# KVM-Explorer/AscendPathTracing

Hardware: AMD Instinct MI355X
Metric: Mray/s (ray segments per second) at 1920x1080, 8 bounces, 256 spp, demo scene (higher is better)
Workload: dtype f32; 1 GPU; C2: gen_spheres() 8-sphere scene, 1920x1080, S=64 (256 spp), depth 8, rays generated on device (counter RNG, seed 0), K-mode arithmetic, all segments traced (no retirement); segments_per_gpu=4246732800, parallelism=single GPU

## Files before the change

### __graft_entry__.py

```python
import os
import subprocess
import sys

ROOT = os.path.dirname(os.path.abspath(__file__))
if ROOT not in sys.path:
    sys.path.insert(0, ROOT)


def _is_current():
    import glob
    try:
        from ascendpathtracing_amd import _lib
    except ImportError:
        return False
    pkg = os.path.join(ROOT, "ascendpathtracing_amd")
    csrc = os.path.join(pkg, "csrc")
    pairs = [([os.path.join(pkg, "librender_mi355x.so"), os.path.join(pkg, "render_gpu")] + [st.built_path for st in _lib.STAGES.values()],
              glob.glob(os.path.join(csrc, "*.h")) + glob.glob(os.path.join(csrc, "*.hip")) + glob.glob(os.path.join(csrc, "*.cpp"))
              + [os.path.join(csrc, "Makefile"), os.path.join(csrc, "apt_exports.map")] + _lib.public_headers()),
             ([os.path.join(ROOT, "oracle", "libpt_oracle.so")],
              [os.path.join(ROOT, "oracle", "pt_oracle.c"), os.path.join(ROOT, "oracle", "Makefile")])]
    for outs, srcs in pairs:
        if not all(os.path.exists(o) for o in outs):
            return False
        if min(os.path.getmtime(o) for o in outs) < max(os.path.getmtime(x) for x in srcs):
            return False
    return True


def _load_all():
    import ascendpathtracing_amd
    from ascendpathtracing_amd import _lib
    _lib.lib()
    for name in _lib.STAGES:
        _lib.stage_lib(name)
    return ascendpathtracing_amd


def build():
    import fcntl
    if _is_current():
        return _load_all()
    with open(os.path.join(ROOT, ".build.lock"), "w") as lock:
        fcntl.flock(lock, fcntl.LOCK_EX)
        try:
            subprocess.run(["make", "-s", "-C", os.path.join(ROOT, "ascendpathtracing_amd", "csrc")], check=True, stdout=sys.stderr)
            subprocess.run(["make", "-s", "-C", os.path.join(ROOT, "oracle")], check=True, stdout=sys.stderr)
            tiny = os.path.join(ROOT, "profiles", "microbench", "lib_tiny_guard.so")
            lib_so = os.path.join(ROOT, "ascendpathtracing_amd", "librender_mi355x.so")
            if not os.path.exists(tiny) or os.path.getmtime(tiny) < os.path.getmtime(lib_so):
                r = subprocess.run(["bash", os.path.join(ROOT, "profiles", "build_variant.sh"), "tiny_guard", "-DAPT_TEST_TINY_GUARD"], stdout=sys.stderr)
                if r.returncode != 0:
                    print("build(): the test variant lib_tiny_guard.so could not be built (ignored)", file=sys.stderr)
        finally:
            fcntl.flock(lock, fcntl.LOCK_UN)
    return _load_all()


def smoke():
    build()
    import numpy as np
    import torch
    import ascendpathtracing_amd as apt
    from ascendpathtracing_amd import gen_data, render
    from oracle import oracle
    apt._lib.require_gpu()
    rays = gen_data.gen_rays(16, 16, 1, seed=0)
    sph = gen_data.gen_spheres()
    d_rays, d_sph = torch.from_numpy(rays.ravel()).cuda(), torch.from_numpy(sph).cuda()
    colors = torch.zeros(3 * 1024, device="cuda")
    render.set_default_params(apt.default_params())
    render.render_do(8, None, None, d_rays, d_sph, colors)
    torch.cuda.synchronize()
    want, _ = oracle.render_paths(oracle.make_params(16, 16, 1, depth=5, mode=oracle.MODE_K), rays, sph)
    got = colors.cpu().numpy().view(np.uint32)
    assert np.array_equal(got, want.ravel().view(np.uint32)), "render_do differs from the CPU restatement"
    for s_, d_ in ((8, 5), (32, 8)):
        p = apt.make_params(16, 16, s_, depth=d_, seed=1)
        fb, u8 = render.render_frame(p, d_sph)
        torch.cuda.synchronize()
        fb_w, u8_w, _, _ = oracle.render_frame(oracle.make_params(16, 16, s_, depth=d_, seed=1), sph, threads=4)
        assert np.array_equal(fb.cpu().numpy().view(np.uint32), fb_w.view(np.uint32)), "render_frame differs"
        assert np.array_equal(u8.cpu().numpy(), u8_w)
    print("smoke ok: render_do and render_frame are bit-identical to the oracle on", torch.cuda.get_device_name(0))


if __name__ == "__main__":
    build()
    if len(sys.argv) > 1 and sys.argv[1] == "smoke":
        smoke()
```

### ascendpathtracing_amd/csrc/apt_host.h

```cpp
#pragma once
#include <stdint.h>

#include <mutex>

#include "../../include/render_mi355x.h"
#include "pt_core.h"

#define APT_API __attribute__((visibility("default")))

namespace apt {

void clear_error();
int set_error(int code, const char *fmt, const char *detail = "");

constexpr uint32_t kDefaultRefillLanes = 32;
constexpr int kMaxStatusDevices = 16;

struct Debug {
    uint32_t queue_ppw = 0;
    uint32_t queue_nbuf = 0;
    uint32_t queue_lds_pad = 0;
    uint32_t grid_walk = 0;
    double grid_spheres_per_cell = 0;
};

}

struct apt_context {
    struct Values {
        apt_render_params params;
        unsigned long long *trace_counter;
        uint32_t refill_lanes;
        apt::Debug debug;
        bool has_camera = false;
        apt_camera camera;
        bool has_env = false;
        apt_environment env;
    };
    apt_context();
    Values snapshot();
    void set_params(const apt_render_params &p);
    void set_trace_counter(unsigned long long *c);
    void set_refill_lanes(uint32_t lanes);
    void set_camera(const apt_camera *cam_or_null);
    void set_environment(const apt_environment *env_or_null);
    int set_debug(const char *key, double value);
    int get_debug(const char *key, double *value);

    uint32_t *status_lookup(int dev);
    uint32_t *status_adopt(int dev, uint32_t *fresh, uint32_t **spare);
    void status_release(uint32_t *out[apt::kMaxStatusDevices]);

  private:
    std::mutex m_;
    Values v_;
    uint32_t *status_[apt::kMaxStatusDevices] = {};
};

namespace apt {
apt_context &default_context();
int film_resolve_check(const apt_film_resolve *r, const void *film, const void *table, const void *out, const void *u8, const char *what);
inline double grid_spheres_per_cell() {
    const double knob = default_context().snapshot().debug.grid_spheres_per_cell;
    return knob > 0.0 ? knob : kGridSpheresPerCell;
}
}
```

### ascendpathtracing_amd/csrc/pt_kernels.h

```cpp
#pragma once
#include "pt_trace.h"
#include "pt_trace2.h"
#include "pt_queue.h"
#include "pt_frame_mt.h"

namespace {

template <int MODE, int SC, bool RETIRE>
__global__ __launch_bounds__(kBlock, SC == kSceneGrid ? APT_GRID_WAVES : 1) void render_paths_kernel(const float *__restrict__ rays,
                                                              const float *__restrict__ sph,
                                                              float *__restrict__ colors, uint64_t n_total,
                                                              uint64_t begin, uint64_t count, TraceArgs ta) {
    constexpr bool NS8 = SC == kScene8;
    static_assert(!(RETIRE && NS8), "APT_FLAG_RETIRE on the 8-sphere scene is render_paths_queue_kernel's");
    __shared__ float4 tab[kTab8Floats4];
    __shared__ float4 tile[SC == kSceneTiles ? kTile : 1];
    Scene8 sc;
    Tab8 tab8{tab, tab + 8};
    if (NS8) tab8 = load_scene8(sph, sc, tab);
    const uint64_t local = (uint64_t)blockIdx.x * kBlock + threadIdx.x;
    const bool valid = local < count;
    const uint64_t p = begin + (valid ? local : 0);
    PathState s;
    path_init(s, rays[p], rays[n_total + p], rays[2 * n_total + p], rays[3 * n_total + p], rays[4 * n_total + p],
              rays[5 * n_total + p]);
    uint32_t traced;
    if (SC == kScene8) traced = trace_ns8<MODE, RETIRE>(sc, tab8, s, valid, ta, p);
    else if (SC == kSceneGrid) traced = trace_grid<MODE, RETIRE>(sph, ta.grid, s, valid, ta, p);
    else traced = trace_dyn<MODE, RETIRE>(sph, tile, s, valid, ta, p);
    if (valid) {
        const Gain3 gain = load_gain(sph, ta);
        colors[p] = s.rxy.x * gain.r;
        colors[n_total + p] = s.rxy.y * gain.g;
        colors[2 * n_total + p] = s.rz * gain.b;
    }
    count_traced(ta, valid ? traced : 0);
}

constexpr int kPaths2Pairs = 2;
template <int MODE>
__global__ __launch_bounds__(kBlock, APT_TWO_WAVES) void render_paths2_kernel(const float *__restrict__ rays, const float *__restrict__ sph,
                                                                              float *__restrict__ colors, uint64_t n_total, uint64_t begin,
                                                                              uint64_t count, TraceArgs ta) {
    __shared__ float4 tab[kTab8Floats4];
    Scene8 sc;
    const Tab8 tab8 = load_scene8(sph, sc, tab);
    const Gain3 gain = load_gain(sph, ta);
    uint32_t traced = 0;
    for (int it = 0; it < kPaths2Pairs; ++it) {
        const uint64_t local = ((uint64_t)blockIdx.x * kPaths2Pairs + it) * (2 * kBlock) + threadIdx.x;
        if (__builtin_amdgcn_readfirstlane((int)(((uint64_t)blockIdx.x * kPaths2Pairs + it) * (2 * kBlock) >= count))) break;
        const bool va = local < count, vb = local + kBlock < count;
        const uint64_t pa = begin + (va ? local : 0), pb = vb ? begin + local + kBlock : pa;
        PathPair pp;
        pp.ox = f2{rays[pa], rays[pb]}; pp.oy = f2{rays[n_total + pa], rays[n_total + pb]}; pp.oz = f2{rays[2 * n_total + pa], rays[2 * n_total + pb]};
        pp.dx = f2{rays[3 * n_total + pa], rays[3 * n_total + pb]}; pp.dy = f2{rays[4 * n_total + pa], rays[4 * n_total + pb]};
        pp.dz = f2{rays[5 * n_total + pa], rays[5 * n_total + pb]};
        trace2_ns8<MODE>(sc, tab8, pp, ta, sc.planes);
        if (va) { colors[pa] = pp.rx.x * gain.r; colors[n_total + pa] = pp.ry.x * gain.g; colors[2 * n_total + pa] = pp.rz.x * gain.b; }
        if (vb) { colors[pb] = pp.rx.y * gain.r; colors[n_total + pb] = pp.ry.y * gain.g; colors[2 * n_total + pb] = pp.rz.y * gain.b; }
        traced += ((va ? 1u : 0u) + (vb ? 1u : 0u)) * ta.depth;
    }
    count_traced(ta, traced);
}

constexpr uint32_t kQueueChunk = 64 * 16;
template <int MODE>
__global__ __launch_bounds__(kBlock) void render_paths_queue_kernel(const float *__restrict__ rays,
                                                                    const float *__restrict__ sph,
                                                                    float *__restrict__ colors, uint64_t n_total,
                                                                    uint64_t begin, uint64_t count, TraceArgs ta) {
    __shared__ float4 tab[kTab8Floats4];
    Scene8 sc;
    const Tab8 tab8 = load_scene8(sph, sc, tab);
    const Gain3 gain = load_gain(sph, ta);
    const KeyConsts kc = make_key_consts(ta.eps);
    const uint64_t wave = (uint64_t)blockIdx.x * (kBlock / 64) + (uint32_t)__builtin_amdgcn_readfirstlane((int)(threadIdx.x >> 6));
    uint64_t next = wave * kQueueChunk;
    const uint64_t end = min(count, next + kQueueChunk);
    uint32_t depth_left = 0, traced = 0;
    uint64_t cur = 0, cur_key = 0;
    PathState s, n;
    path_init(s, 0.f, 0.f, 0.f, 0.f, 0.f, 1.f);
    n = s;
    f2 thr_xy = {1.0f, 1.0f};
    float thr_z = 1.0f;
    uint64_t alive = 0;
    auto refill = [&](PathState &st) -> bool {
        for (;;) {
            const bool want = depth_left == 0;
            const unsigned long long wants = __ballot(want);
            if (next < end && wants) {
                const uint32_t rank = __builtin_amdgcn_mbcnt_hi((uint32_t)(wants >> 32), __builtin_amdgcn_mbcnt_lo((uint32_t)wants, 0u));
                const uint64_t remaining = end - next;
                const bool take = want && rank < remaining;
                if (take) {
                    cur = begin + next + rank;
                    st.oxy = f2{rays[cur], rays[n_total + cur]}; st.oz = rays[2 * n_total + cur];
                    st.dxy = f2{rays[3 * n_total + cur], rays[4 * n_total + cur]}; st.dz = rays[5 * n_total + cur];
                    thr_xy = f2{1.0f, 1.0f}; thr_z = 1.0f;
                    depth_left = ta.depth;
                    if (ta.rr_start) cur_key = rr_path_key(ta.seed, cur);
                    if (ta.depth == 0) { colors[cur] = gain.r; colors[n_total + cur] = gain.g; colors[2 * n_total + cur] = gain.b; }
                }
                alive |= __builtin_amdgcn_ballot_w64(take);
                next += min((uint64_t)__popcll(wants), remaining);
            }
            if (__any(depth_left != 0)) return false;
            if (next >= end) return true;
        }
    };
    auto post = [&](bool active) {
        if (ta.rr_start && ta.depth - depth_left + 1 >= ta.rr_start) {
            PathState t;
            t.rxy = thr_xy; t.rz = thr_z; t.alive = select_const(alive, 1);
            russian_roulette(t, cur_key, ta.depth - depth_left);
            thr_xy = t.rxy; thr_z = t.rz;
        }
        traced += active ? 1u : 0u;
        depth_left -= active ? 1u : 0u;
        const bool fin = select_const(alive, 1) == 0 || (thr_xy.x == 0.0f && thr_xy.y == 0.0f && thr_z == 0.0f);
        if (active && (depth_left == 0 || fin)) {
            depth_left = 0;
            colors[cur] = thr_xy.x * gain.r;
            colors[n_total + cur] = thr_xy.y * gain.g;
            colors[2 * n_total + cur] = thr_z * gain.b;
        }
    };
    auto step_fast = [&](const PathState &in, PathState &out) -> bool {
        const bool active = depth_left != 0;
        Albedo albedo;
        uint64_t alive_out = alive;
        const uint64_t redo = bounce_ns8_v2p<MODE>(sc, tab8, in, out, ta, kc, alive_out, albedo, sc.planes) & __builtin_amdgcn_ballot_w64(active);
        if (__builtin_expect(redo != 0, 0)) {
            const bool fin = select_const(alive, 1) == 0 || (thr_xy.x == 0.0f && thr_xy.y == 0.0f && thr_z == 0.0f);
            if (__any(select_const(redo, 1) != 0 && !fin)) return true;
        }
        apply_albedo(thr_xy, thr_z, albedo, alive_out);
        alive = alive_out;
        post(active);
        return false;
    };
    auto step_exact = [&](PathState &in, PathState &out) {
        const bool active = depth_left != 0;
        in.rxy = thr_xy; in.rz = thr_z; in.alive = select_const(alive, 1);
        bounce_ns8_exact<MODE>(sc, tab8, in, out, ta);
        thr_xy = out.rxy; thr_z = out.rz;
        alive = __builtin_amdgcn_ballot_w64(out.alive != 0);
        post(active);
    };
    bool done = refill(s), exact = !eps_allows_rootkey(ta.eps);
    if (!done && !exact) {
        for (;;) {
            if (__builtin_expect(step_fast(s, n), 0)) { exact = true; break; }
            if ((done = refill(n))) break;
            if (__builtin_expect(step_fast(n, s), 0)) { exact = true; s = n; break; }
            if ((done = refill(s))) break;
        }
    }
    if (!done && exact) {
        for (;;) {
            step_exact(s, n);
            s = n;
            if (refill(s)) break;
        }
    }
    count_traced(ta, traced);
}

template <int MODE, int SC, int GROUP, bool RETIRE, bool TWO = false>
__global__ __launch_bounds__(kBlock, TWO ? APT_TWO_WAVES : (SC == kSceneGrid ? APT_GRID_WAVES : (SC == kSceneTiles ? APT_TILE_WAVES : APT_FULL_WAVES))) void render_frame_kernel(const float *__restrict__ sph, FrameArgs fa,
                                                              TraceArgs ta, LeafProg lp) {
    constexpr bool NS8 = SC == kScene8;
    static_assert(!(RETIRE && NS8 && GROUP == 8), "APT_FLAG_RETIRE on the 8-sphere scene with samples >= 8 is render_frame_queue8_kernel's (pt_queue.h)");
    if (SC == kSceneGrid && ta.grid_walk == 2u && grid_queue_usable(ta)) return;
    __shared__ float4 tab[kTab8Floats4];
    __shared__ float4 tile[SC == kSceneTiles ? kTile : 1];
    extern __shared__ float dyn_lds[];
    float *stack_lds = dyn_lds;
    float *queue_lds = dyn_lds + (lp.nleaves > 1 ? kMaxStack * 3 * kStackSlots : 0);
    __shared__ Camera cam;
    park_camera(cam, fa);
    Scene8 sc;
    Tab8 tab8{tab, tab + 8};
    if (NS8) tab8 = load_scene8(sph, sc, tab);
    else __syncthreads();
    const bool planes = NS8 && sc.planes;
    (void)planes;

    const uint32_t lane = threadIdx.x & 63;
    const FrameLane<GROUP> fl = frame_lane<GROUP>(fa);
    const uint32_t j = fl.j, sub = fl.sub;
    const uint64_t pl = fl.pl;
    const bool valid = fl.valid;
    const uint32_t pi = fl.pi, pj = fl.pj, sy = fl.sy, sx = fl.sx;
    const uint64_t pbase = fl.pbase;
    uint32_t traced = 0;
    uint32_t queue_traced = 0;

    const Gain3 gain = load_gain(sph, ta);
    struct Col { float r, g, b; };
    auto sample = [&](uint32_t k) __attribute__((always_inline)) -> Col {
        uint64_t pb = pbase;
        if (TWO) {
            uint32_t tid = threadIdx.x;
            asm volatile("" : "+v"(tid));
            pb = frame_lane<GROUP>(fa, tid).pbase;
        }
        double u1, u2;
        path_uniforms(fa.seed, pb + k, u1, u2);
        float rox, roy, roz, rdx, rdy, rdz;
        camera_ray(cam, fa.width, fa.height, pi, pj, sy, sx, u1, u2, rox, roy, roz, rdx, rdy, rdz);
        PathState s;
        path_init(s, rox, roy, roz, rdx, rdy, rdz);
        if (SC == kScene8) traced += trace_ns8<MODE, RETIRE>(sc, tab8, s, valid, ta, pb + k);
        else if (SC == kSceneGrid) traced += trace_grid<MODE, RETIRE>(sph, ta.grid, s, valid, ta, pb + k);
        else traced += trace_dyn<MODE, RETIRE>(sph, tile, s, valid, ta, pb + k);
        return Col{s.rxy.x * gain.r, s.rxy.y * gain.g, s.rz * gain.b};
    };
    auto add = [](const Col &a, const Col &b) { return Col{a.r + b.r, a.g + b.g, a.b + b.b}; };
    struct Col2 { Col a, b; };
    const uint64_t lane_state = TWO ? lane_base_state(fa.seed, pbase, j) : 0;
    auto sample2 = [&](uint32_t u) __attribute__((always_inline)) -> Col2 {
        PathPair pp;
        camera_ray_pair(cam, fa.width, fa.height, pi, pj, sy, sx, chain_state_uniform(lane_state, u), pp.ox, pp.oy, pp.oz, pp.dx, pp.dy, pp.dz);
        asm("" : "+v"(pp.ox), "+v"(pp.oy), "+v"(pp.oz), "+v"(pp.dx), "+v"(pp.dy), "+v"(pp.dz));
        trace2_ns8<MODE>(sc, tab8, pp, ta, planes);
        traced += 2 * ta.depth;
        return Col2{Col{pp.rx.x * gain.r, pp.ry.x * gain.g, pp.rz.x * gain.b}, Col{pp.rx.y * gain.r, pp.ry.y * gain.g, pp.rz.y * gain.b}};
    };

    float res[3] = {0.0f, 0.0f, 0.0f};
    uint32_t start = 0;
    int sp = 0;
    for (uint32_t leaf = 0; leaf < lp.nleaves; ++leaf) {
        const uint32_t n = lp.len(leaf);
        float acc[3];
        if (GROUP == 1) {
            Col a = {0.0f, 0.0f, 0.0f};
            for (uint32_t k = 0; k < n; ++k) a = add(a, sample(start + k));
            acc[0] = a.r; acc[1] = a.g; acc[2] = a.b;
        } else {
            const uint32_t nfull = n & ~7u;
            if (RETIRE && SC == kSceneTiles) {
                float *colq = queue_lds + (size_t)(threadIdx.x >> 6) * 3u * 8u * lp.maxleaf;
                const uint32_t total = 8u * nfull;
                const uint32_t qstride = 8u * lp.maxleaf;
                uint32_t next = 0;
                uint32_t depth_left = 0, cur_item = 0, slot_item = 0;
                uint64_t cur_key = 0, slot_key = 0;
                uint32_t n_bounce_exec = 0, n_gen_exec = 0;
                float sl_ox = 0.f, sl_oy = 0.f, sl_oz = 0.f, sl_dx = 0.f, sl_dy = 0.f, sl_dz = 1.f;
                bool slot_full = false, slot_valid = false, cur_valid = false;
                PathState s;
                path_init(s, 0.f, 0.f, 0.f, 0.f, 0.f, 1.f);
                auto refill = [&](PathState &cur) -> bool {
                    for (;;) {
                        const bool want = !slot_full;
                        const unsigned long long wants = __ballot(want);
                        const bool busy_any = __any(depth_left != 0 || slot_full);
                        if (next < total && wants && ((uint32_t)__popcll(wants) >= ta.refill_lanes || !busy_any)) {
                            ++n_gen_exec;
                            const uint32_t rank = __builtin_amdgcn_mbcnt_hi((uint32_t)(wants >> 32),
                                                  __builtin_amdgcn_mbcnt_lo((uint32_t)wants, 0u));
                            const uint32_t remaining = total - next;
                            const bool take = want && rank < remaining;
                            const uint32_t item = take ? next + rank : 0u;
                            const uint32_t g = item / nfull, k = item - g * nfull;
                            const int src = (int)(8u * g);
                            const uint32_t gpi = __shfl(pi, src, 64), gpj = __shfl(pj, src, 64);
                            const uint32_t gsub = __shfl(sub, src, 64);
                            const uint32_t blo = __shfl((uint32_t)pbase, src, 64), bhi = __shfl((uint32_t)(pbase >> 32), src, 64);
                            const bool gvalid = __shfl((int)valid, src, 64) != 0;
                            if (take) {
                                slot_valid = gvalid;
                                double u1, u2;
                                const uint64_t path = (((uint64_t)bhi << 32) | blo) + start + k;
                                if (ta.rr_start) slot_key = rr_path_key(ta.seed, path);
                                path_uniforms(fa.seed, path, u1, u2);
                                camera_ray(cam, fa.width, fa.height, gpi, gpj, gsub >> 1, gsub & 1u, u1, u2, sl_ox, sl_oy, sl_oz, sl_dx,
                                           sl_dy, sl_dz);
                                slot_item = item;
                                slot_full = true;
                            }
                            next += min((uint32_t)__popcll(wants), remaining);
                        }
                        const bool begin = depth_left == 0 && slot_full;
                        if (begin) {
                            cur.oxy = f2{sl_ox, sl_oy}; cur.oz = sl_oz; cur.dxy = f2{sl_dx, sl_dy}; cur.dz = sl_dz;
                            cur.rxy = f2{1.0f, 1.0f}; cur.rz = 1.0f; cur.alive = 1u;
                            cur_item = slot_item;
                            cur_key = slot_key;
                            cur_valid = slot_valid;
                            depth_left = ta.depth;
                            slot_full = false;
                            if (ta.depth == 0 || !cur_valid) {
                                depth_left = 0;
                                colq[cur_item] = gain.r; colq[qstride + cur_item] = gain.g; colq[2 * qstride + cur_item] = gain.b;
                            }
                        }
                        if (__any(depth_left != 0)) return false;
                        if (next >= total && !__any(slot_full)) return true;
                    }
                };
                for (;;) {
                    const bool wave_done = refill(s);
                    if (__syncthreads_and(wave_done)) break;
                    const bool active = depth_left != 0;
                    dyn_segment<MODE>(sph, tile, s, !active, ta);
                    ++n_bounce_exec;
                    if (active && ta.rr_start && ta.depth - depth_left + 1 >= ta.rr_start)
                        russian_roulette(s, cur_key, ta.depth - depth_left);
                    queue_traced += (active && cur_valid) ? 1u : 0u;
                    depth_left -= active ? 1u : 0u;
                    if (active && (depth_left == 0 || path_finished(s))) {
                        depth_left = 0;
                        colq[cur_item] = s.rxy.x * gain.r;
                        colq[qstride + cur_item] = s.rxy.y * gain.g;
                        colq[2 * qstride + cur_item] = s.rz * gain.b;
                    }
                }
                __syncthreads();
                {
                    const uint32_t base = (lane >> 3) * nfull + j;
#pragma unroll
                    for (int ch = 0; ch < 3; ++ch) acc[ch] = colq[ch * qstride + base];
                    for (uint32_t i8 = 8; i8 < nfull; i8 += 8) {
#pragma unroll
                        for (int ch = 0; ch < 3; ++ch) acc[ch] = acc[ch] + colq[ch * qstride + base + i8];
                    }
                }
                __syncthreads();
                if (ta.traced && lane == 0) {
                    atomicAdd(ta.traced + 1, 64ull * n_bounce_exec);
                    atomicAdd(ta.traced + 2, 64ull * n_gen_exec);
                }
            } else {
                Col a;
                uint32_t i8;
                if (TWO && nfull >= 16) {
                    Col2 c = sample2(start);
                    a = add(c.a, c.b);
                    for (i8 = 16; i8 + 16 <= nfull; i8 += 16) {
                        c = sample2(start + i8);
                        a = add(a, c.a);
                        a = add(a, c.b);
                    }
                } else {
                    a = sample(start + j);
                    i8 = 8;
                }
                for (; i8 < nfull; i8 += 8) a = add(a, sample(start + i8 + j));
                acc[0] = a.r; acc[1] = a.g; acc[2] = a.b;
            }
#pragma unroll
            for (int ch = 0; ch < 3; ++ch) {
                float v = acc[ch];
                v = v + __shfl_xor(v, 1, 64);
                v = v + __shfl_xor(v, 2, 64);
                v = v + __shfl_xor(v, 4, 64);
                acc[ch] = v;
            }
            const uint32_t nt = n - nfull;
            if (nt) {
                const uint32_t traced_before = traced;
                const Col c = sample(start + nfull + (j < nt ? j : 0));
                if (j >= nt) traced = traced_before;
                for (uint32_t t = 0; t < nt; ++t) {
                    const int src = (int)((lane & ~7u) + t);
                    acc[0] = acc[0] + __shfl(c.r, src, 64);
                    acc[1] = acc[1] + __shfl(c.g, src, 64);
                    acc[2] = acc[2] + __shfl(c.b, src, 64);
                }
            }
        }
        start += n;
        if (lp.nleaves == 1) {
            res[0] = acc[0]; res[1] = acc[1]; res[2] = acc[2];
        } else {
#pragma unroll
            for (int ch = 0; ch < 3; ++ch) stack_lds[(sp * 3 + ch) * kStackSlots + (threadIdx.x >> 3)] = acc[ch];
            ++sp;
            for (uint32_t m = 0; m < lp.ncomb(leaf); ++m) {
                --sp;
#pragma unroll
                for (int ch = 0; ch < 3; ++ch) {
                    const float a = stack_lds[((sp - 1) * 3 + ch) * kStackSlots + (threadIdx.x >> 3)];
                    const float b = stack_lds[(sp * 3 + ch) * kStackSlots + (threadIdx.x >> 3)];
                    stack_lds[((sp - 1) * 3 + ch) * kStackSlots + (threadIdx.x >> 3)] = a + b;
                }
            }
        }
    }
    if (lp.nleaves > 1) {
#pragma unroll
        for (int ch = 0; ch < 3; ++ch) res[ch] = stack_lds[ch * kStackSlots + (threadIdx.x >> 3)];
    }

    __shared__ uint32_t u8pack[frame_u8_words(GROUP)];
    frame_decode<GROUP, TWO>(fa, pl, valid, res, u8pack);
    count_traced(ta, (valid ? traced : 0) + queue_traced);
}

__global__ __launch_bounds__(kBlock) void test_scene_kernel(const float *__restrict__ rays,
                                                            const float *__restrict__ sph, float *__restrict__ out,
                                                            uint64_t n_total, uint32_t ns, int32_t light, float eps) {
    const uint64_t p = (uint64_t)blockIdx.x * kBlock + threadIdx.x;
    if (p >= n_total) return;
    const float ox = rays[p], oy = rays[n_total + p], oz = rays[2 * n_total + p];
    const float dx = rays[3 * n_total + p], dy = rays[4 * n_total + p], dz = rays[5 * n_total + p];
    float mind = kMissT;
    int id = -1;
    for (uint32_t k = 0; k < ns; ++k)
        test_scene_sphere(sph[ns + k], sph[2 * (size_t)ns + k], sph[3 * (size_t)ns + k], sph[k], ox, oy, oz, dx, dy, dz,
                          eps, (int)k, mind, id);
#pragma unroll
    for (int c = 0; c < 3; ++c) {
        float v = 0.0f;
        if (id >= 0) v = (id == light) ? sph[(size_t)(4 + c) * ns + id] : sph[(size_t)(7 + c) * ns + id];
        out[(uint64_t)c * n_total + p] = v;
    }
}

__global__ __launch_bounds__(kBlock) void gen_rays_kernel(Camera cam, uint32_t width, uint32_t height,
                                                          uint32_t samples, uint64_t seed, uint64_t n_total,
                                                          uint64_t begin, uint64_t count, float *__restrict__ rays) {
    const uint64_t local = (uint64_t)blockIdx.x * kBlock + threadIdx.x;
    if (local >= count) return;
    const uint64_t p = begin + local;
    uint32_t i, j, sy, sx;
    path_coords(p, height, samples, i, j, sy, sx);
    double u1, u2;
    path_uniforms(seed, p, u1, u2);
    float rox, roy, roz, rdx, rdy, rdz;
    camera_ray(cam, width, height, i, j, sy, sx, u1, u2, rox, roy, roz, rdx, rdy, rdz);
    rays[p] = rox; rays[n_total + p] = roy; rays[2 * n_total + p] = roz;
    rays[3 * n_total + p] = rdx; rays[4 * n_total + p] = rdy; rays[5 * n_total + p] = rdz;
}

constexpr int kMtN = 624, kMtM = 397, kPathsPerBlock = 156;

__device__ __forceinline__ uint32_t mt_temper(uint32_t y) {
    y ^= y >> 11;
    y ^= (y << 7) & 0x9d2c5680u;
    y ^= (y << 15) & 0xefc60000u;
    y ^= y >> 18;
    return y;
}

constexpr int kMtGroup = 8;

__global__ __launch_bounds__(kBlock) void gen_rays_mt_kernel(const uint32_t *__restrict__ checkpoints, uint32_t stride,
                                                             uint64_t first_block, uint64_t num_blocks, Camera cam, uint32_t width,
                                                             uint32_t height, uint32_t samples, uint64_t n_total,
                                                             uint64_t begin, uint64_t end, float *__restrict__ rays) {
    __shared__ uint32_t mt[kMtN];
    __shared__ __align__(16) uint32_t outw[kMtGroup * kMtN];
    const uint64_t cb = first_block + (uint64_t)blockIdx.x * stride;
    for (int i = threadIdx.x; i < kMtN; i += kBlock) mt[i] = checkpoints[(uint64_t)blockIdx.x * kMtN + i];
    __syncthreads();
    const uint64_t last = min(cb + stride, num_blocks);
    for (uint64_t g0 = cb; g0 < last; g0 += kMtGroup) {
        const uint32_t nb = (uint32_t)min((uint64_t)kMtGroup, last - g0);
        for (uint32_t bl = 0; bl < nb; ++bl) {
            if (g0 + bl != cb) {
                const int t = threadIdx.x;
                const int lo[3] = {0, 227, 454}, hi[3] = {227, 454, 624};
#pragma unroll
                for (int ph = 0; ph < 3; ++ph) {
                    const int i = lo[ph] + t;
                    uint32_t v = 0;
                    const bool on = i < hi[ph];
                    if (on) {
                        const uint32_t y = (mt[i] & 0x80000000u) | (mt[(i + 1) % kMtN] & 0x7fffffffu);
                        v = mt[(i + kMtM) % kMtN] ^ (y >> 1) ^ ((y & 1u) ? 0x9908b0dfu : 0u);
                    }
                    __syncthreads();
                    if (on) mt[i] = v;
                    __syncthreads();
                }
            }
            for (int i = threadIdx.x; i < kMtN; i += kBlock) outw[bl * kMtN + i] = mt_temper(mt[i]);
        }
        __syncthreads();
        const uint64_t pbase = g0 * kPathsPerBlock;
        const uint64_t rb = pbase / samples;
        const uint32_t kb = (uint32_t)(pbase - rb * samples);
        const uint32_t npaths = nb * kPathsPerBlock;
        for (uint32_t q = threadIdx.x; q < npaths; q += kBlock) {
            const uint64_t p = pbase + q;
            if (p < begin || p >= end) continue;
            const uint4 w4 = *reinterpret_cast<const uint4 *>(&outw[4 * q]);
            const uint32_t a1 = w4.x >> 5, b1 = w4.y >> 6, a2 = w4.z >> 5, b2 = w4.w >> 6;
            const double u1 = ((double)a1 * 67108864.0 + (double)b1) / 9007199254740992.0;
            const double u2 = ((double)a2 * 67108864.0 + (double)b2) / 9007199254740992.0;
            const uint64_t r = rb + (kb + q) / samples;
            const uint32_t sx = (uint32_t)(r & 1), sy = (uint32_t)((r >> 1) & 1);
            const uint64_t r4 = r >> 2;
            uint32_t i, j;
            if (r4 <= 0xffffffffull) { i = (uint32_t)r4 / height; j = (uint32_t)r4 - i * height; }
            else { i = (uint32_t)(r4 / height); j = (uint32_t)(r4 % height); }
            float rox, roy, roz, rdx, rdy, rdz;
            camera_ray(cam, width, height, i, j, sy, sx, u1, u2, rox, roy, roz, rdx, rdy, rdz);
            rays[p] = rox; rays[n_total + p] = roy; rays[2 * n_total + p] = roz;
            rays[3 * n_total + p] = rdx; rays[4 * n_total + p] = rdy; rays[5 * n_total + p] = rdz;
        }
        __syncthreads();
    }
}

__device__ float pairwise_leaf(const float *a, uint32_t n) {
    if (n < 8) {
        float r = 0.0f;
        for (uint32_t i = 0; i < n; ++i) r = r + a[i];
        return r;
    }
    float r[8];
#pragma unroll
    for (int k = 0; k < 8; ++k) r[k] = a[k];
    uint32_t i;
    for (i = 8; i < n - (n % 8); i += 8) {
#pragma unroll
        for (int k = 0; k < 8; ++k) r[k] = r[k] + a[i + k];
    }
    float res = ((r[0] + r[1]) + (r[2] + r[3])) + ((r[4] + r[5]) + (r[6] + r[7]));
    for (; i < n; ++i) res = res + a[i];
    return res;
}

__global__ __launch_bounds__(kBlock) void decode_color_kernel(const float *__restrict__ colors, uint32_t samples,
                                                              uint64_t npix, LeafProg lp, float *__restrict__ fb,
                                                              uint8_t *__restrict__ fb_u8) {
    const uint64_t L = (uint64_t)blockIdx.x * kBlock + threadIdx.x;
    const uint32_t sub = (uint32_t)(L & 3);
    const uint64_t pc = L >> 2;
    const bool valid = pc < 3 * npix;
    const uint64_t ch = valid ? pc / npix : 0, q = valid ? pc % npix : 0;
    const uint64_t n_total = npix * 4 * samples;
    const float *a = colors + ch * n_total + (q * 4 + sub) * samples;
    float st[kMaxStack];
    int sp = 0;
    uint32_t start = 0;
    for (uint32_t leaf = 0; leaf < lp.nleaves; ++leaf) {
        st[sp++] = pairwise_leaf(a + start, lp.len(leaf));
        start += lp.len(leaf);
        for (uint32_t m = 0; m < lp.ncomb(leaf); ++m) { --sp; st[sp - 1] = st[sp - 1] + st[sp]; }
    }
    const float mean = st[0] / (float)samples;
    const int gbase = (int)((threadIdx.x & 63) & ~3u);
    double acc = 0.0;
#pragma unroll
    for (int sq = 0; sq < 4; ++sq) acc = acc + (double)__shfl(mean, gbase + sq, 64);
    const double v = acc / 4;
    const double cl = v < 0 ? 0 : (v > 1 ? 1 : v);
    if (valid && sub == 0) {
        fb[ch * npix + q] = (float)cl;
        if (fb_u8) fb_u8[q * 3 + ch] = (uint8_t)(cl * 255);
    }
}

__global__ __launch_bounds__(kBlock) void decode_color_kernel8(const float *__restrict__ colors, uint32_t samples,
                                                               uint64_t npix, LeafProg lp, float *__restrict__ fb,
                                                               uint8_t *__restrict__ fb_u8) {
    __shared__ float stack_lds[kMaxStack * kStackSlots];
    const uint32_t lane = threadIdx.x & 63;
    const uint32_t j = threadIdx.x & 7u;
    const uint32_t sub = (threadIdx.x >> 3) & 3u;
    const uint32_t slot = threadIdx.x >> 3;
    const uint64_t n_total = npix * 4 * samples;
    const uint64_t items = 3 * npix, per_block = kBlock / 32;
    const uint64_t rounds = (items + per_block * gridDim.x - 1) / (per_block * gridDim.x);
    for (uint64_t r = 0; r < rounds; ++r) {
    const uint64_t pc = (r * gridDim.x + blockIdx.x) * per_block + (threadIdx.x >> 5);
    const bool valid = pc < items;
    const uint64_t ch = valid ? pc / npix : 0, q = valid ? pc % npix : 0;
    const float *a = colors + ch * n_total + (q * 4 + sub) * samples;
    float res = 0.0f;
    uint32_t start = 0;
    int sp = 0;
    for (uint32_t leaf = 0; leaf < lp.nleaves; ++leaf) {
        const uint32_t n = lp.len(leaf), nfull = n & ~7u;
        float v[16];
#pragma unroll
        for (int m = 0; m < 16; ++m) v[m] = (8u * m < nfull) ? a[start + 8u * m + j] : 0.0f;
        float acc = v[0];
#pragma unroll
        for (int m = 1; m < 16; ++m)
            if (8u * m < nfull) acc = acc + v[m];
        acc = acc + __shfl_xor(acc, 1, 64);
        acc = acc + __shfl_xor(acc, 2, 64);
        acc = acc + __shfl_xor(acc, 4, 64);
        const uint32_t nt = n - nfull;
        if (nt) {
            const float c = a[start + nfull + (j < nt ? j : 0)];
            for (uint32_t t = 0; t < nt; ++t) acc = acc + __shfl(c, (int)((lane & ~7u) + t), 64);
        }
        start += n;
        if (lp.nleaves == 1) {
            res = acc;
        } else {
            stack_lds[sp * kStackSlots + slot] = acc;
            ++sp;
            for (uint32_t m = 0; m < lp.ncomb(leaf); ++m) {
                --sp;
                const float x = stack_lds[(sp - 1) * kStackSlots + slot], y = stack_lds[sp * kStackSlots + slot];
                stack_lds[(sp - 1) * kStackSlots + slot] = x + y;
            }
        }
    }
    if (lp.nleaves > 1) res = stack_lds[slot];
    const float mean = res / (float)samples;
    const int gbase = (int)(lane & ~31u);
    double acc64 = 0.0;
#pragma unroll
    for (int sq = 0; sq < 4; ++sq) acc64 = acc64 + (double)__shfl(mean, gbase + sq * 8, 64);
    const double v = acc64 / 4;
    const double cl = v < 0 ? 0 : (v > 1 ? 1 : v);
    if (valid && (lane & 31u) == 0) {
        fb[ch * npix + q] = (float)cl;
        if (fb_u8) fb_u8[q * 3 + ch] = (uint8_t)(cl * 255);
    }
    }
}

constexpr int kDecode4Blocks = 4;
__global__ __launch_bounds__(kBlock) void decode_color_kernel4(const float *__restrict__ colors, uint32_t samples, uint64_t npix, LeafProg lp,
                                                               float *__restrict__ fb, uint8_t *__restrict__ fb_u8) {
    const uint32_t lane = threadIdx.x & 63;
    const uint32_t L = threadIdx.x & 1u;
    const uint32_t sub = (threadIdx.x >> 1) & 3u;
    const uint64_t n_total = npix * 4 * samples;
    const uint64_t items = 3 * npix, per_block = kBlock / 8;
    const uint64_t rounds = (items + per_block * gridDim.x - 1) / (per_block * gridDim.x);
    const uint32_t n = lp.len(0), nfull = n & ~7u, nt = n - nfull;
    for (uint64_t r = 0; r < rounds; ++r) {
        const uint64_t pc = (r * gridDim.x + blockIdx.x) * per_block + (threadIdx.x >> 3);
        const bool valid = pc < items;
        const uint64_t ch = valid ? pc / npix : 0, q = valid ? pc % npix : 0;
        const float *a = colors + ch * n_total + (q * 4 + sub) * samples;
        float4 v[kDecode4Blocks];
#pragma unroll
        for (int m = 0; m < kDecode4Blocks; ++m)
            v[m] = (8u * m < nfull) ? *reinterpret_cast<const float4 *>(a + 8u * m + 4u * L) : make_float4(0.f, 0.f, 0.f, 0.f);
        float4 acc = v[0];
#pragma unroll
        for (int m = 1; m < kDecode4Blocks; ++m)
            if (8u * m < nfull) { acc.x = acc.x + v[m].x; acc.y = acc.y + v[m].y; acc.z = acc.z + v[m].z; acc.w = acc.w + v[m].w; }
        float res = (acc.x + acc.y) + (acc.z + acc.w);
        res = res + __shfl_xor(res, 1, 64);
        if (nt) {
            float c[4];
#pragma unroll
            for (int k = 0; k < 4; ++k) c[k] = (4u * L + k < nt) ? a[nfull + 4u * L + k] : 0.0f;
#pragma unroll
            for (int t = 0; t < 7; ++t)
                if ((uint32_t)t < nt) res = res + __shfl(c[t & 3], (int)((lane & ~1u) + (t >> 2)), 64);
        }
        const float mean = res / (float)samples;
        const int gbase = (int)(lane & ~7u);
        double acc64 = 0.0;
#pragma unroll
        for (int sq = 0; sq < 4; ++sq) acc64 = acc64 + (double)__shfl(mean, gbase + sq * 2, 64);
        const double v64 = acc64 / 4;
        const double cl = v64 < 0 ? 0 : (v64 > 1 ? 1 : v64);
        if (valid && (lane & 7u) == 0) {
            fb[ch * npix + q] = (float)cl;
            if (fb_u8) fb_u8[q * 3 + ch] = (uint8_t)(cl * 255);
        }
    }
}

__global__ __launch_bounds__(kBlock) void selftest_sqrt_kernel(int variant, uint64_t begin, uint64_t count,
                                                               unsigned long long *result) {
#if defined(__HIP_DEVICE_COMPILE__)
    const uint64_t stride = (uint64_t)gridDim.x * kBlock;
    unsigned long long bad = 0, first = ~0ull;
    for (uint64_t i = (uint64_t)blockIdx.x * kBlock + threadIdx.x; i < count; i += stride) {
        const uint32_t bits = (uint32_t)(begin + i);
        const float x = __uint_as_float(bits);
        float amin = 1.0f;
        const float got = variant == 0 ? sqrt_rn_core(x, amin) : variant == 1 ? sqrt_rn_markstein(x, amin)
                        : variant == 2 ? sqrt_rn_rsq1(x, amin) : sqrt_rn_rsq2(x, amin);
        const float want = sqrtf(x);
        const bool fallback = amin < 0x1p-96f;
        const bool same = (__float_as_uint(got) == __float_as_uint(want)) || (got != got && want != want);
        if (!same && !fallback) { ++bad; if (first == ~0ull) first = bits; }
    }
    if (bad) {
        atomicAdd(&result[0], bad);
        atomicMin(&result[1], first);
    }
#endif
}

__global__ __launch_bounds__(kBlock) void selftest_div3_kernel(uint64_t begin, uint64_t count,
                                                               unsigned long long *result) {
#if defined(__HIP_DEVICE_COMPILE__)
    const uint64_t stride = (uint64_t)gridDim.x * kBlock;
    unsigned long long bad = 0, first = ~0ull, accepted = 0;
    if (blockIdx.x == 0 && threadIdx.x == 0) {
        const float qn = __uint_as_float(0x7fc00000u);
        float one = 1.0f, a = -0.5f, b = 3.0f;
        asm volatile("" : "+v"(one), "+v"(a), "+v"(b));
        const float m0 = minimum3_abs(one, a, b), m1 = minimum3_abs(one, qn, b), m2 = minimum3_abs(one, b, -qn), m3 = minimum3_abs(qn, a, b);
        if (!(m0 == 0.5f) || m1 == m1 || m2 == m2 || m3 == m3 || (m1 >= kFastMin) || !(m0 >= kFastMin)) { ++bad; first = 0; }
    }
    for (uint64_t i = (uint64_t)blockIdx.x * kBlock + threadIdx.x; i < count; i += stride) {
        const uint64_t ctr = begin + i;
        uint64_t h = splitmix64(ctr);
        float v[3];
#pragma unroll
        for (int k = 0; k < 3; ++k) {
            h = splitmix64(h);
            uint32_t man = (uint32_t)h & 0x7fffffu, ex = 127u - 100u + (uint32_t)((h >> 23) % 134u), sg = (uint32_t)(h >> 63);
            if ((ctr & 3u) == 0u) {
                const uint32_t pick = (uint32_t)(h >> 40) & 7u;
                man = pick == 0 ? 0x7fffffu : pick == 1 ? 0u : pick == 2 ? 1u : pick == 3 ? 0x7ffffeu
                    : pick == 4 ? 0x400000u : pick == 5 ? 0x3fffffu : pick == 6 ? 0x400001u : man;
                if (((h >> 44) & 3u) == 0u) ex = ((h >> 46) & 1u) ? 127u - 96u : 127u + 29u;
            }
            v[k] = __uint_as_float((sg << 31) | (ex << 23) | man);
        }
        if ((ctr & 63u) == 1u) v[(ctr >> 6) % 3u] = (ctr & 64u) ? 0.0f : -0.0f;
        const uint32_t how = (uint32_t)((ctr >> 2) % 3u);
        float len2, d;
        if (how == 0) {
            len2 = 0.0f + v[0] * v[0];
            len2 = len2 + v[1] * v[1];
            len2 = len2 + v[2] * v[2];
            d = sqrtf(len2);
        } else if (how == 1) {
            const float p0 = v[0] * v[0], p1 = v[1] * v[1], p2 = v[2] * v[2];
            double acc = 0.0 + (double)p0;
            acc = acc + (double)p1;
            acc = acc + (double)p2;
            len2 = (float)acc;
            d = sqrtf(len2);
        } else {
            h = splitmix64(h);
            uint32_t man = (uint32_t)h & 0x7fffffu;
            const uint32_t ex = 127u - 50u + (uint32_t)((h >> 23) % 84u);
            if ((ctr & 3u) == 0u) man = ((h >> 40) & 1u) ? 0x7fffffu : 0u;
            d = __uint_as_float((ex << 23) | man);
            len2 = d * d;
        }
        const float wx = v[0] / d, wy = v[1] / d, wz = v[2] / d;
        {
            float ux, uy, uz, amin = 1.0f;
            uint32_t hiflag = 0;
            div3_shared(v[0], v[1], v[2], d, len2, ux, uy, uz, amin, hiflag);
            if (!(amin < 0x1p-96f || (int32_t)hiflag < 0)) {
                ++accepted;
                if (__float_as_uint(ux) != __float_as_uint(wx) || __float_as_uint(uy) != __float_as_uint(wy) ||
                    __float_as_uint(uz) != __float_as_uint(wz)) { ++bad; if (first == ~0ull) first = ctr; }
            }
        }
        if (div3_operands_ok(len2, v[0], v[1], v[2])) {
            ++accepted;
            f2 uxy;
            float uz;
            div3_packed(f2{v[0], v[1]}, v[2], d, uxy, uz);
            if (__float_as_uint(uxy.x) != __float_as_uint(wx) || __float_as_uint(uxy.y) != __float_as_uint(wy) ||
                __float_as_uint(uz) != __float_as_uint(wz)) { ++bad; if (first == ~0ull) first = ctr; }
        }
    }
    if (bad) { atomicAdd(&result[0], bad); atomicMin(&result[1], first); }
    atomicAdd(&result[2], accepted);
#endif
}


}
```

### ascendpathtracing_amd/csrc/pt_trace.h

```cpp
#pragma once
#include <hip/hip_runtime.h>
#include <stdint.h>

#include "pt_core.h"
#include "pt_leaf.h"

namespace {

using namespace apt;


constexpr int kBlock = 256;
constexpr int kScene8 = 0, kSceneTiles = 1, kSceneGrid = 2;
constexpr int kTile = 1024;
#ifndef APT_GRID_WAVES
#define APT_GRID_WAVES 8
#endif
#ifndef APT_TILE_WAVES
#define APT_TILE_WAVES 6
#endif
#ifndef APT_TWO_WAVES
#define APT_TWO_WAVES 4
#endif
#ifndef APT_FULL_WAVES
#define APT_FULL_WAVES 6
#endif
constexpr int kMaxStack = 8;
constexpr int kStackSlots = kBlock / 8;


struct Scene8 {
    float cx[8], cy[8], cz[8], r2[8];
    bool planes;
};
__device__ __forceinline__ bool scene8_shares_planes(const Scene8 &sc) {
    auto eq = [](float a, float b) { return f32_bits(a) == f32_bits(b); };
    return eq(sc.cx[2], sc.cx[3]) && eq(sc.cx[2], sc.cx[4]) && eq(sc.cx[2], sc.cx[5]) && eq(sc.cx[2], sc.cx[7]) &&
           eq(sc.cy[0], sc.cy[1]) && eq(sc.cy[0], sc.cy[2]) && eq(sc.cy[0], sc.cy[3]) &&
           eq(sc.cz[0], sc.cz[1]) && eq(sc.cz[0], sc.cz[4]) && eq(sc.cz[0], sc.cz[5]) && eq(sc.cz[0], sc.cz[7]);
}

struct Tab8 { const float4 *geo, *alb; };
constexpr int kTab8Floats4 = 17;

struct TraceArgs {
    uint32_t ns;
    uint32_t depth;
    int32_t light;
    float eps, gain;
    uint32_t refill_lanes;
    uint32_t emission;
    uint32_t rr_start;
    uint64_t seed;
    const uint32_t *grid;
    uint32_t grid_walk;
    unsigned long long *traced;
    uint32_t *status;
};
template <uint32_t K>
__device__ __forceinline__ uint32_t xcd_chunked_block(uint32_t wg, uint32_t nwg) {
    constexpr uint32_t kXcds = 8, G = kXcds * K;
    static_assert((K & (K - 1)) == 0, "shifts and masks");
    const uint32_t full = nwg & ~(G - 1u);
    if (wg >= full) return wg;
    const uint32_t r = wg & (G - 1u);
    return (wg & ~(G - 1u)) + (r & (kXcds - 1u)) * K + r / kXcds;
}

__device__ __forceinline__ void report_status(const TraceArgs &ta, uint32_t bit) {
    if (ta.status && (threadIdx.x & 63u) == 0u) atomicOr(ta.status, bit);
}


__device__ __forceinline__ float twice_canonical(float dot) { return __builtin_fmaf(dot, 2.0f, 0.0f); }
__device__ __forceinline__ f2 twice_canonical(f2 dot) { return __builtin_elementwise_fma(dot, f2{2.0f, 2.0f}, f2{0.0f, 0.0f}); }

__device__ __forceinline__ float sum3_f64(float p0, float p1, float p2) {
    double acc = (double)p0;
    acc = acc + (double)p1;
    acc = acc + (double)p2;
    return (float)acc;
}

template <int MODE>
__device__ __forceinline__ float normal_len2(f2 nxy, float nz) {
    const f2 sq = nxy * nxy;
    if (MODE == kModeOracle) return sum3_f64(sq.x, sq.y, nz * nz);
    const float acc = sq.x + sq.y;
    return acc + nz * nz;
}
template <int MODE>
__device__ __forceinline__ float reflect_k2(f2 dxy, float dz, f2 uxy, float uz) {
    const f2 pr = dxy * uxy;
    const float pz = dz * uz;
    if (MODE == kModeOracle) return twice_canonical(sum3_f64(pr.x, pr.y, pz));
    float dot = pr.x;
    dot = dot + pr.y;
    dot = dot + pz;
    return twice_canonical(dot);
}

struct HitPre2 { f2 b, disc; };
__device__ __forceinline__ HitPre2 intersect_pre2(const f2 cx, const f2 cy, const f2 cz, const f2 r2, float ox,
                                                  float oy, float oz, float dx, float dy, float dz) {
    const f2 ocx = cx - ox, ocy = cy - oy, ocz = cz - oz;
    f2 b = ocx * dx;
    b = b + ocy * dy;
    b = b + ocz * dz;
    f2 c = ocx * ocx;
    c = c + ocy * ocy;
    c = c + ocz * ocz;
    c = c - r2;
    f2 disc = b * b;
    disc = disc - c;
    return {b, disc};
}
__device__ __forceinline__ HitPre2 intersect_pre2(const float4 a, const float4 c4, float ox, float oy, float oz,
                                                  float dx, float dy, float dz) {
    return intersect_pre2(f2{a.x, a.y}, f2{a.z, a.w}, f2{c4.x, c4.y}, f2{c4.z, c4.w}, ox, oy, oz, dx, dy, dz);
}


template <bool WANT_C67 = false>
__device__ __forceinline__ void intersect_pre_planes_pairs(const f2 X1, const f2 X2, const f2 Y1, const f2 Y2, const f2 Y3, const f2 Z1, const f2 Z2,
                                                           const f2 R0, const f2 R1, const f2 R2, const f2 R3, float ox, float oy, float oz,
                                                           float dx, float dy, float dz, HitPre2 (&h)[4], f2 *c67 = nullptr) {
    const f2 x1 = X1 - ox, x2 = X2 - ox, y1 = Y1 - oy, y2 = Y2 - oy, y3 = Y3 - oy, z1 = Z1 - oz, z2 = Z2 - oz;
    auto lo = [](f2 v) { return f2{v.x, v.x}; };
    auto swap = [](f2 v) { return f2{v.y, v.x}; };
    {
        const f2 px1 = x1 * dx, px2 = x2 * dx, py1 = y1 * dy, py2 = y2 * dy, py3 = y3 * dy, pz1 = z1 * dz, pz2 = z2 * dz;
        h[0].b = (px1 + py3) + lo(pz2);
        h[1].b = (lo(px2) + py3) + pz1;
        h[2].b = (lo(px2) + py1) + lo(pz2);
        h[3].b = (swap(px2) + py2) + swap(pz2);
    }
    {
        const f2 qx1 = x1 * x1, qx2 = x2 * x2, qy1 = y1 * y1, qy2 = y2 * y2, qy3 = y3 * y3, qz1 = z1 * z1, qz2 = z2 * z2;
        f2 c0 = (qx1 + qy3) + lo(qz2), c1 = (lo(qx2) + qy3) + qz1, c2 = (lo(qx2) + qy1) + lo(qz2), c3 = (swap(qx2) + qy2) + swap(qz2);
        c0 = c0 - R0; c1 = c1 - R1; c2 = c2 - R2; c3 = c3 - R3;
        h[0].disc = h[0].b * h[0].b - c0; h[1].disc = h[1].b * h[1].b - c1;
        h[2].disc = h[2].b * h[2].b - c2; h[3].disc = h[3].b * h[3].b - c3;
        if (WANT_C67) *c67 = c3;
    }
}
template <bool WANT_C67 = false>
__device__ __forceinline__ void intersect_pre_planes(const Scene8 &sc, float ox, float oy, float oz, float dx, float dy, float dz,
                                                     HitPre2 (&h)[4], f2 *c67 = nullptr) {
    intersect_pre_planes_pairs<WANT_C67>(f2{sc.cx[0], sc.cx[1]}, f2{sc.cx[2], sc.cx[6]}, f2{sc.cy[4], sc.cy[5]}, f2{sc.cy[6], sc.cy[7]}, f2{sc.cy[0], sc.cy[0]},
                               f2{sc.cz[2], sc.cz[3]}, f2{sc.cz[0], sc.cz[6]}, f2{sc.r2[0], sc.r2[1]}, f2{sc.r2[2], sc.r2[3]}, f2{sc.r2[4], sc.r2[5]},
                               f2{sc.r2[6], sc.r2[7]}, ox, oy, oz, dx, dy, dz, h, c67);
}

template <int MODE>
__device__ __forceinline__ void bounce_ns8_exact(const Scene8 &sc, const Tab8 tab, const PathState &s, PathState &n,
                                                 const TraceArgs &ta) {
    const int miss = (MODE == kModeOracle) ? -1 : 0;
    float tmin = kMissT;
    int idx = miss;
#pragma unroll
    for (int k = 0; k < 8; ++k) {
        float t0, t1;
        intersect_roots(sc.cx[k], sc.cy[k], sc.cz[k], sc.r2[k], s.oxy.x, s.oxy.y, s.oz, s.dxy.x, s.dxy.y, s.dz, t0, t1);
        const float t = select_root(t0, t1, ta.eps);
        if (t < tmin) { tmin = t; idx = k; }
    }
    const int g = (idx < 0) ? 7 : idx;
    const float4 c = tab.geo[g], col = tab.alb[g];
    n = s;
    shade_and_reflect<MODE>(n, tmin, c.x, c.y, c.z, col.x, col.y, col.z, idx == ta.light);
}

struct KeyConsts { uint32_t bias, init; uint64_t nbias2; };
__device__ __forceinline__ KeyConsts make_key_consts(float eps) {
    KeyConsts kc;
    kc.bias = f32_bits(eps) + 1u;
    kc.init = f32_bits(kMissT) - kc.bias;
    kc.nbias2 = ((uint64_t)(0u - kc.bias) << 32) | (0x80000000u - kc.bias);
    asm volatile("" : "+v"(kc.bias), "+v"(kc.init));
    asm volatile("" : "+s"(kc.nbias2));
    return kc;
}
template <int HALF>
__device__ __forceinline__ uint64_t root_pair(f2 b, f2 q) {
    uint64_t r;
    if (HALF == 0) asm("v_pk_add_f32 %0, %1, %2 op_sel:[0,0] op_sel_hi:[0,0] neg_lo:[1,0] neg_hi:[0,0]" : "=v"(r) : "v"(b), "v"(q));
    else asm("v_pk_add_f32 %0, %1, %2 op_sel:[1,1] op_sel_hi:[1,1] neg_lo:[1,0] neg_hi:[0,0]" : "=v"(r) : "v"(b), "v"(q));
    return r;
}
__device__ __forceinline__ float min3_abs(float a, float b, float c) {
    float r;
    asm("v_min3_f32 %0, %1, |%2|, |%3|" : "=v"(r) : "v"(a), "v"(b), "v"(c));
    return r;
}
constexpr float kFastMin = 0x1p-29f;
__device__ __forceinline__ float minimum3_abs(float a, float b, float c) {
    float r;
    asm("v_minimum3_f32 %0, %1, |%2|, |%3|" : "=v"(r) : "v"(a), "v"(b), "v"(c));
    return r;
}
__device__ __forceinline__ float minimum3_abs_after_trans(float a, float b, float c) {
    float r;
    asm("s_nop 0\n\tv_minimum3_f32 %0, %1, |%2|, |%3|" : "=v"(r) : "v"(a), "v"(b), "v"(c));
    return r;
}
__device__ __forceinline__ float rsq_here(float x) {
    float r;
    asm("v_rsq_f32 %0, %1\n\ts_nop 0" : "=v"(r) : "v"(x));
    return r;
}
__device__ __forceinline__ uint32_t min3_u32(uint32_t a, uint32_t b, uint32_t c) {
    uint32_t r;
    asm("v_min3_u32 %0, %1, %2, %3" : "=v"(r) : "v"(a), "v"(b), "v"(c));
    return r;
}
__device__ __forceinline__ uint32_t select_const(uint64_t mask, uint32_t value_if_set) {
    uint32_t r;
    asm("" : "+s"(mask));
    asm("v_cndmask_b32_e64 %0, 0, %1, %2" : "=v"(r) : "n"(value_if_set), "s"(mask));
    return r;
}

struct Albedo { f2 xy; float z; };
__device__ __forceinline__ void apply_albedo(f2 &rxy, float &rz, const Albedo &a, uint64_t alive) {
    uint64_t saved;
    asm("" : "+s"(alive));
    asm volatile("s_and_saveexec_b64 %[sv], %[m]\n\t"
                 "v_pk_mul_f32 %[rxy], %[cxy], %[rxy]\n\t"
                 "v_mul_f32 %[rz], %[cz], %[rz]\n\t"
                 "s_mov_b64 exec, %[sv]"
                 : [sv] "=&s"(saved), [rxy] "+v"(rxy), [rz] "+v"(rz)
                 : [m] "s"(alive), [cxy] "v"(a.xy), [cz] "v"(a.z)
                 : "scc");
}

struct Hit8 { float tmin; uint32_t addr; uint64_t light; };
__device__ __forceinline__ bool pair_misses_wave(f2 disc) {
    return __builtin_amdgcn_ballot_w64(__builtin_fmaxf(disc.x, disc.y) >= 0.0f) == 0;
}
constexpr float kBehindGuard = 0x1p-60f;
__device__ __forceinline__ uint64_t sphere_reachable_mask(float disc, float b, float c) {
    return __builtin_amdgcn_ballot_w64(__builtin_amdgcn_fmed3f(disc, b, -c) >= -kBehindGuard);
}
__device__ __forceinline__ uint32_t any_lane(uint64_t mask) {
    uint32_t r;
    asm("s_cmp_lg_u64 %1, 0\n\ts_cselect_b32 %0, 1, 0" : "=s"(r) : "s"(mask) : "scc");
    return r;
}
template <int MODE, bool PLANES = false, int SKIP = 0>
__device__ __forceinline__ Hit8 intersect_ns8_v2(const Scene8 &sc, float ox, float oy, float oz, float dx, float dy, float dz,
                                                 const TraceArgs &ta, const KeyConsts &kc, float &amin) {
    uint32_t best = kc.init;
    uint64_t b0 = 0, b1 = 0, b2 = 0, any = 0;
    auto update_keys = [&](uint32_t m0, uint32_t m1, int k) {
        const uint32_t nb = min3_u32(best, m0, m1);
        const uint64_t better = __builtin_amdgcn_ballot_w64(nb != best);
        best = nb;
        b0 = (k & 1) ? (b0 | better) : (b0 & ~better);
        b1 = (k & 2) ? (b1 | better) : (b1 & ~better);
        b2 = (k & 4) ? (b2 | better) : (b2 & ~better);
        if (MODE == kModeOracle) any |= better;
    };
    auto update64 = [&](uint64_t keys, int k) { update_keys((uint32_t)keys, (uint32_t)(keys >> 32), k); };
    auto full_stage = [&](const HitPre2 &h, int k) __attribute__((always_inline)) {
        amin = minimum3_abs(amin, h.disc.x, h.disc.y);
        const f2 q = sqrt_rn_rsq1_pair(h.disc);
        update64(root_pair<0>(h.b, q) + kc.nbias2, k);
        update64(root_pair<1>(h.b, q) + kc.nbias2, k + 1);
    };
    static_assert((SKIP >> 4) == 0 || ((SKIP >> 4) == 0x8 && PLANES), "the per-sphere form: pair (6,7) of the shared-planes form only");
    HitPre2 hp[4];
    f2 c67 = {0.0f, 0.0f};
    if (PLANES) intersect_pre_planes<(SKIP >> 4) != 0>(sc, ox, oy, oz, dx, dy, dz, hp, &c67);
#pragma unroll
    for (int k = 0; k < 8; k += 2) {
        const HitPre2 h = PLANES ? hp[k / 2]
                                 : intersect_pre2(f2{sc.cx[k], sc.cx[k + 1]}, f2{sc.cy[k], sc.cy[k + 1]}, f2{sc.cz[k], sc.cz[k + 1]},
                                                  f2{sc.r2[k], sc.r2[k + 1]}, ox, oy, oz, dx, dy, dz);
        if ((SKIP >> (k / 2)) & 1) {
            if (pair_misses_wave(h.disc)) continue;
        }
        if ((SKIP >> (4 + k / 2)) & 1) {
            const uint32_t lo = any_lane(sphere_reachable_mask(h.disc.x, h.b.x, c67.x)), hi = any_lane(sphere_reachable_mask(h.disc.y, h.b.y, c67.y));
            uint32_t both = lo & hi, only_lo = lo & ~hi, only_hi = hi & ~lo;
            asm("" : "+s"(both), "+s"(only_lo), "+s"(only_hi));
            if (both != 0u) full_stage(h, k);
            if (only_lo != 0u) {
                amin = minimum3_abs(amin, h.disc.x, h.disc.x);
                const float r0 = rsq_here(h.disc.x);
                update64(root_pair<0>(h.b, sqrt_rsq_step(h.disc, f2{r0, r0})) + kc.nbias2, k);
            }
            if (only_hi != 0u) {
                amin = minimum3_abs(amin, h.disc.y, h.disc.y);
                const float r0 = rsq_here(h.disc.y);
                update64(root_pair<1>(h.b, sqrt_rsq_step(h.disc, f2{r0, r0})) + kc.nbias2, k + 1);
            }
            continue;
        }
        full_stage(h, k);
    }
    const float tmin = bits_f32(best + kc.bias);
    uint64_t light_mask;
    if (MODE == kModeOracle) {
        b0 |= ~any; b1 |= ~any; b2 |= ~any;
    }
    uint32_t addr;
    {
        const uint32_t a0 = select_const(b0, 16), a1 = select_const(b1, 32), a2 = select_const(b2, 64);
        asm("v_or3_b32 %0, %1, %2, %3" : "=v"(addr) : "v"(a0), "v"(a1), "v"(a2));
    }
    light_mask = __builtin_amdgcn_ballot_w64(addr == (uint32_t)ta.light * 16u);
    if (MODE == kModeOracle) light_mask &= any;
    return Hit8{tmin, addr, light_mask};
}

template <int MODE, bool PLANES = false, bool CAN_BE_LAST = false>
__device__ __forceinline__ uint64_t bounce_ns8_v2(const Scene8 &sc, const Tab8 tab, const PathState &s, PathState &n,
                                                  const TraceArgs &ta, const KeyConsts &kc, uint64_t &alive, Albedo &albedo, bool last = false) {
    float amin = 1.0f;
    const Hit8 hit = intersect_ns8_v2<MODE, PLANES>(sc, s.oxy.x, s.oxy.y, s.oz, s.dxy.x, s.dxy.y, s.dz, ta, kc, amin);
    const float tmin = hit.tmin;
    const uint32_t addr = hit.addr;
    const uint64_t light_mask = hit.light;
    const float4 c = *reinterpret_cast<const float4 *>(reinterpret_cast<const char *>(tab.geo) + addr);
    const float4 col = *reinterpret_cast<const float4 *>(reinterpret_cast<const char *>(tab.alb) + addr);
    if (!(CAN_BE_LAST && last)) {
        const f2 oxy = s.oxy, dxy = s.dxy;
        const f2 hxy = oxy + dxy * tmin;
        const float hz = s.oz + s.dz * tmin;
        const f2 nxy = hxy - f2{c.x, c.y};
        const float nz = hz - c.z;
        const float len2 = normal_len2<MODE>(nxy, nz);
        const float r0 = __builtin_amdgcn_rsqf(len2);
        amin = minimum3_abs_after_trans(amin, r0, nxy.x);
        amin = minimum3_abs(amin, nxy.y, nz);
        const float L = sqrt_rsq_step(len2, r0);
        f2 uxy;
        float uz;
        div3_packed(nxy, nz, L, uxy, uz);
        const float k2 = reflect_k2<MODE>(dxy, s.dz, uxy, uz);
        n.dxy = dxy - uxy * k2;
        n.dz = s.dz - uz * k2;
        n.oxy = hxy; n.oz = hz;
    }
    alive &= ~light_mask;
    n.alive = s.alive;
    albedo = Albedo{f2{col.x, col.y}, col.z};
    return __builtin_amdgcn_ballot_w64(!(amin >= kFastMin));
}

struct Bounce8Mid {
    f2 hxy, nxy;
    float hz, nz, len2, r0;
    float4 col;
    uint64_t light;
};
template <int MODE, bool PLANES>
__device__ __forceinline__ uint64_t bounce_ns8_v2_hit(const Scene8 &sc, const Tab8 tab, const PathState &s, const TraceArgs &ta, const KeyConsts &kc,
                                                      Bounce8Mid &m) {
    float amin = 1.0f;
    const Hit8 hit = intersect_ns8_v2<MODE, PLANES>(sc, s.oxy.x, s.oxy.y, s.oz, s.dxy.x, s.dxy.y, s.dz, ta, kc, amin);
    const float tmin = hit.tmin;
    const float4 c = *reinterpret_cast<const float4 *>(reinterpret_cast<const char *>(tab.geo) + hit.addr);
    m.col = *reinterpret_cast<const float4 *>(reinterpret_cast<const char *>(tab.alb) + hit.addr);
    m.light = hit.light;
    m.hxy = s.oxy + s.dxy * tmin;
    m.hz = s.oz + s.dz * tmin;
    m.nxy = m.hxy - f2{c.x, c.y};
    m.nz = m.hz - c.z;
    m.len2 = normal_len2<MODE>(m.nxy, m.nz);
    m.r0 = __builtin_amdgcn_rsqf(m.len2);
    amin = minimum3_abs_after_trans(amin, m.r0, m.nxy.x);
    amin = minimum3_abs(amin, m.nxy.y, m.nz);
    return __builtin_amdgcn_ballot_w64(!(amin >= kFastMin));
}
template <int MODE>
__device__ __forceinline__ void bounce_ns8_v2_reflect(PathState &s, const Bounce8Mid &m, uint64_t &alive, Albedo &albedo) {
    const float L = sqrt_rsq_step(m.len2, m.r0);
    f2 uxy;
    float uz;
    div3_packed(m.nxy, m.nz, L, uxy, uz);
    const float k2 = reflect_k2<MODE>(s.dxy, s.dz, uxy, uz);
    s.dxy = s.dxy - uxy * k2;
    s.dz = s.dz - uz * k2;
    s.oxy = m.hxy; s.oz = m.hz;
    alive &= ~m.light;
    albedo = Albedo{f2{m.col.x, m.col.y}, m.col.z};
}

template <int MODE>
__device__ __forceinline__ float reflect_packed(const PathState &s, float tmin, float cx, float cy, float cz, PathState &n) {
    const f2 hxy = s.oxy + s.dxy * tmin;
    const float hz = s.oz + s.dz * tmin;
    const f2 nxy = hxy - f2{cx, cy};
    const float nz = hz - cz;
    const float len2 = normal_len2<MODE>(nxy, nz);
    const float r0 = __builtin_amdgcn_rsqf(len2);
    float amin = minimum3_abs_after_trans(1.0f, r0, nxy.x);
    amin = minimum3_abs(amin, nxy.y, nz);
    const float L = sqrt_rsq_step(len2, r0);
    f2 uxy;
    float uz;
    div3_packed(nxy, nz, L, uxy, uz);
    const float k2 = reflect_k2<MODE>(s.dxy, s.dz, uxy, uz);
    n.dxy = s.dxy - uxy * k2;
    n.dz = s.dz - uz * k2;
    n.oxy = hxy; n.oz = hz;
    return amin;
}

template <int MODE>
__device__ __forceinline__ uint64_t bounce_ns8_v2p(const Scene8 &sc, const Tab8 tab, const PathState &s, PathState &n, const TraceArgs &ta,
                                                   const KeyConsts &kc, uint64_t &alive, Albedo &albedo, bool planes) {
    return planes ? bounce_ns8_v2<MODE, true>(sc, tab, s, n, ta, kc, alive, albedo)
                  : bounce_ns8_v2<MODE, false>(sc, tab, s, n, ta, kc, alive, albedo);
}

template <int MODE>
__device__ __forceinline__ void bounce_ns8_checked(const Scene8 &sc, const Tab8 tab, const PathState &s, PathState &n,
                                                   const TraceArgs &ta, const KeyConsts &kc, bool fast_ok,
                                                   uint64_t &alive, bool want_lane_alive, uint64_t active = ~0ull) {
    const uint64_t alive_in = alive;
    uint64_t redo = ~0ull;
    Albedo albedo;
    bool fast_stands = false;
    if (__builtin_expect(fast_ok, 1)) { redo = bounce_ns8_v2p<MODE>(sc, tab, s, n, ta, kc, alive, albedo, sc.planes); fast_stands = true; }
    if (__builtin_expect((redo & active) != 0, 0)) {
        PathState cold = s;
        cold.alive = select_const(alive_in, 1);
        const bool lane = select_const(redo & active, 1) != 0 && (!fast_ok || !path_finished(cold));
        if (__any(lane)) {
            asm volatile("" ::: "memory");
            bounce_ns8_exact<MODE>(sc, tab, cold, n, ta);
            alive = __builtin_amdgcn_ballot_w64(n.alive != 0);
            fast_stands = false;
            if (ta.traced && (threadIdx.x & 63) == 0) atomicAdd(ta.traced + 3, 1ull);
        }
    }
    if (__builtin_expect(fast_stands, 1)) {
        n.rxy = s.rxy; n.rz = s.rz;
        apply_albedo(n.rxy, n.rz, albedo, alive);
    }
    if (want_lane_alive) n.alive = select_const(alive, 1);
}

template <int MODE, bool RETIRE>
__device__ __forceinline__ uint32_t trace_ns8(const Scene8 &sc, const Tab8 tab, PathState &s, bool valid,
                                              const TraceArgs &ta, uint64_t path) {
    uint32_t traced = 0;
    const uint64_t rr_key = ta.rr_start ? rr_path_key(ta.seed, path) : 0;
    const KeyConsts kc = make_key_consts(ta.eps);
    const bool fast_ok = eps_allows_rootkey(ta.eps);
    const bool lane_alive = RETIRE || ta.rr_start != 0;
    uint64_t alive = __builtin_amdgcn_ballot_w64(s.alive != 0);
    if (RETIRE) {
        for (uint32_t d = 0; d < ta.depth; ++d) {
            const bool fin = !valid || path_finished(s);
            if (__all(fin)) break;
            PathState n;
            uint64_t alive_n = alive;
            bounce_ns8_checked<MODE>(sc, tab, s, n, ta, kc, fast_ok, alive_n, true);
            if (ta.rr_start && d + 1 >= ta.rr_start) russian_roulette(n, rr_key, d);
            if (!fin) { s = n; ++traced; }
            alive = __builtin_amdgcn_ballot_w64(s.alive != 0);
        }
    } else {
        f2 rxy = s.rxy;
        float rz = s.rz;
        auto rest_exact = [&](PathState &from, uint32_t d) {
            from.alive = select_const(alive, 1);
            from.rxy = rxy; from.rz = rz;
            for (; d < ta.depth; ++d) {
                PathState n;
                bounce_ns8_exact<MODE>(sc, tab, from, n, ta);
                if (ta.rr_start && d + 1 >= ta.rr_start) russian_roulette(n, rr_key, d);
                from = n;
            }
            if (ta.traced && (threadIdx.x & 63) == 0) atomicAdd(ta.traced + 3, 1ull);
            s = from;
        };
        auto step = [&](PathState &in, PathState &out, uint32_t d) -> bool {
            Albedo albedo;
            uint64_t alive_out = alive;
            const bool last = d + 1 == ta.depth;
            const uint64_t redo = sc.planes ? bounce_ns8_v2<MODE, true, true>(sc, tab, in, out, ta, kc, alive_out, albedo, last)
                                            : bounce_ns8_v2<MODE, false, true>(sc, tab, in, out, ta, kc, alive_out, albedo, last);
            if (__builtin_expect(redo != 0, 0)) {
                const bool fin = select_const(alive, 1) == 0 || (rxy.x == 0.0f && rxy.y == 0.0f && rz == 0.0f);
                if (__any(select_const(redo, 1) != 0 && !fin)) return true;
            }
            apply_albedo(rxy, rz, albedo, alive_out);
            alive = alive_out;
            if (ta.rr_start && d + 1 >= ta.rr_start) {
                PathState t;
                t.rxy = rxy; t.rz = rz; t.alive = select_const(alive, 1);
                russian_roulette(t, rr_key, d);
                rxy = t.rxy; rz = t.rz;
            }
            return false;
        };
        traced = ta.depth;
        PathState n;
        uint32_t d = 0;
        if (__builtin_expect(!fast_ok, 0)) { rest_exact(s, 0); return traced; }
        for (; d + 2 <= ta.depth; d += 2) {
            if (__builtin_expect(step(s, n, d), 0)) { rest_exact(s, d); return traced; }
            if (__builtin_expect(step(n, s, d + 1), 0)) { rest_exact(n, d + 1); return traced; }
        }
        if (d < ta.depth) {
            if (__builtin_expect(step(s, n, d), 0)) { rest_exact(s, d); return traced; }
        }
        s.rxy = rxy; s.rz = rz;
        if (lane_alive) s.alive = select_const(alive, 1);
    }
    return traced;
}

template <class Update>
__device__ __forceinline__ void tile_scan(const float *sph, float4 *tile, uint32_t ns, float eps, float ox, float oy, float oz,
                                          float dx, float dy, float dz, Update &&update) {
    const float *r2 = sph, *cx = sph + ns, *cy = sph + 2 * (size_t)ns, *cz = sph + 3 * (size_t)ns;
    for (uint32_t base = 0; base < ns; base += kTile) {
        const uint32_t n = min((uint32_t)kTile, ns - base);
        __syncthreads();
        {
            float *tf = reinterpret_cast<float *>(tile);
            const uint32_t n4 = (n + 3u) & ~3u;
            for (uint32_t k = threadIdx.x; k < n4; k += kBlock) {
                const bool real = k < n;
                const float qn = __uint_as_float(0x7fc00000u);
                const uint32_t o = (k >> 1) * 8u + (k & 1u);
                tf[o] = real ? cx[base + k] : qn;
                tf[o + 2] = real ? cy[base + k] : qn;
                tf[o + 4] = real ? cz[base + k] : qn;
                tf[o + 6] = real ? r2[base + k] : qn;
            }
        }
        __syncthreads();
        auto hit = [&](float b, float disc, uint32_t sphere) {
            if (__any(disc >= 0.0f)) update(intersect_post(HitPre{b, disc}, eps), sphere);
        };
        for (uint32_t k = 0; k < n; k += 4) {
            const float4 a0 = tile[k], c0 = tile[k + 1], a1 = tile[k + 2], c1 = tile[k + 3];
            const HitPre2 h01 = intersect_pre2(a0, c0, ox, oy, oz, dx, dy, dz);
            const HitPre2 h23 = intersect_pre2(a1, c1, ox, oy, oz, dx, dy, dz);
            const float m = fmaxf(fmaxf(h01.disc.x, h01.disc.y), fmaxf(h23.disc.x, h23.disc.y));
            if (__any(m >= 0.0f)) {
                hit(h01.b.x, h01.disc.x, base + k);
                hit(h01.b.y, h01.disc.y, base + k + 1);
                hit(h23.b.x, h23.disc.x, base + k + 2);
                hit(h23.b.y, h23.disc.y, base + k + 3);
            }
        }
    }
}

template <int MODE>
__device__ __forceinline__ void dyn_segment(const float *__restrict__ sph, float4 *tile, PathState &s, bool fin,
                                            const TraceArgs &ta) {
    const uint32_t ns = ta.ns;
    const float *cx = sph + ns, *cy = sph + 2 * (size_t)ns, *cz = sph + 3 * (size_t)ns;
    const float *colx = sph + 7 * (size_t)ns, *coly = sph + 8 * (size_t)ns, *colz = sph + 9 * (size_t)ns;
    float tmin = kMissT;
    int idx = (MODE == kModeOracle) ? -1 : 0;
    tile_scan(sph, tile, ns, ta.eps, s.oxy.x, s.oxy.y, s.oz, s.dxy.x, s.dxy.y, s.dz, [&](float t, uint32_t sphere) __attribute__((always_inline)) {
        if (t < tmin) { tmin = t; idx = (int)sphere; }
    });
    const uint32_t g = (idx < 0) ? ns - 1 : (uint32_t)idx;
    PathState n = s;
    shade_and_reflect<MODE>(n, tmin, cx[g], cy[g], cz[g], colx[g], coly[g], colz[g], idx == ta.light);
    if (!fin) s = n;
}

template <int MODE, bool RETIRE>
__device__ __forceinline__ uint32_t trace_dyn(const float *__restrict__ sph, float4 *tile, PathState &s, bool valid,
                                              const TraceArgs &ta, uint64_t path) {
    const uint64_t rr_key = ta.rr_start ? rr_path_key(ta.seed, path) : 0;
    uint32_t traced = 0;
    for (uint32_t d = 0; d < ta.depth; ++d) {
        const bool fin = !valid || (RETIRE && path_finished(s));
        if (RETIRE && __syncthreads_and(fin)) break;
        dyn_segment<MODE>(sph, tile, s, fin, ta);
        if (!fin) {
            if (ta.rr_start && d + 1 >= ta.rr_start) russian_roulette(s, rr_key, d);
            ++traced;
        }
    }
    return traced;
}

__device__ __forceinline__ void grid_stats(const TraceArgs &ta, uint32_t n_cells, uint32_t n_tests) {
    if (ta.traced) {
        unsigned long long c = n_cells, t = n_tests;
        for (int off = 32; off > 0; off >>= 1) { c += __shfl_xor(c, off, 64); t += __shfl_xor(t, off, 64); }
        if ((threadIdx.x & 63) == 0) { atomicAdd(ta.traced + 1, c); atomicAdd(ta.traced + 2, t); }
    }
}

template <class TestItem, class Nearest>
__device__ __forceinline__ void grid_walk_cells(const GridHeader &h, const uint32_t *cells, const float4 *item_geom, float ox, float oy, float oz,
                                                float dx, float dy, float dz, uint32_t &n_cells, uint32_t &n_tests, TestItem &&test_item,
                                                Nearest &&nearest) {
    const int n0 = (int)h.n[0], n1 = (int)h.n[1], n2 = (int)h.n[2];
    float tn = 0.0f, tf = 3.0e38f;
    bool inbox = true;
    auto recip = [&](float dv) {
#if defined(__HIP_DEVICE_COMPILE__)
        return __builtin_amdgcn_rcpf(dv);
#else
        return 1.0f / dv;
#endif
    };
    const float ix = recip(dx), iy = recip(dy), iz = recip(dz);
    auto slab = [&](float o, float dv, float inv, float lo, float hi) {
        if (fabsf(dv) > 1e-20f) {
            const float t1 = (lo - o) * inv, t2 = (hi - o) * inv;
            tn = fmaxf(tn, fminf(t1, t2));
            tf = fminf(tf, fmaxf(t1, t2));
        } else if (!(o >= lo && o <= hi)) inbox = false;
    };
    slab(ox, dx, ix, h.gmin[0], h.gmax[0]);
    slab(oy, dy, iy, h.gmin[1], h.gmax[1]);
    slab(oz, dz, iz, h.gmin[2], h.gmax[2]);
    if (inbox && tn <= tf) {
        auto axis = [&](float o, float dv, float inv, float lo, float cellw, float invw, int na, int &c, int &step,
                        float &tmax, float &tdel) {
            int ci = (int)floorf((o + dv * tn - lo) * invw);
            ci = ci < 0 ? 0 : (ci >= na ? na - 1 : ci);
            c = ci;
            if (dv > 1e-20f) { step = 1; tmax = (lo + (float)(ci + 1) * cellw - o) * inv; tdel = cellw * inv; }
            else if (dv < -1e-20f) { step = -1; tmax = (lo + (float)ci * cellw - o) * inv; tdel = -cellw * inv; }
            else { step = 0; tmax = 3.0e38f; tdel = 3.0e38f; }
        };
        int c0, c1, c2, st0, st1, st2;
        float tm0, tm1, tm2, td0, td1, td2;
        axis(ox, dx, ix, h.gmin[0], h.cell[0], h.inv_cell[0], n0, c0, st0, tm0, td0);
        axis(oy, dy, iy, h.gmin[1], h.cell[1], h.inv_cell[1], n1, c1, st1, tm1, td1);
        axis(oz, dz, iz, h.gmin[2], h.cell[2], h.inv_cell[2], n2, c2, st2, tm2, td2);
        const int max_steps = n0 + n1 + n2 + 3;
        uint32_t cell = (uint32_t)((c2 * n1 + c1) * n0 + c0);
        uint32_t b = cells[cell], e = cells[cell + 1];
        for (int it = 0; it < max_steps; ++it) {
            ++n_cells;
            n_tests += e - b;
            const float te = fminf(tm0, fminf(tm1, tm2));
            const bool s0 = tm0 <= tm1 && tm0 <= tm2, s1 = !s0 && tm1 <= tm2, s2 = !s0 && !s1;
            if (s0) { c0 += st0; tm0 += td0; }
            if (s1) { c1 += st1; tm1 += td1; }
            if (s2) { c2 += st2; tm2 += td2; }
            const bool inside = (unsigned)c0 < (unsigned)n0 && (unsigned)c1 < (unsigned)n1 && (unsigned)c2 < (unsigned)n2;
            uint32_t nb = 0, ne = 0;
            if (inside) {
                cell = (uint32_t)((c2 * n1 + c1) * n0 + c0);
                nb = cells[cell];
                ne = cells[cell + 1];
            }
            uint32_t i = b;
            for (; i + 2 <= e; i += 2) {
                const float4 ga = item_geom[i], gb = item_geom[i + 1];
                test_item(ga, i);
                test_item(gb, i + 1);
            }
            if (i < e) test_item(item_geom[i], i);
            if (nearest() < te - (1e-3f * fabsf(te) + h.margin)) break;
            if (!inside) break;
            b = nb;
            e = ne;
        }
    }
}

struct GridCtx {
    const GridHeader *h;
    const float *sph;
    const uint32_t *grid;
    const TraceArgs *ta;
};

template <int MODE>
__device__ __forceinline__ void grid_segment(const GridCtx &ctx, PathState &s, bool fin, uint32_t &n_cells, uint32_t &n_tests) {
    const GridHeader &h = *ctx.h;
    const TraceArgs &ta = *ctx.ta;
    const float *__restrict__ sph = ctx.sph;
    const uint32_t *__restrict__ grid = ctx.grid;
    const uint32_t ns = ta.ns;
    const uint32_t *large = grid + h.off_large, *cells = grid + h.off_cells, *items = grid + h.off_items;
    const float4 *geom = reinterpret_cast<const float4 *>(grid + h.off_geom);
    const float4 *item_geom = reinterpret_cast<const float4 *>(grid + h.off_item_geom);
    const float *colx = sph + 7 * (size_t)ns, *coly = sph + 8 * (size_t)ns, *colz = sph + 9 * (size_t)ns;
    const bool grid_ok = h.magic == kGridMagic && h.num_spheres == ns;
    const float *r2p = sph, *cxp = sph + ns, *cyp = sph + 2 * (size_t)ns, *czp = sph + 3 * (size_t)ns;
        float tmin = kMissT;
    int idx = (MODE == kModeOracle) ? -1 : 0;
    auto test_geom = [&](const float4 g, uint32_t k) {
        const HitPre hp = intersect_pre(g.x, g.y, g.z, g.w, s.oxy.x, s.oxy.y, s.oz, s.dxy.x, s.dxy.y, s.dz);
        if (hp.disc >= 0.0f) {
            const float t = intersect_post(hp, ta.eps);
            if (t < tmin || (t == tmin && (int)k < idx)) { tmin = t; idx = (int)k; }
        }
    };
    auto test = [&](uint32_t k) { ++n_tests; test_geom(geom[k], k); };
    uint32_t pos = ~0u;
    auto test_item = [&](const float4 g, uint32_t i) {
        const HitPre hp = intersect_pre(g.x, g.y, g.z, g.w, s.oxy.x, s.oxy.y, s.oz, s.dxy.x, s.dxy.y, s.dz);
        if (hp.disc >= 0.0f) {
            const float t = intersect_post(hp, ta.eps);
            if (t < tmin) { tmin = t; pos = i; }
            else if (t == tmin) {
                const int cur = (pos != ~0u) ? (int)items[pos] : idx;
                if ((int)items[i] < cur) pos = i;
            }
        }
    };
    auto test_large = [&](const float4 g, uint32_t k) {
        ++n_tests;
        const HitPre hp = intersect_pre(g.x, g.y, g.z, g.w, s.oxy.x, s.oxy.y, s.oz, s.dxy.x, s.dxy.y, s.dz);
        float q;
#if defined(__HIP_DEVICE_COMPILE__)
        float am = 1.0f;
        q = sqrt_rn_rsq1(hp.disc, am);
        if (__builtin_expect(__any(am < 0x1p-96f), 0)) {
            asm volatile("" ::: "memory");
            q = sqrtf(hp.disc);
        }
#else
        q = sqrtf(hp.disc);
#endif
        const float t = select_root(hp.b - q, hp.b + q, ta.eps);
        if (t < tmin || (t == tmin && (int)k < idx)) { tmin = t; idx = (int)k; }
    };
#if defined(__HIP_DEVICE_COMPILE__)
    if (grid_ok && h.off_cellslot) {
        typedef float f32x8 __attribute__((ext_vector_type(8)));
        typedef uint32_t u32x2 __attribute__((ext_vector_type(2)));
        const float *sg = reinterpret_cast<const float *>(grid + h.off_slots);
        const uint32_t *si = grid + h.off_slot_ids;
        for (uint32_t j = 0; j < h.slot_base; ++j) {
            f32x8 g8;
            u32x2 id2;
            asm volatile("s_load_dwordx8 %0, %2, 0x0\n\ts_load_dwordx2 %1, %3, 0x0\n\ts_waitcnt lgkmcnt(0)" : "=&s"(g8), "=&s"(id2) : "s"(sg + 8 * j), "s"(si + 2 * j) : "memory");
            test_large(make_float4(g8[0], g8[2], g8[4], g8[6]), id2[0]);
            if (id2[1] != kGridNoSphere) test_large(make_float4(g8[1], g8[3], g8[5], g8[7]), id2[1]);
        }
    } else
#endif
    if (grid_ok)
        for (uint32_t i = 0; i < h.nlarge; ++i) { const uint32_t k = large[i]; test_large(geom[k], k); }
    const float dd = s.dxy.x * s.dxy.x + s.dxy.y * s.dxy.y + s.dz * s.dz;
    const bool unit = fabsf(dd - 1.0f) <= 1e-3f;
    if (!grid_ok) {
        if (!fin)
            for (uint32_t k = 0; k < ns; ++k) { ++n_tests; test_geom(make_float4(cxp[k], cyp[k], czp[k], r2p[k]), k); }
    } else if (!fin && !unit) {
        for (uint32_t k = 0; k < ns; ++k) test(k);
    } else if (!fin) {
        grid_walk_cells(h, cells, item_geom, s.oxy.x, s.oxy.y, s.oz, s.dxy.x, s.dxy.y, s.dz, n_cells, n_tests, test_item, [&]() { return tmin; });
    }
    if (!fin) {
        if (pos != ~0u) idx = (int)items[pos];
        const uint32_t g = (idx < 0) ? ns - 1 : (uint32_t)idx;
        const float4 gc = grid_ok ? geom[g] : make_float4(cxp[g], cyp[g], czp[g], r2p[g]);
#if defined(__HIP_DEVICE_COMPILE__)
        {
            PathState n = s;
            float amin = 1.0f;
            shade_and_reflect<MODE, true>(n, tmin, gc.x, gc.y, gc.z, colx[g], coly[g], colz[g], idx == ta.light, &amin);
            if (__builtin_expect(__any(amin < 0x1p-96f), 0)) {
                asm volatile("" ::: "memory");
                n = s;
                shade_and_reflect<MODE>(n, tmin, gc.x, gc.y, gc.z, colx[g], coly[g], colz[g], idx == ta.light);
            }
            s = n;
        }
#else
        shade_and_reflect<MODE>(s, tmin, gc.x, gc.y, gc.z, colx[g], coly[g], colz[g], idx == ta.light);
#endif
    }
}

__device__ __forceinline__ bool grid_queue_usable(const TraceArgs &ta) {
    const GridHeader *h = reinterpret_cast<const GridHeader *>(ta.grid);
    return h && h->magic == kGridMagic && h->num_spheres == ta.ns && h->off_cellslot != 0 && eps_allows_rootkey(ta.eps);
}

__device__ __forceinline__ GridHeader load_grid_header(const uint32_t *grid) {
    static_assert(sizeof(GridHeader) == 128, "two s_load_dwordx16");
    GridHeader h;
#if defined(__HIP_DEVICE_COMPILE__)
    typedef uint32_t u32x16 __attribute__((ext_vector_type(16)));
    u32x16 w0, w1;
    asm volatile("s_load_dwordx16 %0, %2, 0x0\n\ts_load_dwordx16 %1, %2, 0x40\n\ts_waitcnt lgkmcnt(0)" : "=&s"(w0), "=&s"(w1) : "s"(grid) : "memory");
    uint32_t hw[32];
#pragma unroll
    for (int i = 0; i < 16; ++i) { hw[i] = w0[i]; hw[16 + i] = w1[i]; }
    __builtin_memcpy(&h, hw, sizeof h);
#else
    __builtin_memcpy(&h, grid, sizeof h);
#endif
    return h;
}

template <int MODE, bool RETIRE>
__device__ __forceinline__ uint32_t trace_grid(const float *__restrict__ sph, const uint32_t *__restrict__ grid,
                                               PathState &s, bool valid, const TraceArgs &ta, uint64_t path) {
    const GridHeader hdr = load_grid_header(grid);
    const GridCtx gc{&hdr, sph, grid, &ta};
    const uint64_t rr_key = ta.rr_start ? rr_path_key(ta.seed, path) : 0;
    uint32_t traced = 0, n_cells = 0, n_tests = 0;
    for (uint32_t d = 0; d < ta.depth; ++d) {
        const bool fin = !valid || (RETIRE && path_finished(s));
        if (RETIRE && __all(fin)) break;
        grid_segment<MODE>(gc, s, fin, n_cells, n_tests);
        if (!fin) {
            if (ta.rr_start && d + 1 >= ta.rr_start) russian_roulette(s, rr_key, d);
            ++traced;
        }
    }
    grid_stats(ta, n_cells, n_tests);
    return traced;
}

template <bool ONES = true>
__device__ __forceinline__ Tab8 load_scene8(const float *__restrict__ sph, Scene8 &sc, float4 *tab) {
#pragma unroll
    for (int k = 0; k < 8; ++k) {
        sc.r2[k] = sph[k]; sc.cx[k] = sph[8 + k]; sc.cy[k] = sph[16 + k]; sc.cz[k] = sph[24 + k];
    }
    if (threadIdx.x < 8) {
        const int k = threadIdx.x;
        tab[k] = make_float4(sph[8 + k], sph[16 + k], sph[24 + k], sph[k]);
        tab[8 + k] = make_float4(sph[56 + k], sph[64 + k], sph[72 + k], 0.0f);
    }
    if (ONES && threadIdx.x == 8) tab[16] = make_float4(1.0f, 1.0f, 1.0f, 0.0f);
    sc.planes = scene8_shares_planes(sc);
    __syncthreads();
    return Tab8{tab, tab + 8};
}

struct Gain3 { float r, g, b; };
__device__ __forceinline__ Gain3 load_gain(const float *__restrict__ sph, const TraceArgs &ta) {
    if (ta.emission) {
        const size_t ns = ta.ns, l = (size_t)ta.light;
        return Gain3{sph[4 * ns + l], sph[5 * ns + l], sph[6 * ns + l]};
    }
    return Gain3{ta.gain, ta.gain, ta.gain};
}

__device__ __forceinline__ void count_traced(const TraceArgs &ta, uint32_t traced) {
    if (ta.traced) {
        unsigned long long t = traced;
        for (int off = 32; off > 0; off >>= 1) t += __shfl_xor(t, off, 64);
        if ((threadIdx.x & 63) == 0 && t) atomicAdd(ta.traced, t);
    }
}


}
```

### ascendpathtracing_amd/csrc/pt_trace2.h

```cpp
#pragma once
#include <type_traits>

#include "pt_trace.h"

namespace {

struct PathPair {
    f2 ox, oy, oz, dx, dy, dz;
    f2 rx, ry, rz;
#ifdef APT_COUNT_PAIR_SKIP
    uint32_t hitA, hitB;
#endif
};

__device__ __forceinline__ PathState unpack_path(const PathPair &p, int which, uint64_t alive, bool first) {
    PathState s;
    if (which == 0) path_init(s, p.ox.x, p.oy.x, p.oz.x, p.dx.x, p.dy.x, p.dz.x);
    else path_init(s, p.ox.y, p.oy.y, p.oz.y, p.dx.y, p.dy.y, p.dz.y);
    if (first) return s;
    s.rxy = which == 0 ? f2{p.rx.x, p.ry.x} : f2{p.rx.y, p.ry.y};
    s.rz = which == 0 ? p.rz.x : p.rz.y;
    s.alive = select_const(alive, 1);
    return s;
}

template <int MODE>
struct ArgMin8 {
    uint32_t best;
    uint64_t b0 = 0, b1 = 0, b2 = 0, any = 0;
    __device__ __forceinline__ void update64(uint64_t keys, int k) {
        const uint32_t nb = min3_u32(best, (uint32_t)keys, (uint32_t)(keys >> 32));
        const uint64_t better = __builtin_amdgcn_ballot_w64(nb != best);
        best = nb;
        b0 = (k & 1) ? (b0 | better) : (b0 & ~better);
        b1 = (k & 2) ? (b1 | better) : (b1 & ~better);
        b2 = (k & 4) ? (b2 | better) : (b2 & ~better);
        if (MODE == kModeOracle) any |= better;
    }
    __device__ __forceinline__ Hit8 finish(const TraceArgs &ta, const KeyConsts &kc) {
        const float tmin = bits_f32(best + kc.bias);
        if (MODE == kModeOracle) { b0 |= ~any; b1 |= ~any; b2 |= ~any; }
        uint32_t addr;
        {
            const uint32_t a0 = select_const(b0, 16), a1 = select_const(b1, 32), a2 = select_const(b2, 64);
            asm("v_or3_b32 %0, %1, %2, %3" : "=v"(addr) : "v"(a0), "v"(a1), "v"(a2));
        }
        uint64_t light_mask = __builtin_amdgcn_ballot_w64(addr == (uint32_t)ta.light * 16u);
        if (MODE == kModeOracle) light_mask &= any;
        return Hit8{tmin, addr, light_mask};
    }
};

template <int HALF>
__device__ __forceinline__ f2 pair_half_minus(f2 cpair, f2 v) {
    f2 r;
    if (HALF == 0) asm("v_pk_add_f32 %0, %1, %2 op_sel:[0,0] op_sel_hi:[0,1] neg_lo:[0,1] neg_hi:[0,1]" : "=v"(r) : "s"(cpair), "v"(v));
    else asm("v_pk_add_f32 %0, %1, %2 op_sel:[1,0] op_sel_hi:[1,1] neg_lo:[0,1] neg_hi:[0,1]" : "=v"(r) : "s"(cpair), "v"(v));
    return r;
}
template <int HALF>
__device__ __forceinline__ f2 minus_pair_half(f2 v, f2 cpair) {
    f2 r;
    if (HALF == 0) asm("v_pk_add_f32 %0, %1, %2 op_sel:[0,0] op_sel_hi:[1,0] neg_lo:[0,1] neg_hi:[0,1]" : "=v"(r) : "v"(v), "s"(cpair));
    else asm("v_pk_add_f32 %0, %1, %2 op_sel:[0,1] op_sel_hi:[1,1] neg_lo:[0,1] neg_hi:[0,1]" : "=v"(r) : "v"(v), "s"(cpair));
    return r;
}

constexpr int kAbSkip = 0xC0;

template <int MODE, int SKIP>
__device__ __forceinline__ void intersect2_ns8_planes(const Scene8 &sc, const PathPair &s, const TraceArgs &ta, const KeyConsts &kc,
                                                      float &aminA, float &aminB, Hit8 &hA, Hit8 &hB) {
    struct Term { f2 p, q; };
    auto term = [](auto half, f2 cpair, f2 o, f2 d) __attribute__((always_inline)) {
        const f2 t = pair_half_minus<decltype(half)::value>(cpair, o);
        return Term{t * d, t * t};
    };
    struct Pre { f2 b, c, disc; };
    auto pre = [](const Term &x, const Term &y, const Term &z, auto half, f2 r2pair) __attribute__((always_inline)) {
        Pre h;
        h.b = (x.p + y.p) + z.p;
        h.c = minus_pair_half<decltype(half)::value>((x.q + y.q) + z.q, r2pair);
        h.disc = h.b * h.b - h.c;
        return h;
    };
    ArgMin8<MODE> A, B;
    A.best = kc.init; B.best = kc.init;
    auto stage = [&](const Pre &h, int k) __attribute__((always_inline)) {
        const f2 q = sqrt_rn_rsq1_pair(h.disc);
        A.update64(root_pair<0>(h.b, q) + kc.nbias2, k);
        B.update64(root_pair<1>(h.b, q) + kc.nbias2, k);
    };
    auto walls = [&](const Pre &h0, const Pre &h1, int k) __attribute__((always_inline)) {
        aminA = minimum3_abs(aminA, h0.disc.x, h1.disc.x);
        aminB = minimum3_abs(aminB, h0.disc.y, h1.disc.y);
        stage(h0, k);
        stage(h1, k + 1);
    };
    auto tested = [&](const Pre &h, int k) __attribute__((always_inline)) {
        if ((SKIP >> k) & 1) {
            const float mA = __builtin_amdgcn_fmed3f(h.disc.x, h.b.x, -h.c.x), mB = __builtin_amdgcn_fmed3f(h.disc.y, h.b.y, -h.c.y);
            uint32_t run = any_lane(__builtin_amdgcn_ballot_w64(__builtin_fmaxf(mA, mB) >= -kBehindGuard));
            asm("" : "+s"(run));
            if (run == 0u) return;
        }
        aminA = minimum3_abs(aminA, h.disc.x, h.disc.x);
        aminB = minimum3_abs(aminB, h.disc.y, h.disc.y);
        stage(h, k);
    };
    static_assert((SKIP & 0x3F) == 0, "the walls have no test: the room lies inside their spheres");
    const f2 X1 = {sc.cx[0], sc.cx[1]}, X2 = {sc.cx[2], sc.cx[6]}, Y1 = {sc.cy[4], sc.cy[5]}, Y2 = {sc.cy[6], sc.cy[7]}, Y3 = {sc.cy[0], sc.cy[0]};
    const f2 Z1 = {sc.cz[2], sc.cz[3]}, Z2 = {sc.cz[0], sc.cz[6]};
    const f2 R0 = {sc.r2[0], sc.r2[1]}, R1 = {sc.r2[2], sc.r2[3]}, R2 = {sc.r2[4], sc.r2[5]}, R3 = {sc.r2[6], sc.r2[7]};
    using Lo = std::integral_constant<int, 0>;
    using Hi = std::integral_constant<int, 1>;
    const Term x2 = term(Lo{}, X2, s.ox, s.dx), y0 = term(Lo{}, Y3, s.oy, s.dy), z0 = term(Lo{}, Z2, s.oz, s.dz);
    walls(pre(term(Lo{}, X1, s.ox, s.dx), y0, z0, Lo{}, R0), pre(term(Hi{}, X1, s.ox, s.dx), y0, z0, Hi{}, R0), 0);
    walls(pre(x2, y0, term(Lo{}, Z1, s.oz, s.dz), Lo{}, R1), pre(x2, y0, term(Hi{}, Z1, s.oz, s.dz), Hi{}, R1), 2);
    walls(pre(x2, term(Lo{}, Y1, s.oy, s.dy), z0, Lo{}, R2), pre(x2, term(Hi{}, Y1, s.oy, s.dy), z0, Hi{}, R2), 4);
    tested(pre(term(Hi{}, X2, s.ox, s.dx), term(Lo{}, Y2, s.oy, s.dy), term(Hi{}, Z2, s.oz, s.dz), Lo{}, R3), 6);
    tested(pre(x2, term(Hi{}, Y2, s.oy, s.dy), z0, Hi{}, R3), 7);
    hA = A.finish(ta, kc);
    hB = B.finish(ta, kc);
}

template <int MODE, bool PLANES, bool FIRST>
__device__ __forceinline__ void bounce2_ns8_t(const Scene8 &sc, const Tab8 tab, const PathPair &s, PathPair &n,
                                              const TraceArgs &ta, const KeyConsts &kc, uint32_t ones_off,
                                              uint64_t &aliveA, uint64_t &aliveB, uint64_t &redoA, uint64_t &redoB) {
    float aminA = 1.0f, aminB = 1.0f;
    Hit8 hA, hB;
    if (PLANES) {
        intersect2_ns8_planes<MODE, kAbSkip>(sc, s, ta, kc, aminA, aminB, hA, hB);
    } else {
        hA = intersect_ns8_v2<MODE>(sc, s.ox.x, s.oy.x, s.oz.x, s.dx.x, s.dy.x, s.dz.x, ta, kc, aminA);
        hB = intersect_ns8_v2<MODE>(sc, s.ox.y, s.oy.y, s.oz.y, s.dx.y, s.dy.y, s.dz.y, ta, kc, aminB);
    }
    if (FIRST) {
        aliveA = ~hA.light;
        aliveB = ~hB.light;
    } else {
        aliveA &= ~hA.light;
        aliveB &= ~hB.light;
    }
    const char *geo = reinterpret_cast<const char *>(tab.geo);
    uint32_t cA, cB;
    asm("v_cndmask_b32_e64 %0, %1, %2, %3" : "=v"(cA) : "v"(ones_off), "v"(hA.addr), "s"(aliveA));
    asm("v_cndmask_b32_e64 %0, %1, %2, %3" : "=v"(cB) : "v"(ones_off), "v"(hB.addr), "s"(aliveB));
    const uint32_t gA = (uint32_t)(uintptr_t)geo + hA.addr, gB = (uint32_t)(uintptr_t)geo + hB.addr;
    const uint32_t aA = (uint32_t)(uintptr_t)geo + cA, aB = (uint32_t)(uintptr_t)geo + cB;
    float cxA, cyA, czA, cxB, cyB, czB, axA, ayA, azA, axB, ayB, azB;
    asm volatile("ds_read_b32 %0, %12\n ds_read_b32 %1, %12 offset:4\n ds_read_b32 %2, %12 offset:8\n"
                 "ds_read_b32 %3, %13\n ds_read_b32 %4, %13 offset:4\n ds_read_b32 %5, %13 offset:8\n"
                 "ds_read_b32 %6, %14 offset:128\n ds_read_b32 %7, %14 offset:132\n ds_read_b32 %8, %14 offset:136\n"
                 "ds_read_b32 %9, %15 offset:128\n ds_read_b32 %10, %15 offset:132\n ds_read_b32 %11, %15 offset:136\n"
                 "s_waitcnt lgkmcnt(0)"
                 : "=&v"(cxA), "=&v"(cyA), "=&v"(czA), "=&v"(cxB), "=&v"(cyB), "=&v"(czB), "=&v"(axA), "=&v"(ayA), "=&v"(azA),
                   "=&v"(axB), "=&v"(ayB), "=&v"(azB)
                 : "v"(gA), "v"(gB), "v"(aA), "v"(aB)
                 : "memory");
    const f2 cx = {cxA, cxB}, cy = {cyA, cyB}, cz = {czA, czB};
    const f2 ax = {axA, axB}, ay = {ayA, ayB}, az = {azA, azB};
    const f2 t = {hA.tmin, hB.tmin};
    const f2 hx = s.ox + s.dx * t, hy = s.oy + s.dy * t, hz = s.oz + s.dz * t;
    const f2 nx = hx - cx, ny = hy - cy, nz = hz - cz;
    f2 len2;
    if (MODE == kModeOracle) {
        const f2 p0 = nx * nx, p1 = ny * ny, p2 = nz * nz;
        len2 = f2{sum3_f64(p0.x, p1.x, p2.x), sum3_f64(p0.y, p1.y, p2.y)};
    } else {
        len2 = nx * nx + ny * ny;
        len2 = len2 + nz * nz;
    }
    const f2 r0 = {__builtin_amdgcn_rsqf(len2.x), __builtin_amdgcn_rsqf(len2.y)};
    aminA = minimum3_abs_after_trans(aminA, r0.x, nx.x);
    aminA = minimum3_abs(aminA, ny.x, nz.x);
    aminB = minimum3_abs_after_trans(aminB, r0.y, nx.y);
    aminB = minimum3_abs(aminB, ny.y, nz.y);
    const f2 L = sqrt_rsq_step(len2, r0);
    f2 ux, uy, uz, e1;
    div3_seeded_packed2(nx, ny, nz, L, r0, ux, uy, uz, e1);
    f2 dot;
    if (MODE == kModeOracle) {
        const f2 p0 = s.dx * ux, p1 = s.dy * uy, p2 = s.dz * uz;
        dot = f2{sum3_f64(p0.x, p1.x, p2.x), sum3_f64(p0.y, p1.y, p2.y)};
    } else {
        dot = s.dx * ux;
        dot = dot + s.dy * uy;
        dot = dot + s.dz * uz;
    }
    const f2 k2 = twice_canonical(dot);
    n.dx = s.dx - ux * k2; n.dy = s.dy - uy * k2; n.dz = s.dz - uz * k2;
    n.ox = hx; n.oy = hy; n.oz = hz;
    if (FIRST) { n.rx = ax; n.ry = ay; n.rz = az; }
    else { n.rx = ax * s.rx; n.ry = ay * s.ry; n.rz = az * s.rz; }
    redoA = __builtin_amdgcn_ballot_w64(!(aminA >= kFastMin)) | __builtin_amdgcn_ballot_w64(e1.x == kDiv3SeededStuck);
    redoB = __builtin_amdgcn_ballot_w64(!(aminB >= kFastMin)) | __builtin_amdgcn_ballot_w64(e1.y == kDiv3SeededStuck);
#ifdef APT_COUNT_PAIR_SKIP
    n.hitA = hA.addr; n.hitB = hB.addr;
#endif
}
template <int MODE, bool PLANES>
__device__ __forceinline__ void bounce2_ns8(const Scene8 &sc, const Tab8 tab, const PathPair &s, PathPair &n,
                                            const TraceArgs &ta, const KeyConsts &kc, uint32_t ones_off,
                                            uint64_t &aliveA, uint64_t &aliveB, uint64_t &redoA, uint64_t &redoB) {
    bounce2_ns8_t<MODE, PLANES, false>(sc, tab, s, n, ta, kc, ones_off, aliveA, aliveB, redoA, redoB);
}
template <int MODE, bool PLANES>
__device__ __forceinline__ void bounce2_ns8_first(const Scene8 &sc, const Tab8 tab, const PathPair &s, PathPair &n,
                                                  const TraceArgs &ta, const KeyConsts &kc, uint32_t ones_off,
                                                  uint64_t &aliveA, uint64_t &aliveB, uint64_t &redoA, uint64_t &redoB) {
    bounce2_ns8_t<MODE, PLANES, true>(sc, tab, s, n, ta, kc, ones_off, aliveA, aliveB, redoA, redoB);
}

template <int MODE, bool PLANES, bool FIRST = false>
__device__ __forceinline__ void bounce2_ns8_last(const Scene8 &sc, const Tab8 tab, const PathPair &s, f2 &rx, f2 &ry, f2 &rz,
                                                 const TraceArgs &ta, const KeyConsts &kc, uint32_t ones_off,
                                                 uint64_t &aliveA, uint64_t &aliveB, uint64_t &redoA, uint64_t &redoB) {
    float aminA = 1.0f, aminB = 1.0f;
    Hit8 hA, hB;
    if (PLANES) {
        intersect2_ns8_planes<MODE, kAbSkip>(sc, s, ta, kc, aminA, aminB, hA, hB);
    } else {
        hA = intersect_ns8_v2<MODE>(sc, s.ox.x, s.oy.x, s.oz.x, s.dx.x, s.dy.x, s.dz.x, ta, kc, aminA);
        hB = intersect_ns8_v2<MODE>(sc, s.ox.y, s.oy.y, s.oz.y, s.dx.y, s.dy.y, s.dz.y, ta, kc, aminB);
    }
    if (FIRST) {
        aliveA = ~hA.light;
        aliveB = ~hB.light;
    } else {
        aliveA &= ~hA.light;
        aliveB &= ~hB.light;
    }
    uint32_t cA, cB;
    asm("v_cndmask_b32_e64 %0, %1, %2, %3" : "=v"(cA) : "v"(ones_off), "v"(hA.addr), "s"(aliveA));
    asm("v_cndmask_b32_e64 %0, %1, %2, %3" : "=v"(cB) : "v"(ones_off), "v"(hB.addr), "s"(aliveB));
    const char *geo = reinterpret_cast<const char *>(tab.geo);
    const uint32_t aA = (uint32_t)(uintptr_t)geo + cA, aB = (uint32_t)(uintptr_t)geo + cB;
    float axA, ayA, azA, axB, ayB, azB;
    asm volatile("ds_read_b32 %0, %6 offset:128\n ds_read_b32 %1, %6 offset:132\n ds_read_b32 %2, %6 offset:136\n"
                 "ds_read_b32 %3, %7 offset:128\n ds_read_b32 %4, %7 offset:132\n ds_read_b32 %5, %7 offset:136\n"
                 "s_waitcnt lgkmcnt(0)"
                 : "=&v"(axA), "=&v"(ayA), "=&v"(azA), "=&v"(axB), "=&v"(ayB), "=&v"(azB)
                 : "v"(aA), "v"(aB)
                 : "memory");
    if (FIRST) { rx = f2{axA, axB}; ry = f2{ayA, ayB}; rz = f2{azA, azB}; }
    else { rx = f2{axA, axB} * s.rx; ry = f2{ayA, ayB} * s.ry; rz = f2{azA, azB} * s.rz; }
    redoA = __builtin_amdgcn_ballot_w64(!(aminA >= kFastMin));
    redoB = __builtin_amdgcn_ballot_w64(!(aminB >= kFastMin));
}

template <int MODE, bool PLANES>
__device__ __forceinline__ void trace2_ns8_t(const Scene8 &sc, const Tab8 tab, PathPair &s, const TraceArgs &ta) {
    const KeyConsts kc = make_key_consts(ta.eps);
    uint32_t ones_off = 8 * 16;
    asm volatile("" : "+v"(ones_off));
    uint64_t aliveA = __builtin_amdgcn_ballot_w64(true), aliveB = aliveA;
    const bool fast_ok = eps_allows_rootkey(ta.eps);
    auto redo_stands = [&](const PathPair &in, uint64_t redoA, uint64_t redoB, bool first) __attribute__((always_inline)) {
        if (first) return (redoA | redoB) != 0;
        const bool finA = select_const(aliveA, 1) == 0 || (in.rx.x == 0.0f && in.ry.x == 0.0f && in.rz.x == 0.0f);
        const bool finB = select_const(aliveB, 1) == 0 || (in.rx.y == 0.0f && in.ry.y == 0.0f && in.rz.y == 0.0f);
        return __builtin_amdgcn_ballot_w64((select_const(redoA, 1) != 0 && !finA) || (select_const(redoB, 1) != 0 && !finB)) != 0;
    };
    auto exact_pair = [&](const PathPair &in, PathState &na, PathState &nb, bool first) __attribute__((always_inline)) {
        PathState a = unpack_path(in, 0, aliveA, first), b = unpack_path(in, 1, aliveB, first);
        bounce_ns8_exact<MODE>(sc, tab, a, na, ta);
        bounce_ns8_exact<MODE>(sc, tab, b, nb, ta);
        if (ta.traced && (threadIdx.x & 63) == 0) atomicAdd(ta.traced + 3, 1ull);
    };
#ifdef APT_COUNT_PAIR_SKIP
    uint32_t count_bounce = 0;
    auto count_pairs = [&](const PathPair &in) __attribute__((always_inline)) {
        if (!ta.traced) return;
        const bool lane0 = (threadIdx.x & 63) == 0;
        for (int half = 0; half < 2; ++half) {
            const float ox = half ? in.ox.y : in.ox.x, oy = half ? in.oy.y : in.oy.x, oz = half ? in.oz.y : in.oz.x;
            const float dx = half ? in.dx.y : in.dx.x, dy = half ? in.dy.y : in.dy.x, dz = half ? in.dz.y : in.dz.x;
            HitPre2 hp[4];
            f2 c67 = {0.0f, 0.0f};
            if (PLANES) intersect_pre_planes<true>(sc, ox, oy, oz, dx, dy, dz, hp, &c67);
            for (int k = 0; k < 8; k += 2) {
                const HitPre2 h = PLANES ? hp[k / 2]
                                         : intersect_pre2(f2{sc.cx[k], sc.cx[k + 1]}, f2{sc.cy[k], sc.cy[k + 1]}, f2{sc.cz[k], sc.cz[k + 1]},
                                                          f2{sc.r2[k], sc.r2[k + 1]}, ox, oy, oz, dx, dy, dz);
                const uint32_t slot = 4u + (uint32_t)(half * 8 + (count_bounce < 7u ? count_bounce : 7u)) * 4u + (uint32_t)(k / 2);
                if (pair_misses_wave(h.disc) && lane0) atomicAdd(ta.traced + slot, 1ull);
                if (PLANES && k == 6) {
                    const uint32_t s67 = 72u + (uint32_t)(half * 8 + (count_bounce < 7u ? count_bounce : 7u)) * 4u;
                    const bool u6 = sphere_reachable_mask(h.disc.x, h.b.x, c67.x) == 0, u7 = sphere_reachable_mask(h.disc.y, h.b.y, c67.y) == 0;
                    const bool r6 = h.disc.x >= 0.0f && !(h.b.x < 0.0f && c67.x > 0.0f), r7 = h.disc.y >= 0.0f && !(h.b.y < 0.0f && c67.y > 0.0f);
                    const bool plain = __builtin_amdgcn_ballot_w64(r6 || r7) == 0;
                    if (u6 && lane0) atomicAdd(ta.traced + s67, 1ull);
                    if (u7 && lane0) atomicAdd(ta.traced + s67 + 1, 1ull);
                    if (u6 && u7 && lane0) atomicAdd(ta.traced + s67 + 2, 1ull);
                    if (plain && lane0) atomicAdd(ta.traced + s67 + 3, 1ull);
                }
            }
        }
        if (PLANES) {
            const uint32_t bb = count_bounce < 7u ? count_bounce : 7u;
            auto bcd = [&](int k, float ox, float oy, float oz, float dx, float dy, float dz, float &b, float &c, float &disc) {
                const float x = sc.cx[k] - ox, y = sc.cy[k] - oy, z = sc.cz[k] - oz;
                b = x * dx; b = b + y * dy; b = b + z * dz;
                c = x * x; c = c + y * y; c = c + z * z; c = c - sc.r2[k];
                disc = b * b; disc = disc - c;
            };
            bool strict[8], relaxed[8];
            for (int k = 0; k < 8; ++k) {
                float bA, cA, dA, bB, cB, dB;
                bcd(k, in.ox.x, in.oy.x, in.oz.x, in.dx.x, in.dy.x, in.dz.x, bA, cA, dA);
                bcd(k, in.ox.y, in.oy.y, in.oz.y, in.dx.y, in.dy.y, in.dz.y, bB, cB, dB);
                const bool behindA = bA < -kBehindGuard, behindB = bB < -kBehindGuard;
                const bool reach_s = __builtin_amdgcn_fmed3f(dA, bA, -cA) >= -kBehindGuard || __builtin_amdgcn_fmed3f(dB, bB, -cB) >= -kBehindGuard;
                const bool reach_r = (dA >= 0.0f && !(behindA && cA >= 0.0f)) || (dB >= 0.0f && !(behindB && cB >= 0.0f));
                const bool reach_ns = !(behindA && cA > kBehindGuard && behindB && cB > kBehindGuard);
                const bool reach_nr = !(behindA && cA >= 0.0f && behindB && cB >= 0.0f);
                strict[k] = __builtin_amdgcn_ballot_w64(reach_s) == 0;
                relaxed[k] = __builtin_amdgcn_ballot_w64(reach_r) == 0;
                if (strict[k] && lane0) atomicAdd(ta.traced + 136u + bb * 8u + (uint32_t)k, 1ull);
                if (relaxed[k] && lane0) atomicAdd(ta.traced + 200u + bb * 8u + (uint32_t)k, 1ull);
                if (__builtin_amdgcn_ballot_w64(reach_ns) == 0 && lane0) atomicAdd(ta.traced + 264u + bb * 8u + (uint32_t)k, 1ull);
                if (__builtin_amdgcn_ballot_w64(reach_nr) == 0 && lane0) atomicAdd(ta.traced + 328u + bb * 8u + (uint32_t)k, 1ull);
            }
            if (count_bounce > 0) {
                const uint32_t w = (uint32_t)__builtin_amdgcn_readfirstlane((int)in.hitA);
                if (w < 6u * 16u && __builtin_amdgcn_ballot_w64(in.hitA != w || in.hitB != w) == 0) {
                    const uint32_t k = w / 16u;
                    bool s = false, r = false, opp = false;
                    for (uint32_t j = 0; j < 6; ++j) {
                        if (j == k) { s = strict[j]; r = relaxed[j]; }
                        if (j == (k ^ 1u)) opp = strict[j];
                    }
                    if (lane0) {
                        atomicAdd(ta.traced + 392u + bb * 4u, 1ull);
                        if (s) atomicAdd(ta.traced + 393u + bb * 4u, 1ull);
                        if (r) atomicAdd(ta.traced + 394u + bb * 4u, 1ull);
                        if (opp) atomicAdd(ta.traced + 395u + bb * 4u, 1ull);
                    }
                }
            }
        }
        if (count_bounce == 0 && lane0) atomicAdd(ta.traced + 68, 1ull);
        ++count_bounce;
    };
#endif
    auto step = [&](const PathPair &in, PathPair &out, auto first_tag) __attribute__((always_inline)) {
        constexpr bool first = decltype(first_tag)::value;
#ifdef APT_COUNT_PAIR_SKIP
        count_pairs(in);
#endif
        uint64_t oa = aliveA, ob = aliveB;
        bool redo_any = !fast_ok;
        if (__builtin_expect(fast_ok, 1)) {
            uint64_t redoA, redoB;
            bounce2_ns8_t<MODE, PLANES, first>(sc, tab, in, out, ta, kc, ones_off, oa, ob, redoA, redoB);
            if (__builtin_expect((redoA | redoB) != 0, 0)) redo_any = redo_stands(in, redoA, redoB, first);
        }
        if (__builtin_expect(redo_any, 0)) {
            PathState na, nb;
            exact_pair(in, na, nb, first);
            out.ox = f2{na.oxy.x, nb.oxy.x}; out.oy = f2{na.oxy.y, nb.oxy.y}; out.oz = f2{na.oz, nb.oz};
            out.dx = f2{na.dxy.x, nb.dxy.x}; out.dy = f2{na.dxy.y, nb.dxy.y}; out.dz = f2{na.dz, nb.dz};
            out.rx = f2{na.rxy.x, nb.rxy.x}; out.ry = f2{na.rxy.y, nb.rxy.y}; out.rz = f2{na.rz, nb.rz};
            oa = __builtin_amdgcn_ballot_w64(na.alive != 0);
            ob = __builtin_amdgcn_ballot_w64(nb.alive != 0);
#ifdef APT_COUNT_PAIR_SKIP
            out.hitA = ~0u; out.hitB = ~0u;
#endif
        }
        aliveA = oa; aliveB = ob;
    };
    auto last = [&](const PathPair &in, auto first_tag) __attribute__((always_inline)) {
        constexpr bool first = decltype(first_tag)::value;
#ifdef APT_COUNT_PAIR_SKIP
        count_pairs(in);
#endif
        uint64_t oa = aliveA, ob = aliveB;
        f2 rx, ry, rz;
        bool redo_any = !fast_ok;
        if (__builtin_expect(fast_ok, 1)) {
            uint64_t redoA, redoB;
            bounce2_ns8_last<MODE, PLANES, first>(sc, tab, in, rx, ry, rz, ta, kc, ones_off, oa, ob, redoA, redoB);
            if (__builtin_expect((redoA | redoB) != 0, 0)) redo_any = redo_stands(in, redoA, redoB, first);
        }
        if (__builtin_expect(redo_any, 0)) {
            PathState na, nb;
            exact_pair(in, na, nb, first);
            rx = f2{na.rxy.x, nb.rxy.x}; ry = f2{na.rxy.y, nb.rxy.y}; rz = f2{na.rz, nb.rz};
        }
        s.rx = rx; s.ry = ry; s.rz = rz;
    };
    using Yes = std::true_type;
    using No = std::false_type;
    if (ta.depth == 0) {
        const f2 one = {1.0f, 1.0f};
        s.rx = one; s.ry = one; s.rz = one;
        return;
    }
    if (ta.depth == 1) {
        last(s, Yes{});
        return;
    }
    const uint32_t full = ta.depth - 1;
    PathPair n;
    step(s, n, Yes{});
    uint32_t d = 1;
    for (; d + 2 <= full; d += 2) {
        step(n, s, No{});
        step(s, n, No{});
    }
    if (d < full) {
        step(n, s, No{});
        last(s, No{});
    } else {
        last(n, No{});
    }
}

template <int MODE>
__device__ __forceinline__ void trace2_ns8(const Scene8 &sc, const Tab8 tab, PathPair &s, const TraceArgs &ta, bool planes) {
    if (planes) {
        Scene8 p = sc;
        p.cx[3] = p.cx[4] = p.cx[5] = p.cx[7] = sc.cx[2];
        p.cy[1] = p.cy[2] = p.cy[3] = sc.cy[0];
        p.cz[1] = p.cz[4] = p.cz[5] = p.cz[7] = sc.cz[0];
        trace2_ns8_t<MODE, true>(p, tab, s, ta);
    } else {
        trace2_ns8_t<MODE, false>(sc, tab, s, ta);
    }
}

}
```

### ascendpathtracing_amd/csrc/render_kernels.hip

```cpp
#include <hip/hip_runtime.h>
#include <algorithm>
#include <new>
#include <stdint.h>
#include <stdio.h>
#include <stdlib.h>
#include <string.h>
#include <string>
#include <type_traits>
#include <vector>

#include "../../include/render_mi355x.h"
#include "apt_host.h"
#include "apt_materials.h"
#include "hip_own.h"
#include "pt_core.h"
#include "pt_dispatch.h"

#include "pt_kernels.h"
#include "pt_grid_build.h"

namespace {

using apt::clear_error;
int fail(int code, const char *fmt, const char *detail = "") { return apt::set_error(code, fmt, detail); }
int hip_fail(hipError_t e) { return fail(APT_ERR_DEVICE, "HIP: %s", hipGetErrorString(e)); }
#define HIP_TRY(call) do { if (hipError_t e_ = (call); e_ != hipSuccess) return hip_fail(e_); } while (0)
int launched() { HIP_TRY(hipGetLastError()); return APT_OK; }


int no_leaf_plan() { return fail(APT_ERR_ARG, "samples too large: its pairwise-sum plan needs more than 64 leaves (every count <= 7688 fits, and 8192)%s"); }
int make_leaf_prog(uint32_t samples, LeafProg &lp) { return make_leaf_plan(samples, lp) ? APT_OK : no_leaf_plan(); }

int one_launch(uint64_t blocks, const char *msg, unsigned *grid = nullptr) {
    if (blocks > 0x7fffffffull) return fail(APT_ERR_ARG, msg);
    if (grid) *grid = (unsigned)blocks;
    return APT_OK;
}

enum class Reads { All, Materials, Features };
int check_params(const apt_render_params *p, Reads reads = Reads::All) {
    if (!p) return fail(APT_ERR_ARG, "params is null%s");
    if (p->struct_size != sizeof(apt_render_params)) return fail(APT_ERR_STRUCT, "apt_render_params.struct_size mismatch%s");
    if (!p->width || !p->height || !p->samples) return fail(APT_ERR_ARG, "width/height/samples must be non-zero%s");
    if (reads != Reads::Features && p->mode > APT_MODE_ORACLE) return fail(APT_ERR_ARG, "unknown mode%s");
    if (p->num_spheres == 0) return fail(APT_ERR_SCENE, "num_spheres is 0%s");
    if (reads == Reads::Features) return APT_OK;
    if (p->light_index >= (int32_t)p->num_spheres) return fail(APT_ERR_SCENE, "light_index out of range%s");
    if (reads == Reads::All && (p->flags & APT_FLAG_EMISSION) && p->light_index < 0) return fail(APT_ERR_SCENE, "APT_FLAG_EMISSION needs a light_index >= 0%s");
    return APT_OK;
}

int check_materials(const apt_render_params *p, const uint32_t *materials, bool lights = false) {
    if (!materials) return fail(APT_ERR_ARG, "materials must be non-null%s");
    if (p->mode != APT_MODE_KERNEL) return fail(APT_ERR_ARG, "materials need APT_MODE_KERNEL (O-mode restates test_soa, which has none)%s");
    if (p->accel && !(p->flags & APT_FLAG_GRID_SLOTS)) return fail(APT_ERR_ARG, "materials: accel (grid) needs APT_FLAG_GRID_SLOTS (apt_grid_flags of the built grid)%s");
    if (!lights && (p->flags & APT_FLAG_NEE) && p->light_index < 0) return fail(APT_ERR_SCENE, "APT_FLAG_NEE samples the sphere light_index: it needs a light_index >= 0%s");
    return APT_OK;
}

int refuse_camera(const apt_context::Values &cv, const char *entry) {
    if (cv.has_env) return fail(APT_ERR_ARG, "%s: the context has an environment set (apt_context_set_environment), which the mirror frame entries do not take: unset it, or use the material entries", entry);
    return cv.has_camera ? fail(APT_ERR_ARG, "%s: the context has a camera set (apt_context_set_camera), which the mirror frame entries do not take: unset it, or use apt_gen_rays_camera_device + render_do_ex + apt_decode_color_device", entry) : APT_OK;
}

struct MatArgs {
    const uint32_t *materials = nullptr;
    bool with_lights = false;
    const void *lights = nullptr;
    apt::MatFilm film = apt::MatFilm::None;
    bool list = false;
};
int check_mat_args(const apt_render_params *p, const MatArgs &m) {
    int rc = check_materials(p, m.materials, m.with_lights);
    if (rc) return rc;
    if (m.with_lights && !m.lights) return fail(APT_ERR_ARG, "lights must be non-null (a device light table: apt_build_lights_host)%s");
    return APT_OK;
}
int check_lights_status(const MatArgs &m, const uint32_t *status) {
    if (m.with_lights && !status) return fail(APT_ERR_DEVICE, "lights: the context has no device status word here (its first launch on this device is inside a stream capture, or the device index is beyond its table)%s");
    return APT_OK;
}

uint32_t *status_word(apt_context &ctx, hipStream_t st) {
    int dev = 0;
    if (hipGetDevice(&dev) != hipSuccess) { (void)hipGetLastError(); return nullptr; }
    if (dev < 0 || dev >= apt::kMaxStatusDevices) return nullptr;
    if (uint32_t *w = ctx.status_lookup(dev)) return w;
    hipStreamCaptureStatus cs = hipStreamCaptureStatusNone;
    if (hipStreamIsCapturing(st, &cs) != hipSuccess) { (void)hipGetLastError(); return nullptr; }
    if (cs != hipStreamCaptureStatusNone) return nullptr;
    apt::DeviceBuffer<uint32_t> fresh;
    if (fresh.alloc(1) != hipSuccess || hipMemset(fresh.get(), 0, sizeof(uint32_t)) != hipSuccess) { (void)hipGetLastError(); return nullptr; }
    uint32_t *spare = nullptr;
    uint32_t *w = ctx.status_adopt(dev, fresh.release(), &spare);
    apt::DeviceBuffer<uint32_t> loser(spare);
    return w;
}

struct Launch { apt_context::Values cv; uint32_t *status; };
Launch launch_state(apt_context &ctx, void *stream) { return Launch{ctx.snapshot(), status_word(ctx, (hipStream_t)stream)}; }

TraceArgs make_trace_args(const apt_render_params *p, const Launch &ls) {
    const apt_context::Values &cv = ls.cv;
    TraceArgs ta;
    ta.ns = p->num_spheres; ta.depth = p->depth; ta.light = p->light_index;
    ta.eps = p->eps; ta.gain = p->gain; ta.traced = cv.trace_counter;
    ta.status = ls.status;
    ta.refill_lanes = cv.refill_lanes;
    ta.grid = (p->num_spheres != 8) ? reinterpret_cast<const uint32_t *>((uintptr_t)p->accel) : nullptr;
    ta.grid_walk = 0;
    ta.emission = (p->flags & APT_FLAG_EMISSION) ? 1u : 0u;
    ta.rr_start = (p->flags & APT_FLAG_RR) ? (p->rr_start ? p->rr_start : 3u) : 0u;
    ta.seed = p->seed;
    return ta;
}

apt::MatTrace make_mat_trace(const apt_render_params *p, const Launch &ls, const MatArgs &m) {
    const TraceArgs ta = make_trace_args(p, ls);
    const uint32_t *lights = m.with_lights ? static_cast<const uint32_t *>(m.lights) : nullptr;
    const bool nee = !lights && (p->flags & APT_FLAG_NEE) != 0, gloss = (p->flags & APT_FLAG_GLOSS) != 0;
    return apt::MatTrace{ta.ns, ta.depth, ta.rr_start, ta.light, nee, ta.eps, ta.seed, ta.status ? ta.grid : nullptr, ta.status, ta.traced, lights,
                         gloss, (p->flags & APT_FLAG_MIS) != 0 && gloss && (nee || lights)};
}

struct PathRange {
    uint64_t n_image, b, c;
    bool band;
    unsigned grid = 0;
    uint64_t plane() const { return band ? c : n_image; }
    template <class T> T *base(T *buf) const { return band ? buf - b : buf; }
};
int path_range(const apt_render_params *p, PathRange &r) {
    r.n_image = (uint64_t)p->width * p->height * 4u * p->samples;
    r.b = p->path_begin;
    if (r.b > r.n_image) return fail(APT_ERR_ARG, "path_begin beyond the image%s");
    r.c = p->path_count ? p->path_count : r.n_image - r.b;
    if (r.b + r.c > r.n_image) return fail(APT_ERR_ARG, "path range beyond the image%s");
    r.band = p->flags & APT_FLAG_BAND_BUFFERS;
    return APT_OK;
}
int pixel_range(const apt_render_params *p, uint64_t pixel_begin, uint64_t pixel_count) {
    const uint64_t npix = (uint64_t)p->width * p->height;
    return (pixel_begin > npix || pixel_count > npix - pixel_begin) ? fail(APT_ERR_ARG, "pixel range beyond the image%s") : APT_OK;
}

int pixel_list(const apt_render_params *p, uint64_t list_address, uint64_t list_count) {
    const uint64_t npix = (uint64_t)p->width * p->height;
    if (list_address == 0 || (list_address & 3u)) return fail(APT_ERR_ARG, "pixel list: pixel_begin must carry a non-null, 4-byte aligned device address%s");
    if (list_count > npix) return fail(APT_ERR_ARG, "pixel list: more entries than the image has pixels%s");
    return npix > (1ull << 32) ? fail(APT_ERR_ARG, "pixel list: an image of more than 2^32 pixels has no 32-bit pixel indices%s") : APT_OK;
}

FrameArgs make_frame_args(const apt_render_params *p, uint64_t pixel_begin, uint64_t pixel_count, float *fb, uint8_t *fb_u8) {
    FrameArgs fa;
    camera_init(fa.cam, p->width, p->height);
    fa.width = p->width; fa.height = p->height; fa.samples = p->samples; fa.seed = p->seed;
    fa.pixel_begin = pixel_begin; fa.pixel_count = pixel_count; fa.fb = fb; fa.fb_u8 = fb_u8;
    return fa;
}

size_t sphere_table_bytes(uint32_t num_spheres) { return ((size_t)num_spheres * 10 + 127) / 128 * 128 * sizeof(float); }

constexpr uint64_t kTwoPathBufferMin = 1ull << 20;

int paths_launch_range(const apt_render_params *p, bool pointers, PathRange &r, const char *which = "rays/spheres/colors must be non-null%s") {
    if (!pointers) return fail(APT_ERR_ARG, which);
    if (int rc = path_range(p, r); rc || r.c == 0) return rc;
    return one_launch((r.c + kBlock - 1) / kBlock, "path_count too large for one launch; shard it%s", &r.grid);
}

int frame_launch_shape(const apt_render_params *p, bool pointers, uint64_t pixel_begin, uint64_t pixel_count, FrameShape &fs, bool list = false) {
    if (!pointers) return fail(APT_ERR_ARG, "spheres/fb must be non-null%s");
    if (int rc = list ? pixel_list(p, pixel_begin, pixel_count) : pixel_range(p, pixel_begin, pixel_count)) return rc;
    fs = FrameShape{};
    if (pixel_count == 0) return APT_OK;
    if (!frame_shape(p->samples, pixel_count, fs)) return no_leaf_plan();
    return one_launch(fs.blocks, "pixel_count too large for one launch; shard it%s");
}

int do_render_paths(const Launch &ls, const apt_render_params *p, void *stream, const float *rays,
                    const float *spheres, float *colors) {
    int rc = check_params(p);
    if (rc) return rc;
    PathRange r;
    if ((rc = paths_launch_range(p, rays && spheres && colors, r)) || r.c == 0) return rc;
    const uint64_t n = r.plane(), b = r.b, c = r.c;
    hipStream_t st = (hipStream_t)stream;
    const bool ns8 = p->num_spheres == 8;
    const TraceArgs ta = make_trace_args(p, ls);
    const bool retire = p->flags & APT_FLAG_RETIRE;
    const dim3 grid(r.grid);
    rays = r.base(rays);
    colors = r.base(colors);
    with_mode(p->mode, [&](auto m) {
        if (ns8 && !retire && ta.rr_start == 0 && c >= kTwoPathBufferMin) {
            const uint64_t per_block = 2ull * kBlock * kPaths2Pairs;
            const dim3 grid2((unsigned)((c + per_block - 1) / per_block));
            hipLaunchKernelGGL((render_paths2_kernel<m>), grid2, dim3(kBlock), 0, st, rays, spheres, colors, n, b, c, ta);
        } else if (ns8 && retire) {
            const uint64_t waves = (c + kQueueChunk - 1) / kQueueChunk;
            const dim3 qgrid((unsigned)((waves + kBlock / 64 - 1) / (kBlock / 64)));
            hipLaunchKernelGGL((render_paths_queue_kernel<m>), qgrid, dim3(kBlock), 0, st, rays, spheres, colors, n, b, c, ta);
        } else if (ns8) {
            hipLaunchKernelGGL((render_paths_kernel<m, kScene8, false>), grid, dim3(kBlock), 0, st, rays, spheres, colors, n, b, c, ta);
        } else {
            with_flag(ta.grid != nullptr, [&](auto gr) { with_flag(retire, [&](auto rt) {
                hipLaunchKernelGGL((render_paths_kernel<m, gr ? kSceneGrid : kSceneTiles, rt>), grid, dim3(kBlock), 0, st, rays, spheres, colors, n, b, c, ta);
            }); });
        }
    });
    return launched();
}

struct QueueShape { QueueArgs qa; unsigned waves; size_t lds; };
int queue_launch_shape(const apt::Debug &dbg, const LeafProg &lp, bool rr, bool grid, uint64_t pixel_count, bool retire, QueueShape &q) {
    QueueArgs &qa = q.qa;
    const uint32_t subs = queue_unit_subs(grid), unit_items = subs * lp.maxleaf, window = subs == 4u ? 512u : 384u;
    qa.nbuf = dbg.queue_nbuf ? dbg.queue_nbuf : std::max(2u, std::min(16u, (window + unit_items - 1u) / unit_items));
    qa.buf_bytes = queue_buf_bytes(lp.maxleaf, subs);
    qa.retire = retire ? 1u : 0u;
    const uint64_t ppw = dbg.queue_ppw ? dbg.queue_ppw : std::max<uint64_t>(4, std::min<uint64_t>(16, pixel_count / 8192u));
    qa.ppw = (uint32_t)ppw;
    q.lds = queue_lds_bytes(queue_pool_entries(grid), rr, qa.nbuf, lp.nleaves > 1, qa.buf_bytes, subs) + dbg.queue_lds_pad;
    return one_launch((pixel_count + ppw - 1) / ppw, "pixel_count too large for one launch; shard it%s", &q.waves);
}

int do_render_frame(const Launch &ls, const apt_render_params *p, void *stream, const float *spheres,
                    uint64_t pixel_begin, uint64_t pixel_count, float *fb, uint8_t *fb_u8) {
    int rc = check_params(p);
    if (rc) return rc;
    FrameShape fs;
    if ((rc = frame_launch_shape(p, spheres && fb, pixel_begin, pixel_count, fs)) || fs.blocks == 0) return rc;
    const LeafProg &lp = fs.lp;
    const int group = fs.group;
    const apt::Debug &dbg = ls.cv.debug;
    if ((rc = refuse_camera(ls.cv, "render_frame"))) return rc;
    hipStream_t st = (hipStream_t)stream;
    const bool ns8 = p->num_spheres == 8;
    TraceArgs ta = make_trace_args(p, ls);
    const FrameArgs fa = make_frame_args(p, pixel_begin, pixel_count, fb, fb_u8);
    const bool retire = p->flags & APT_FLAG_RETIRE, rrk = ta.rr_start != 0;
    if (retire && ns8 && group == 8 && p->depth > 0) {
        QueueShape q;
        if ((rc = queue_launch_shape(dbg, lp, rrk, false, pixel_count, true, q))) return rc;
        with_mode(p->mode, [&](auto m) { with_flag(rrk, [&](auto rr) {
            hipLaunchKernelGGL((render_frame_queue8_kernel<m, rr>), dim3(q.waves), dim3(64), q.lds, st, spheres, fa, ta, lp, q.qa);
        }); });
        return launched();
    }
    if (!ns8 && ta.grid && group == 8 && p->depth > 0 && dbg.grid_walk != 1u) {
        QueueShape q;
        if ((rc = queue_launch_shape(dbg, lp, rrk, true, pixel_count, retire, q))) return rc;
        const bool vouched = (p->flags & APT_FLAG_GRID_SLOTS) && eps_allows_rootkey(p->eps) && ta.status != nullptr;
        TraceArgs ta_q = ta;
        ta_q.grid_walk = vouched ? 3u : 0u;
        with_mode(p->mode, [&](auto m) { with_flag(rrk, [&](auto rr) { with_flag(ta.traced != nullptr, [&](auto stats) {
            hipLaunchKernelGGL((render_frame_queue8_kernel<m, rr, kSceneGrid, stats>), dim3(q.waves), dim3(64), q.lds, st, spheres, fa, ta_q, lp, q.qa);
        }); }); });
        if ((rc = launched()) || vouched) return rc;
        ta.grid_walk = 2;
    }
    size_t lds = fs.lds;
    if (retire && !ns8 && !ta.grid && group == 8) lds += (size_t)(kBlock / 64) * 3 * 8 * lp.maxleaf * sizeof(float);
    const dim3 grid((unsigned)fs.blocks);
    with_mode(p->mode, [&](auto m) {
        if (ns8 && group == 8) {
            if (!retire && !rrk && p->samples >= 16)
                hipLaunchKernelGGL((render_frame_kernel<m, kScene8, 8, false, true>), grid, dim3(kBlock), lds, st, spheres, fa, ta, lp);
            else
                hipLaunchKernelGGL((render_frame_kernel<m, kScene8, 8, false>), grid, dim3(kBlock), lds, st, spheres, fa, ta, lp);
        } else if (ns8) {
            with_flag(retire, [&](auto rt) {
                hipLaunchKernelGGL((render_frame_kernel<m, kScene8, 1, rt>), grid, dim3(kBlock), lds, st, spheres, fa, ta, lp);
            });
        } else {
            with_flag(ta.grid != nullptr, [&](auto gr) { with_flag(group == 8, [&](auto g8) { with_flag(retire, [&](auto rt) {
                hipLaunchKernelGGL((render_frame_kernel<m, gr ? kSceneGrid : kSceneTiles, g8 ? 8 : 1, rt>), grid, dim3(kBlock), lds, st, spheres, fa, ta, lp);
            }); }); });
        }
    });
    return launched();
}

void split_range(uint64_t total, uint64_t r, uint64_t parts, uint64_t &begin, uint64_t &count) {
    const uint64_t base = total / parts, extra = total % parts;
    begin = r * base + (r < extra ? r : extra);
    count = base + (r < extra ? 1 : 0);
}

int do_mat_paths(apt_context *ctx, const apt_render_params *p, void *stream, const float *rays, const float *spheres, const MatArgs &ma,
                 float *colors) {
    clear_error();
    if (!ctx) return fail(APT_ERR_ARG, "context is null%s");
    int rc = check_params(p, Reads::Materials);
    if (rc || (rc = check_mat_args(p, ma))) return rc;
    const Launch ls = launch_state(*ctx, stream);
    PathRange r;
    if ((rc = paths_launch_range(p, rays && spheres && colors, r)) || r.c == 0) return rc;
    if ((rc = check_lights_status(ma, ls.status))) return rc;
    apt::mat_render_paths(apt::MatPathsCall{make_mat_trace(p, ls, ma), r.base(rays), spheres, ma.materials, r.base(colors), r.plane(), r.b, r.c,
                                            stream, ls.cv.has_env ? &ls.cv.env : nullptr});
    return launched();
}
int do_mat_frame(apt_context *ctx, const apt_render_params *p, void *stream, const float *spheres, const MatArgs &ma, uint64_t pixel_begin,
                 uint64_t pixel_count, float *fb, uint8_t *fb_u8) {
    clear_error();
    if (!ctx) return fail(APT_ERR_ARG, "context is null%s");
    int rc = check_params(p, Reads::Materials);
    if (rc || (rc = check_mat_args(p, ma))) return rc;
    const Launch ls = launch_state(*ctx, stream);
    const bool film = ma.film != apt::MatFilm::None;
    FrameShape fs;
    if ((rc = frame_launch_shape(p, spheres && (fb || film), pixel_begin, pixel_count, fs, ma.list)) || fs.blocks == 0) return rc;
    if ((rc = check_lights_status(ma, ls.status))) return rc;
    if ((ls.cv.has_camera || ls.cv.has_env || film) && !apt::mat_camera_fits(p->samples)) return fail(APT_ERR_ARG, "camera / environment: a frame with a camera or an environment set takes a pairwise-sum plan of at most 44 leaves (every samples <= 4199 has one)%s");
    if ((rc = apt::mat_render_frame(apt::MatFrameCall{make_mat_trace(p, ls, ma), spheres, ma.materials, p->width, p->height, p->samples,
                                                      ma.list ? 0 : pixel_begin, pixel_count, fb, fb_u8, stream,
                                                      ls.cv.has_camera ? &ls.cv.camera : nullptr, ls.cv.has_env ? &ls.cv.env : nullptr, ma.film,
                                                      ma.list ? reinterpret_cast<const uint32_t *>((uintptr_t)pixel_begin) : nullptr})))
        return rc;
    return launched();
}

int do_features(apt_context *ctx, const apt_render_params *p, void *stream, const float *spheres, uint64_t pixel_begin, uint64_t pixel_count,
                float *features) {
    clear_error();
    if (!ctx) return fail(APT_ERR_ARG, "context is null%s");
    int rc = check_params(p, Reads::Features);
    if (rc) return rc;
    if (p->accel && !(p->flags & APT_FLAG_GRID_SLOTS)) return fail(APT_ERR_ARG, "features: accel (grid) needs APT_FLAG_GRID_SLOTS (apt_grid_flags of the built grid)%s");
    const Launch ls = launch_state(*ctx, stream);
    FrameShape fs;
    if ((rc = frame_launch_shape(p, spheres != nullptr, pixel_begin, pixel_count, fs)) || fs.blocks == 0) return rc;
    if (!apt::mat_camera_fits(p->samples)) return fail(APT_ERR_ARG, "features: the frame takes a pairwise-sum plan of at most 44 leaves, as a film's does (every samples <= 4199 has one)%s");
    const uint32_t *grid = (p->num_spheres != 8 && ls.status) ? reinterpret_cast<const uint32_t *>((uintptr_t)p->accel) : nullptr;
    if ((rc = apt::mat_render_features(apt::FeaturesCall{spheres, p->num_spheres, p->eps, p->seed, grid, ls.status, p->width, p->height, p->samples,
                                                         pixel_begin, pixel_count, features, stream, ls.cv.has_camera ? &ls.cv.camera : nullptr})))
        return rc;
    return launched();
}

}

struct apt_multi {
    struct Band {
        int device = 0;
        apt::Stream stream;
        apt::Event start, stop;
        apt::DeviceBuffer<float> sph;
        apt::DeviceBuffer<float> fb;
        apt::DeviceBuffer<uint8_t> u8;
    };
    std::vector<Band> bands;
    apt_render_params params;
    uint32_t stripes = 1;
    uint64_t max_stripe = 0;
    int root = 0;
    hipError_t add_band(int device, const float *spheres_host, size_t sph_bytes) {
        hipError_t e = hipSetDevice(device);
        if (e != hipSuccess) return e;
        Band &bd = bands.emplace_back();
        bd.device = device;
        int can = 0;
        if (device != root && hipDeviceCanAccessPeer(&can, device, root) == hipSuccess && can && hipDeviceEnablePeerAccess(root, 0) != hipSuccess) (void)hipGetLastError();
        if ((e = bd.stream.create(hipStreamNonBlocking)) != hipSuccess) return e;
        if ((e = bd.start.create()) != hipSuccess || (e = bd.stop.create()) != hipSuccess) return e;
        if ((e = bd.sph.alloc(sph_bytes / sizeof(float))) != hipSuccess) return e;
        if ((e = hipMemcpy(bd.sph.get(), spheres_host, sph_bytes, hipMemcpyHostToDevice)) != hipSuccess) return e;
        if ((e = bd.fb.alloc((size_t)stripes * 3 * max_stripe)) != hipSuccess) return e;
        return bd.u8.alloc((size_t)stripes * 3 * max_stripe);
    }
    ~apt_multi() {
        apt::DeviceScope to_root(root);
        for (; !bands.empty(); bands.pop_back()) (void)hipSetDevice(bands.back().device);
    }
};

extern "C" {

int apt_abi_version(void) { return APT_ABI_VERSION; }

int apt_device_count(void) {
    int n = 0;
    if (hipGetDeviceCount(&n) != hipSuccess) { (void)hipGetLastError(); return 0; }
    return n;
}

apt_context *apt_context_create(void) { clear_error(); return new (std::nothrow) apt_context(); }
void apt_context_destroy(apt_context *ctx) {
    clear_error();
    if (!ctx) return;
    uint32_t *words[apt::kMaxStatusDevices];
    ctx->status_release(words);
    {
        apt::DeviceScope back;
        for (int d = 0; d < apt::kMaxStatusDevices; ++d)
            if (words[d] && hipSetDevice(d) == hipSuccess) { apt::DeviceBuffer<uint32_t> freed(words[d]); }
    }
    (void)hipGetLastError();
    delete ctx;
}

int apt_context_set_debug(apt_context *ctx, const char *key, double value) {
    clear_error();
    if (!ctx) return fail(APT_ERR_ARG, "context is null%s");
    return ctx->set_debug(key, value);
}

int apt_context_get_debug(apt_context *ctx, const char *key, double *value) {
    clear_error();
    if (!ctx || !value) return fail(APT_ERR_ARG, "context/value is null%s");
    return ctx->get_debug(key, value);
}

int apt_context_check(apt_context *ctx, void *stream) {
    clear_error();
    if (!ctx) return fail(APT_ERR_ARG, "context is null%s");
    HIP_TRY(hipStreamSynchronize((hipStream_t)stream));
    uint32_t *w = status_word(*ctx, (hipStream_t)stream);
    if (!w) return APT_OK;
    uint32_t bits = 0;
    HIP_TRY(hipMemcpy(&bits, w, sizeof bits, hipMemcpyDeviceToHost));
    if (!bits) return APT_OK;
    if (hipMemset(w, 0, sizeof bits) != hipSuccess) (void)hipGetLastError();
    std::string what;
    if (bits & APT_DEV_QUEUE_GUARD) what += " queue-loop-bound";
    if (bits & APT_DEV_GRID_TURNS) what += " grid-walk-bound";
    if (bits & APT_DEV_LDS_BASE) what += " lds-base";
    if (bits & APT_DEV_GRID_MISMATCH) what += " grid-mismatch";
    if (bits & APT_DEV_BAD_MATERIAL) what += " bad-material";
    if (bits & APT_DEV_LIGHTS_MISMATCH) what += " lights-mismatch";
    if (bits & APT_DEV_LIST_RANGE) what += " list-range";
    if (bits & ~(uint32_t)(APT_DEV_QUEUE_GUARD | APT_DEV_GRID_TURNS | APT_DEV_LDS_BASE | APT_DEV_GRID_MISMATCH | APT_DEV_BAD_MATERIAL | APT_DEV_LIGHTS_MISMATCH | APT_DEV_LIST_RANGE)) what += " unknown-bits";
    return fail(APT_ERR_DEVICE, "a kernel reported a failure through the device status word:%s (the frame it wrote is incomplete)", what.c_str());
}

int apt_context_set_params(apt_context *ctx, const apt_render_params *p) {
    clear_error();
    if (!ctx) return fail(APT_ERR_ARG, "context is null%s");
    int rc = check_params(p);
    if (rc) return rc;
    ctx->set_params(*p);
    return APT_OK;
}

int apt_context_set_trace_counter(apt_context *ctx, uint64_t *device_counter) {
    clear_error();
    if (!ctx) return fail(APT_ERR_ARG, "context is null%s");
    ctx->set_trace_counter((unsigned long long *)device_counter);
    return APT_OK;
}

int apt_context_set_refill_lanes(apt_context *ctx, uint32_t lanes) {
    clear_error();
    if (!ctx) return fail(APT_ERR_ARG, "context is null%s");
    if (lanes < 1 || lanes > 64) return fail(APT_ERR_ARG, "refill lanes: 1..64%s");
    ctx->set_refill_lanes(lanes);
    return APT_OK;
}

void apt_context_render_do(apt_context *ctx, uint32_t blockDim, void *l2ctrl, void *stream, uint8_t *rays,
                           uint8_t *spheres, uint8_t *colors) {
    clear_error();
    (void)blockDim;
    (void)l2ctrl;
    if (!ctx) { (void)fail(APT_ERR_ARG, "context is null%s"); return; }
    const Launch ls = launch_state(*ctx, stream);
    (void)do_render_paths(ls, &ls.cv.params, stream, (const float *)rays, (const float *)spheres, (float *)colors);
}

int apt_context_render_do_ex(apt_context *ctx, const apt_render_params *p, void *stream, const float *rays,
                             const float *spheres, float *colors) {
    clear_error();
    if (!ctx) return fail(APT_ERR_ARG, "context is null%s");
    return do_render_paths(launch_state(*ctx, stream), p, stream, rays, spheres, colors);
}

int apt_context_render_frame(apt_context *ctx, const apt_render_params *p, void *stream, const float *spheres,
                             uint64_t pixel_begin, uint64_t pixel_count, float *fb, uint8_t *fb_u8) {
    clear_error();
    if (!ctx) return fail(APT_ERR_ARG, "context is null%s");
    return do_render_frame(launch_state(*ctx, stream), p, stream, spheres, pixel_begin, pixel_count, fb, fb_u8);
}

int apt_context_render_frame_materials(apt_context *ctx, const apt_render_params *p, void *stream, const float *spheres,
                                       const uint32_t *materials, uint64_t pixel_begin, uint64_t pixel_count, float *fb, uint8_t *fb_u8) {
    return do_mat_frame(ctx, p, stream, spheres, MatArgs{materials}, pixel_begin, pixel_count, fb, fb_u8);
}

int apt_context_render_paths_materials(apt_context *ctx, const apt_render_params *p, void *stream, const float *rays,
                                       const float *spheres, const uint32_t *materials, float *colors) {
    return do_mat_paths(ctx, p, stream, rays, spheres, MatArgs{materials}, colors);
}

int apt_render_frame_materials(const apt_render_params *p, void *stream, const float *spheres, const uint32_t *materials,
                               uint64_t pixel_begin, uint64_t pixel_count, float *fb, uint8_t *fb_u8) {
    return apt_context_render_frame_materials(&apt::default_context(), p, stream, spheres, materials, pixel_begin, pixel_count, fb, fb_u8);
}

int apt_render_paths_materials(const apt_render_params *p, void *stream, const float *rays, const float *spheres,
                               const uint32_t *materials, float *colors) {
    return apt_context_render_paths_materials(&apt::default_context(), p, stream, rays, spheres, materials, colors);
}

int apt_context_render_frame_lights(apt_context *ctx, const apt_render_params *p, void *stream, const float *spheres,
                                    const uint32_t *materials, const void *lights, uint64_t pixel_begin, uint64_t pixel_count, float *fb,
                                    uint8_t *fb_u8) {
    return do_mat_frame(ctx, p, stream, spheres, MatArgs{materials, true, lights}, pixel_begin, pixel_count, fb, fb_u8);
}

int apt_context_render_paths_lights(apt_context *ctx, const apt_render_params *p, void *stream, const float *rays, const float *spheres,
                                    const uint32_t *materials, const void *lights, float *colors) {
    return do_mat_paths(ctx, p, stream, rays, spheres, MatArgs{materials, true, lights}, colors);
}

int apt_context_render_frame_film(apt_context *ctx, const apt_render_params *p, void *stream, const float *spheres,
                                  const uint32_t *materials, const void *lights, uint64_t pixel_begin, uint64_t pixel_count, float *film,
                                  uint32_t pass) {
    const bool list = p && p->struct_size == sizeof(apt_render_params) && (p->flags & APT_FLAG_PIXEL_LIST) != 0;
    const MatArgs ma{materials, lights != nullptr, lights, pass && !list ? apt::MatFilm::Add : apt::MatFilm::Store, list};
    apt_render_params q;
    if (p && p->struct_size == sizeof q) {
        q = *p;
        q.seed = apt_film_pass_seed(p->seed, pass);
        p = &q;
    }
    return do_mat_frame(ctx, p, stream, spheres, ma, pixel_begin, pixel_count, film, nullptr);
}

int apt_render_frame_film(const apt_render_params *p, void *stream, const float *spheres, const uint32_t *materials, const void *lights,
                          uint64_t pixel_begin, uint64_t pixel_count, float *film, uint32_t pass) {
    return apt_context_render_frame_film(&apt::default_context(), p, stream, spheres, materials, lights, pixel_begin, pixel_count, film, pass);
}

int apt_context_render_frame_features(apt_context *ctx, const apt_render_params *p, void *stream, const float *spheres, uint64_t pixel_begin,
                                      uint64_t pixel_count, float *features) {
    return do_features(ctx, p, stream, spheres, pixel_begin, pixel_count, features);
}

int apt_render_frame_features(const apt_render_params *p, void *stream, const float *spheres, uint64_t pixel_begin, uint64_t pixel_count,
                              float *features) {
    return do_features(&apt::default_context(), p, stream, spheres, pixel_begin, pixel_count, features);
}

int apt_film_resolve_device(const apt_film_resolve *r, void *stream, const float *film, uint64_t pixel_count, const float *table_dev,
                            float *out, uint8_t *u8) {
    clear_error();
    int rc = apt::film_resolve_check(r, film, table_dev, out, u8, "apt_film_resolve_device");
    if (rc || pixel_count == 0) return rc;
    if ((rc = one_launch((pixel_count + kBlock - 1) / kBlock, "pixel_count too large for one launch; shard it%s"))) return rc;
    apt::film_resolve(*r, stream, film, pixel_count, table_dev, out, u8);
    return launched();
}

int apt_render_frame_lights(const apt_render_params *p, void *stream, const float *spheres, const uint32_t *materials, const void *lights,
                            uint64_t pixel_begin, uint64_t pixel_count, float *fb, uint8_t *fb_u8) {
    return apt_context_render_frame_lights(&apt::default_context(), p, stream, spheres, materials, lights, pixel_begin, pixel_count, fb, fb_u8);
}

int apt_render_paths_lights(const apt_render_params *p, void *stream, const float *rays, const float *spheres, const uint32_t *materials,
                            const void *lights, float *colors) {
    return apt_context_render_paths_lights(&apt::default_context(), p, stream, rays, spheres, materials, lights, colors);
}

int apt_set_default_params(const apt_render_params *p) { return apt_context_set_params(&apt::default_context(), p); }
int apt_set_refill_lanes(uint32_t lanes) { return apt_context_set_refill_lanes(&apt::default_context(), lanes); }
int apt_set_trace_counter(uint64_t *device_counter) { return apt_context_set_trace_counter(&apt::default_context(), device_counter); }
int apt_set_debug(const char *key, double value) { return apt_context_set_debug(&apt::default_context(), key, value); }
int apt_get_debug(const char *key, double *value) { return apt_context_get_debug(&apt::default_context(), key, value); }
int apt_check(void *stream) { return apt_context_check(&apt::default_context(), stream); }

int render_do_ex(const apt_render_params *p, void *stream, const float *rays, const float *spheres, float *colors) {
    return apt_context_render_do_ex(&apt::default_context(), p, stream, rays, spheres, colors);
}

void render_do(uint32_t blockDim, void *l2ctrl, void *stream, uint8_t *rays, uint8_t *spheres, uint8_t *colors) {
    apt_context_render_do(&apt::default_context(), blockDim, l2ctrl, stream, rays, spheres, colors);
}

void apt_render_do(uint32_t blockDim, void *l2ctrl, void *stream, uint8_t *rays, uint8_t *spheres, uint8_t *colors) {
    apt_context_render_do(&apt::default_context(), blockDim, l2ctrl, stream, rays, spheres, colors);
}

int render_frame(const apt_render_params *p, void *stream, const float *spheres, uint64_t pixel_begin,
                 uint64_t pixel_count, float *fb, uint8_t *fb_u8) {
    return apt_context_render_frame(&apt::default_context(), p, stream, spheres, pixel_begin, pixel_count, fb, fb_u8);
}

int apt_render_host(uint32_t blockDim, const uint8_t *rays, const uint8_t *spheres, uint8_t *colors) {
    clear_error();
    if (!rays || !spheres || !colors) return fail(APT_ERR_ARG, "rays/spheres/colors must be non-null%s");
    const Launch ls = launch_state(apt::default_context(), nullptr);
    const apt_render_params &p = ls.cv.params;
    const size_t n = (size_t)p.width * p.height * 4u * p.samples;
    if (p.path_begin != 0 || (p.path_count != 0 && p.path_count != n)) return fail(APT_ERR_ARG, "apt_render_host: the default parameters carry a path sub-range; it renders whole frames only%s");
    const size_t sph_bytes = sphere_table_bytes(p.num_spheres);
    apt::DeviceBuffer<float> d_rays, d_sph, d_col;
    HIP_TRY(d_rays.alloc(n * 6)); HIP_TRY(d_sph.alloc(sph_bytes / sizeof(float))); HIP_TRY(d_col.alloc(n * 3));
    HIP_TRY(hipMemcpy(d_rays.get(), rays, n * 24, hipMemcpyHostToDevice));
    HIP_TRY(hipMemcpy(d_sph.get(), spheres, sph_bytes, hipMemcpyHostToDevice));
    (void)blockDim;
    if (int rc = do_render_paths(ls, &p, nullptr, d_rays.get(), d_sph.get(), d_col.get())) return rc;
    HIP_TRY(hipMemcpy(colors, d_col.get(), n * 12, hipMemcpyDeviceToHost));
    return apt_context_check(&apt::default_context(), nullptr);
}

void apt_multi_destroy(apt_multi *m) { clear_error(); delete m; }

int apt_multi_create(const int *device_ids, uint32_t num_bands, uint32_t stripes, const apt_render_params *p,
                     const float *spheres_host, apt_multi **out) {
    clear_error();
    if (!device_ids || !num_bands || !stripes || !spheres_host || !out) return fail(APT_ERR_ARG, "apt_multi_create: bad arguments%s");
    int rc = check_params(p);
    if (rc) return rc;
    if (p->accel) return fail(APT_ERR_ARG, "apt_multi_create: accel is a single-device address; not supported here%s");
    if ((rc = refuse_camera(apt::default_context().snapshot(), "apt_multi_create"))) return rc;
    const int ndev = apt_device_count();
    for (uint32_t b = 0; b < num_bands; ++b)
        if (device_ids[b] < 0 || device_ids[b] >= ndev) return fail(APT_ERR_DEVICE, "apt_multi_create: device id out of range%s");
    const uint64_t npix = (uint64_t)p->width * p->height, parts = (uint64_t)num_bands * stripes;
    if (parts > npix) return fail(APT_ERR_ARG, "apt_multi_create: more stripes than pixels%s");
    apt_multi *m = new (std::nothrow) apt_multi();
    if (!m) return fail(APT_ERR_DEVICE, "out of host memory%s");
    m->params = *p; m->stripes = stripes; m->root = device_ids[0];
    uint64_t b0, c0;
    split_range(npix, 0, parts, b0, c0);
    m->max_stripe = c0;
    m->bands.reserve(num_bands);
    const size_t sph_bytes = sphere_table_bytes(p->num_spheres);
    hipError_t e = hipSuccess;
    {
        apt::DeviceScope to_root(m->root);
        for (uint32_t b = 0; b < num_bands && e == hipSuccess; ++b) e = m->add_band(device_ids[b], spheres_host, sph_bytes);
    }
    if (e != hipSuccess) { delete m; return fail(APT_ERR_DEVICE, "apt_multi_create: HIP: %s", hipGetErrorString(e)); }
    *out = m;
    return APT_OK;
}

int apt_multi_render(apt_multi *m, float *fb_root, uint8_t *u8_root, float *band_kernel_ms) {
    clear_error();
    if (!m || !fb_root) return fail(APT_ERR_ARG, "apt_multi_render: handle/fb must be non-null%s");
    if (int crc = refuse_camera(apt::default_context().snapshot(), "apt_multi_render")) return crc;
    const uint64_t npix = (uint64_t)m->params.width * m->params.height;
    const uint64_t nb = m->bands.size(), parts = nb * m->stripes;
    int rc = APT_OK;
    hipError_t e = hipSuccess;
    apt::DeviceScope to_root(m->root);
    for (uint64_t b = 0; b < nb && rc == APT_OK && e == hipSuccess; ++b) {
        apt_multi::Band &bd = m->bands[b];
        e = hipSetDevice(bd.device);
        if (e != hipSuccess) break;
        Launch ls = launch_state(apt::default_context(), bd.stream.get());
        if (bd.device != m->root) ls.cv.trace_counter = nullptr;
        e = hipEventRecord(bd.start.get(), bd.stream.get());
        for (uint32_t s = 0; s < m->stripes && rc == APT_OK && e == hipSuccess; ++s) {
            uint64_t begin, count;
            split_range(npix, (uint64_t)s * nb + b, parts, begin, count);
            float *fb = bd.fb.get() + (size_t)s * 3 * m->max_stripe;
            uint8_t *u8 = bd.u8.get() + (size_t)s * 3 * m->max_stripe;
            rc = do_render_frame(ls, &m->params, bd.stream.get(), bd.sph.get(), begin, count, fb, u8_root ? u8 : nullptr);
            if (rc != APT_OK) break;
            if (s + 1 == m->stripes) e = hipEventRecord(bd.stop.get(), bd.stream.get());
        }
        for (uint32_t s = 0; s < m->stripes && rc == APT_OK && e == hipSuccess; ++s) {
            uint64_t begin, count;
            split_range(npix, (uint64_t)s * nb + b, parts, begin, count);
            const float *fb = bd.fb.get() + (size_t)s * 3 * m->max_stripe;
            const uint8_t *u8 = bd.u8.get() + (size_t)s * 3 * m->max_stripe;
            for (int ch = 0; ch < 3 && e == hipSuccess; ++ch)
                e = hipMemcpyPeerAsync(fb_root + (size_t)ch * npix + begin, m->root, fb + (size_t)ch * count, bd.device,
                                       count * sizeof(float), bd.stream.get());
            if (u8_root && e == hipSuccess)
                e = hipMemcpyPeerAsync(u8_root + begin * 3, m->root, u8, bd.device, count * 3, bd.stream.get());
        }
    }
    for (auto &bd : m->bands)
        if (hipSetDevice(bd.device) == hipSuccess) { hipError_t se = hipStreamSynchronize(bd.stream.get()); if (e == hipSuccess) e = se; }
    if (band_kernel_ms && rc == APT_OK && e == hipSuccess)
        for (uint64_t b = 0; b < nb; ++b) {
            (void)hipSetDevice(m->bands[b].device);
            if (hipEventElapsedTime(&band_kernel_ms[b], m->bands[b].start.get(), m->bands[b].stop.get()) != hipSuccess) band_kernel_ms[b] = -1.0f;
        }
    int dev_rc = APT_OK;
    std::string dev_msg;
    if (rc == APT_OK && e == hipSuccess)
        for (auto &bd : m->bands)
            if (hipSetDevice(bd.device) == hipSuccess && apt_context_check(&apt::default_context(), bd.stream.get()) != APT_OK && dev_rc == APT_OK) {
                dev_rc = apt_last_status();
                dev_msg = apt_last_error();
            }
    if (rc != APT_OK) return rc;
    if (e != hipSuccess) return hip_fail(e);
    return dev_rc == APT_OK ? APT_OK : fail(dev_rc, "apt_multi_render: %s", dev_msg.c_str());
}

int apt_build_grid_device(const float *spheres_dev, uint32_t ns, void *stream, void *grid_dev, size_t capacity,
                          size_t *out_bytes) {
    clear_error();
    if (!spheres_dev || ns == 0 || !out_bytes) return fail(APT_ERR_ARG, "apt_build_grid_device: spheres/out_bytes must be non-null, num_spheres non-zero%s");
    hipStream_t st = (hipStream_t)stream;
    apt::DeviceBuffer<float> rad;
    apt::DeviceBuffer<uint32_t> large, small, count, cursor, sums, long_count;
    apt::DeviceBuffer<uint2> long_cells;
    apt::DeviceBuffer<GridBuildStats> stats_d;
    HIP_TRY(rad.alloc(ns)); HIP_TRY(large.alloc(ns)); HIP_TRY(small.alloc(ns)); HIP_TRY(stats_d.alloc(1));
    hipLaunchKernelGGL(grid_classify_kernel, dim3(1), dim3(kGB), 0, st, spheres_dev, ns, rad.get(), large.get(), small.get(), stats_d.get());
    GridBuildStats stt;
    HIP_TRY(hipMemcpyAsync(&stt, stats_d.get(), sizeof stt, hipMemcpyDeviceToHost, st));
    HIP_TRY(hipStreamSynchronize(st));
    GridHeader h;
    grid_header_from_stats(ns, stt.nsmall, stt.nlarge, stt.lo, stt.hi, stt.scale, apt::grid_spheres_per_cell(), h);
    const uint64_t nc1 = (uint64_t)h.ncells + 1, nblk = (nc1 + kGB - 1) / kGB;
    HIP_TRY(count.alloc(nc1)); HIP_TRY(cursor.alloc(h.ncells)); HIP_TRY(sums.alloc(nblk));
    HIP_TRY(hipMemsetAsync(count.get(), 0, nc1 * 4, st)); HIP_TRY(hipMemsetAsync(cursor.get(), 0, (size_t)h.ncells * 4, st));
    if (stt.nsmall) hipLaunchKernelGGL(grid_count_kernel, dim3((stt.nsmall + 255) / 256), dim3(256), 0, st, h, spheres_dev, rad.get(), small.get(), stt.nsmall, count.get());
    hipLaunchKernelGGL(scan_blocks_kernel, dim3((unsigned)nblk), dim3(kGB), 0, st, count.get(), nc1, sums.get());
    hipLaunchKernelGGL(scan_sums_kernel, dim3(1), dim3(kGB), 0, st, sums.get(), (uint32_t)nblk);
    hipLaunchKernelGGL(scan_add_kernel, dim3((unsigned)nblk), dim3(kGB), 0, st, count.get(), nc1, sums.get());
    uint32_t nitems = 0;
    HIP_TRY(hipMemcpyAsync(&nitems, count.get() + h.ncells, 4, hipMemcpyDeviceToHost, st));
    HIP_TRY(hipStreamSynchronize(st));
    const size_t words = grid_header_offsets(h, nitems);
    *out_bytes = words * 4;
    if (!grid_dev) return APT_OK;
    if (capacity < words * 4) return fail(APT_ERR_ARG, "apt_build_grid_device: capacity too small (see *out_bytes)%s");
    uint32_t *w = (uint32_t *)grid_dev;
    HIP_TRY(hipMemsetAsync(w, 0, words * 4, st));
    HIP_TRY(hipMemcpyAsync(w, &h, sizeof h, hipMemcpyHostToDevice, st));
    if (h.nlarge) HIP_TRY(hipMemcpyAsync(w + h.off_large, large.get(), (size_t)h.nlarge * 4, hipMemcpyDeviceToDevice, st));
    HIP_TRY(hipMemcpyAsync(w + h.off_cells, count.get(), nc1 * 4, hipMemcpyDeviceToDevice, st));
    if (stt.nsmall) hipLaunchKernelGGL(grid_fill_kernel, dim3((stt.nsmall + 255) / 256), dim3(256), 0, st, h, spheres_dev, rad.get(), small.get(), stt.nsmall, count.get(), cursor.get(), w + h.off_items);
    HIP_TRY(long_cells.alloc(nitems / (kGridSortInline + 1u) + 1u)); HIP_TRY(long_count.alloc(1));
    HIP_TRY(hipMemsetAsync(long_count.get(), 0, 4, st));
    hipLaunchKernelGGL(grid_sort_cells_kernel, dim3((h.ncells + 255) / 256), dim3(256), 0, st, h.ncells, count.get(), w + h.off_items, long_count.get(), long_cells.get());
    uint32_t nlong = 0;
    HIP_TRY(hipMemcpyAsync(&nlong, long_count.get(), 4, hipMemcpyDeviceToHost, st));
    HIP_TRY(hipStreamSynchronize(st));
    if (nlong) {
        std::vector<uint2> cells(nlong);
        std::vector<uint32_t> host_items(nitems);
        HIP_TRY(hipMemcpy(cells.data(), long_cells.get(), (size_t)nlong * sizeof(uint2), hipMemcpyDeviceToHost));
        HIP_TRY(hipMemcpy(host_items.data(), w + h.off_items, (size_t)nitems * 4, hipMemcpyDeviceToHost));
        for (const uint2 &c : cells) std::sort(host_items.begin() + c.x, host_items.begin() + c.y);
        HIP_TRY(hipMemcpy(w + h.off_items, host_items.data(), (size_t)nitems * 4, hipMemcpyHostToDevice));
    }
    const uint32_t ng = ns > nitems ? ns : nitems;
    hipLaunchKernelGGL(grid_geom_kernel, dim3((ng + 255) / 256), dim3(256), 0, st, spheres_dev, ns, w + h.off_items, nitems,
                       reinterpret_cast<float4 *>(w + h.off_geom), reinterpret_cast<float4 *>(w + h.off_item_geom));
    if (h.off_cellslot) hipLaunchKernelGGL(grid_slots_kernel, dim3((std::max(apt::grid_bordered_cells(h.n) + 1u, ns) + 255u) / 256u), dim3(256), 0, st, w, h, spheres_dev);
    HIP_TRY(hipGetLastError());
    HIP_TRY(hipStreamSynchronize(st));
    return APT_OK;
}

int apt_selftest_sqrt(int variant, void *stream, uint64_t first_bits, uint64_t count, uint64_t *device_result2) {
    clear_error();
    if (!device_result2 || variant < 0 || variant > 3) return fail(APT_ERR_ARG, "apt_selftest_sqrt: bad arguments%s");
    if (first_bits + count > (1ull << 32)) return fail(APT_ERR_ARG, "apt_selftest_sqrt: range beyond 2^32%s");
    if (count == 0) return APT_OK;
    hipLaunchKernelGGL(selftest_sqrt_kernel, dim3(256 * 16), dim3(kBlock), 0, (hipStream_t)stream, variant, first_bits,
                       count, (unsigned long long *)device_result2);
    return launched();
}

int apt_selftest_div3(void *stream, uint64_t first, uint64_t count, uint64_t *device_result3) {
    clear_error();
    if (!device_result3) return fail(APT_ERR_ARG, "apt_selftest_div3: bad arguments%s");
    if (count == 0) return APT_OK;
    hipLaunchKernelGGL(selftest_div3_kernel, dim3(256 * 16), dim3(kBlock), 0, (hipStream_t)stream, first, count,
                       (unsigned long long *)device_result3);
    return launched();
}

int apt_selftest_direction(void *stream, const double *d3, uint64_t count, uint64_t *device_result5, uint8_t *device_flags) {
    clear_error();
    if (!d3 || !device_result5) return fail(APT_ERR_ARG, "apt_selftest_direction: bad arguments%s");
    if (count == 0) return APT_OK;
    apt::selftest_direction(stream, d3, count, device_result5, device_flags);
    return launched();
}

int apt_test_scene(const apt_render_params *p, void *stream, const float *rays, const float *spheres, float *out) {
    clear_error();
    int rc = check_params(p);
    if (rc) return rc;
    if (!rays || !spheres || !out) return fail(APT_ERR_ARG, "rays/spheres/out must be non-null%s");
    const uint64_t n = (uint64_t)p->width * p->height * 4u * p->samples;
    unsigned blocks;
    if ((rc = one_launch((n + kBlock - 1) / kBlock, "image too large for one launch%s", &blocks))) return rc;
    hipLaunchKernelGGL(test_scene_kernel, dim3(blocks), dim3(kBlock), 0, (hipStream_t)stream, rays, spheres,
                       out, n, p->num_spheres, p->light_index, p->eps);
    return launched();
}

int apt_gen_rays_device(const apt_render_params *p, void *stream, float *rays) {
    clear_error();
    int rc = check_params(p);
    if (rc) return rc;
    PathRange r;
    if ((rc = paths_launch_range(p, rays != nullptr, r, "rays must be non-null%s")) || r.c == 0) return rc;
    Camera cam;
    camera_init(cam, p->width, p->height);
    hipLaunchKernelGGL(gen_rays_kernel, dim3(r.grid), dim3(kBlock), 0, (hipStream_t)stream, cam, p->width,
                       p->height, p->samples, p->seed, r.plane(), r.b, r.c, r.base(rays));
    return launched();
}

int apt_gen_rays_camera_device(const apt_render_params *p, const apt_camera *cam, void *stream, float *rays) {
    clear_error();
    int rc = check_params(p);
    if (rc) return rc;
    if ((rc = apt_camera_check_host(cam))) return rc;
    PathRange r;
    if ((rc = paths_launch_range(p, rays != nullptr, r, "rays must be non-null%s")) || r.c == 0) return rc;
    apt::mat_gen_rays_camera(apt::CamRaysCall{cam, p->width, p->height, p->samples, p->seed, r.base(rays), r.plane(), r.b, r.c, stream});
    return launched();
}

int apt_gen_rays_mt_device_ex(const apt_render_params *p, void *stream, const uint32_t *checkpoints, uint32_t stride,
                              uint64_t num_checkpoints, uint64_t first_block, float *rays) {
    clear_error();
    int rc = check_params(p);
    if (rc) return rc;
    if (!rays || !checkpoints || stride == 0) return fail(APT_ERR_ARG, "rays/checkpoints must be non-null, stride > 0%s");
    PathRange r;
    if ((rc = path_range(p, r)) || r.c == 0) return rc;
    const uint64_t b = r.b, c = r.c;
    const uint64_t num_blocks = (r.n_image + kPathsPerBlock - 1) / kPathsPerBlock;
    const uint64_t blk_lo = b / kPathsPerBlock, blk_hi = (b + c + kPathsPerBlock - 1) / kPathsPerBlock;
    if (blk_lo < first_block) return fail(APT_ERR_ARG, "path range starts before the checkpoint window%s");
    const uint64_t cp_lo = (blk_lo - first_block) / stride, cp_hi = (blk_hi - first_block + stride - 1) / stride;
    if (cp_hi > num_checkpoints) return fail(APT_ERR_ARG, "not enough MT19937 checkpoints for this path range%s");
    unsigned grid;
    if ((rc = one_launch(cp_hi - cp_lo, "too many checkpoints for one launch%s", &grid))) return rc;
    Camera cam;
    camera_init(cam, p->width, p->height);
    hipLaunchKernelGGL(gen_rays_mt_kernel, dim3(grid), dim3(kBlock), 0, (hipStream_t)stream,
                       checkpoints + cp_lo * kMtN, stride, first_block + cp_lo * stride, num_blocks, cam, p->width, p->height,
                       p->samples, r.plane(), b, b + c, r.base(rays));
    return launched();
}

int apt_gen_rays_mt_device(const apt_render_params *p, void *stream, const uint32_t *checkpoints, uint32_t stride,
                           uint64_t num_checkpoints, float *rays) {
    return apt_gen_rays_mt_device_ex(p, stream, checkpoints, stride, num_checkpoints, 0, rays);
}

int apt_render_frame_mt(const apt_render_params *p, void *stream, const uint32_t *checkpoints, uint64_t num_checkpoints,
                        uint64_t first_group, const float *spheres, uint64_t pixel_begin, uint64_t pixel_count, float *fb, uint8_t *fb_u8) {
    clear_error();
    int rc = check_params(p);
    if (rc) return rc;
    if (!checkpoints || !spheres || !fb) return fail(APT_ERR_ARG, "apt_render_frame_mt: checkpoints/spheres/fb must be non-null%s");
    if (p->num_spheres != 8) return fail(APT_ERR_SCENE, "apt_render_frame_mt: the 8-sphere scene only%s");
    if (p->flags & APT_FLAG_RR) return fail(APT_ERR_ARG, "apt_render_frame_mt: APT_FLAG_RR is not part of the reference's pipeline%s");
    uint32_t log2_s = 0;
    while ((1u << log2_s) < p->samples) ++log2_s;
    const bool pow2_kernel = (1u << log2_s) == p->samples && p->samples >= 8 && p->samples <= 256;
    LeafProg lp;
    if ((rc = make_leaf_prog(p->samples, lp))) return rc;
    if ((rc = pixel_range(p, pixel_begin, pixel_count)) || pixel_count == 0) return rc;
    const uint64_t g_lo = pixel_begin / kMtGroupPixels, g_hi = (pixel_begin + pixel_count + kMtGroupPixels - 1) / kMtGroupPixels;
    if (g_lo < first_group || g_hi - first_group > num_checkpoints) return fail(APT_ERR_ARG, "apt_render_frame_mt: the checkpoint table does not cover the pixel range%s");
    unsigned groups;
    if ((rc = one_launch(g_hi - g_lo, "pixel_count too large for one launch; shard it%s", &groups))) return rc;
    if ((rc = refuse_camera(apt::default_context().snapshot(), "apt_render_frame_mt"))) return rc;
    const TraceArgs ta = make_trace_args(p, launch_state(apt::default_context(), stream));
    const FrameArgs fa = make_frame_args(p, pixel_begin, pixel_count, fb, fb_u8);
    MtFrameArgs ma;
    ma.checkpoints = checkpoints + (g_lo - first_group) * 624; ma.first_group = g_lo; ma.log2_s = log2_s;
    const dim3 grid(groups);
    hipStream_t st = (hipStream_t)stream;
    with_mode(p->mode, [&](auto m) {
        if (pow2_kernel) hipLaunchKernelGGL((render_frame_mt_kernel<m>), grid, dim3(kBlock), 0, st, spheres, fa, ta, ma);
        else hipLaunchKernelGGL((render_frame_mt_any_kernel<m>), grid, dim3(kBlock), 0, st, spheres, fa, ta, ma, lp);
    });
    return launched();
}

int apt_decode_color_band(const apt_render_params *p, void *stream, const float *colors, uint64_t pixel_count, float *fb,
                          uint8_t *fb_u8) {
    clear_error();
    int rc = check_params(p);
    if (rc) return rc;
    if (!colors || !fb) return fail(APT_ERR_ARG, "colors/fb must be non-null%s");
    if (pixel_count == 0) return APT_OK;
    LeafProg lp;
    if ((rc = make_leaf_prog(p->samples, lp))) return rc;
    const uint64_t npix = pixel_count;
    const bool wide = p->samples >= 8;
    const bool quad = wide && p->samples <= 8u * kDecode4Blocks && lp.nleaves == 1 && p->samples % 4 == 0 && ((uintptr_t)colors & 15u) == 0;
    const uint64_t lanes = npix * 3 * 4 * (quad ? 2 : (wide ? 8 : 1));
    unsigned blocks;
    if ((rc = one_launch((lanes + kBlock - 1) / kBlock, "band too large for one launch%s", &blocks))) return rc;
    if (quad)
        hipLaunchKernelGGL(decode_color_kernel4, dim3(std::min(blocks, 256u * 256u)), dim3(kBlock), 0, (hipStream_t)stream, colors,
                           p->samples, npix, lp, fb, fb_u8);
    else if (wide)
        hipLaunchKernelGGL(decode_color_kernel8, dim3(std::min(blocks, p->samples >= 64 ? 256u * 1024u : 256u * 256u)), dim3(kBlock), 0, (hipStream_t)stream, colors,
                           p->samples, npix, lp, fb, fb_u8);
    else
        hipLaunchKernelGGL(decode_color_kernel, dim3(blocks), dim3(kBlock), 0, (hipStream_t)stream, colors,
                           p->samples, npix, lp, fb, fb_u8);
    return launched();
}

int apt_decode_color_device(const apt_render_params *p, void *stream, const float *colors, float *fb, uint8_t *fb_u8) {
    clear_error();
    if (!p) return fail(APT_ERR_ARG, "params is null%s");
    return apt_decode_color_band(p, stream, colors, (uint64_t)p->width * p->height, fb, fb_u8);
}

}
```

Measured before the change: 243,700 Mray/s.

## Add conservative first-bounce plan to skip provably-missed spheres per wave

Adds a small device kernel that runs before the 8-sphere frame render and uses interval arithmetic over the camera footprint to compute per-row and per-column bounds. From these bounds each pixel gets a mask of spheres its first-bounce ray provably cannot hit. The record is written into an enlarged status buffer keyed by a ticket, and the plane-specialised first bounce uses the wave-ANDed mask to skip those sphere tests. This trades a tiny extra launch and some mask logic for fewer VALU ops on the first segment only, and it depends on scene-shape premises that disable the plan when they do not hold.

```diff
diff --git a/__graft_entry__.py b/__graft_entry__.py
--- a/__graft_entry__.py
+++ b/__graft_entry__.py
@@ -15,7 +15,8 @@
         return False
     pkg = os.path.join(ROOT, "ascendpathtracing_amd")
     csrc = os.path.join(pkg, "csrc")
-    pairs = [([os.path.join(pkg, "librender_mi355x.so"), os.path.join(pkg, "render_gpu")] + [st.built_path for st in _lib.STAGES.values()],
+    pairs = [([os.path.join(pkg, "librender_mi355x.so"), os.path.join(pkg, "libfirstplan_mi355x.so"), os.path.join(pkg, "render_gpu")]
+              + [st.built_path for st in _lib.STAGES.values()],
               glob.glob(os.path.join(csrc, "*.h")) + glob.glob(os.path.join(csrc, "*.hip")) + glob.glob(os.path.join(csrc, "*.cpp"))
               + [os.path.join(csrc, "Makefile"), os.path.join(csrc, "apt_exports.map")] + _lib.public_headers()),
              ([os.path.join(ROOT, "oracle", "libpt_oracle.so")],
diff --git a/ascendpathtracing_amd/csrc/apt_host.h b/ascendpathtracing_amd/csrc/apt_host.h
--- a/ascendpathtracing_amd/csrc/apt_host.h
+++ b/ascendpathtracing_amd/csrc/apt_host.h
@@ -59,6 +59,8 @@
 
 namespace apt {
 apt_context &default_context();
+struct Camera;
+bool launch_first_plan(void *stream, const float *spheres_dev, const Camera &cam, uint32_t width, uint32_t height, float eps, uint32_t *status_dev, uint64_t ticket);
 int film_resolve_check(const apt_film_resolve *r, const void *film, const void *table, const void *out, const void *u8, const char *what);
 inline double grid_spheres_per_cell() {
     const double knob = default_context().snapshot().debug.grid_spheres_per_cell;
diff --git a/ascendpathtracing_amd/csrc/first_plan.hip b/ascendpathtracing_amd/csrc/first_plan.hip
--- /dev/null
+++ b/ascendpathtracing_amd/csrc/first_plan.hip
@@ -0,0 +1,28 @@
+#include <hip/hip_runtime.h>
+#include <stdint.h>
+
+#include "apt_host.h"
+#include "pt_first_plan.h"
+
+namespace {
+
+__global__ __launch_bounds__(64) void first_plan_kernel(const float *__restrict__ sph, apt::Camera cam, uint32_t width, uint32_t height, float eps,
+                                                        uint64_t *__restrict__ rec, uint64_t ticket) {
+    if (threadIdx.x != 0 || blockIdx.x >= (uint32_t)apt::kFirstPlanWords) return;
+    apt::FirstPlanGeom g;
+    apt::first_plan_setup(cam, width, height, sph, eps, g);
+    apt::first_plan_premise_origin(g);
+    rec[blockIdx.x] = apt::first_plan_pack(apt::first_plan_entry(g, (int)blockIdx.x), ticket);
+}
+
+}
+
+namespace apt {
+
+bool launch_first_plan(void *stream, const float *spheres_dev, const Camera &cam, uint32_t width, uint32_t height, float eps, uint32_t *status_dev, uint64_t ticket) {
+    uint64_t *const rec = reinterpret_cast<uint64_t *>(status_dev + first_plan_slot_word(ticket));
+    hipLaunchKernelGGL(first_plan_kernel, dim3(kFirstPlanWords), dim3(64), 0, (hipStream_t)stream, spheres_dev, cam, width, height, eps, rec, ticket);
+    return hipGetLastError() == hipSuccess;
+}
+
+}
diff --git a/ascendpathtracing_amd/csrc/first_plan_host.cpp b/ascendpathtracing_amd/csrc/first_plan_host.cpp
--- /dev/null
+++ b/ascendpathtracing_amd/csrc/first_plan_host.cpp
@@ -0,0 +1,36 @@
+#include <math.h>
+#include <stdint.h>
+#include <string.h>
+
+#include "pt_first_plan.h"
+
+extern "C" {
+
+__attribute__((visibility("default"))) int apt_first_plan_host(uint32_t width, uint32_t height, const float *spheres, double eps,
+                                                               const double *camera12, int32_t *record16) {
+    if (!spheres || !record16 || !width || !height) return 1;
+    apt::Camera cam;
+    apt::camera_init(cam, width, height);
+    if (camera12) {
+        for (int i = 0; i < 3; ++i) { cam.pos[i] = camera12[i]; cam.g[i] = camera12[3 + i]; cam.cx[i] = camera12[6 + i]; cam.cy[i] = camera12[9 + i]; }
+    }
+    apt::FirstPlanGeom g;
+    apt::first_plan_setup(cam, width, height, spheres, (float)eps, g);
+    apt::first_plan_premise_origin(g);
+    for (int k = 0; k < apt::kFirstPlanWords; ++k) record16[k] = apt::first_plan_entry(g, k);
+    return 0;
+}
+
+__attribute__((visibility("default"))) int apt_first_plan_camera_host(uint32_t width, uint32_t height, double *camera12) {
+    if (!camera12 || !width || !height) return 1;
+    apt::Camera cam;
+    apt::camera_init(cam, width, height);
+    for (int i = 0; i < 3; ++i) { camera12[i] = cam.pos[i]; camera12[3 + i] = cam.g[i]; camera12[6 + i] = cam.cx[i]; camera12[9 + i] = cam.cy[i]; }
+    return 0;
+}
+
+__attribute__((visibility("default"))) uint32_t apt_first_plan_mask_host(const int32_t *record16, uint32_t width, uint32_t height, uint32_t col, uint32_t row) {
+    return record16 ? apt::first_plan_mask(record16, width, height, col, row) : 0u;
+}
+
+}
diff --git a/ascendpathtracing_amd/csrc/pt_first_plan.h b/ascendpathtracing_amd/csrc/pt_first_plan.h
--- /dev/null
+++ b/ascendpathtracing_amd/csrc/pt_first_plan.h
@@ -0,0 +1,223 @@
+#pragma once
+#include "pt_core.h"
+
+namespace apt {
+
+constexpr int kFirstPlanWords = 16;
+constexpr uint32_t kFirstPlanBase = 16, kFirstPlanSlots = 64;
+constexpr uint32_t kFirstPlanAllocWords = kFirstPlanBase + kFirstPlanSlots * (uint32_t)kFirstPlanWords * 2u;
+APT_HD uint64_t first_plan_pack(int32_t value, uint64_t ticket) { return (uint64_t)(uint32_t)value | ((uint64_t)(uint32_t)ticket << 32); }
+APT_HD uint32_t first_plan_slot_word(uint64_t ticket) { return kFirstPlanBase + (uint32_t)(ticket % kFirstPlanSlots) * (uint32_t)kFirstPlanWords * 2u; }
+constexpr double kFirstPlanDepth = 4.0;
+constexpr double kFirstPlanCErr = 3072.0;
+constexpr double kFirstPlanMaxEps = 1.0;
+
+struct FpIv { double lo, hi; };
+APT_HD FpIv fp_lin(double c, FpIv x, double g) { return c >= 0 ? FpIv{c * x.lo + g, c * x.hi + g} : FpIv{c * x.hi + g, c * x.lo + g}; }
+APT_HD double fp_min(double a, double b) { return a < b ? a : b; }
+APT_HD double fp_max(double a, double b) { return a > b ? a : b; }
+APT_HD double fp_minabs(FpIv x) { return (x.lo <= 0 && x.hi >= 0) ? 0.0 : fp_min(fabs(x.lo), fabs(x.hi)); }
+APT_HD double fp_maxabs(FpIv x) { return fp_max(fabs(x.lo), fabs(x.hi)); }
+APT_HD FpIv fp_mul(FpIv a, FpIv b) {
+    const double p0 = a.lo * b.lo, p1 = a.lo * b.hi, p2 = a.hi * b.lo, p3 = a.hi * b.hi;
+    return FpIv{fp_min(fp_min(p0, p1), fp_min(p2, p3)), fp_max(fp_max(p0, p1), fp_max(p2, p3))};
+}
+APT_HD FpIv fp_from(double c, FpIv x) { return FpIv{c - x.hi, c - x.lo}; }
+
+struct FirstPlanGeom {
+    bool ok;
+    double cx0, cy1, cy2, g1, g2, pos[3];
+    int32_t w, h;
+    double C[8][3], r2[8], R[6];
+    double lo[3], hi[3];
+    double D;
+    double nmin2, nmax;
+    FpIv d0all, d1all, d2all;
+};
+
+APT_HD FpIv fp_footprint(int32_t i0, int32_t i1, int32_t n) {
+    return FpIv{((double)i0 - 0.25) / (double)n - 0.5 - 1e-9, ((double)i1 + 1.25) / (double)n - 0.5 + 1e-9};
+}
+APT_HD FpIv fp_d0(const FirstPlanGeom &g, int32_t i0, int32_t i1) { return fp_lin(g.cx0, fp_footprint(i0, i1, g.w), 0.0); }
+APT_HD FpIv fp_d1(const FirstPlanGeom &g, int32_t j0, int32_t j1) { return fp_lin(g.cy1, fp_footprint(j0, j1, g.h), g.g1); }
+APT_HD FpIv fp_d2(const FirstPlanGeom &g, int32_t j0, int32_t j1) { return fp_lin(g.cy2, fp_footprint(j0, j1, g.h), g.g2); }
+APT_HD FpIv fp_origin(double pos, FpIv d) { return FpIv{pos + 140.0 * d.lo - 0x1p-10, pos + 140.0 * d.hi + 0x1p-10}; }
+
+APT_HD void first_plan_setup(const Camera &cam, uint32_t width, uint32_t height, const float *sph, float eps, FirstPlanGeom &g) {
+    g.ok = false;
+    if (!(cam.cx[1] == 0 && cam.cx[2] == 0 && cam.cy[0] == 0 && cam.g[0] == 0 && cam.cx[0] > 0)) return;
+    if (!(width >= 1 && height >= 1 && width <= (1u << 24) && height <= (1u << 24))) return;
+    if (!(eps_allows_rootkey(eps) && (double)eps <= kFirstPlanMaxEps)) return;
+    g.cx0 = cam.cx[0]; g.cy1 = cam.cy[1]; g.cy2 = cam.cy[2]; g.g1 = cam.g[1]; g.g2 = cam.g[2];
+    g.pos[0] = cam.pos[0]; g.pos[1] = cam.pos[1]; g.pos[2] = cam.pos[2];
+    g.w = (int32_t)width; g.h = (int32_t)height;
+    const float *fx = sph + 8, *fy = sph + 16, *fz = sph + 24;
+    auto eq = [](float a, float b) { return f32_bits(a) == f32_bits(b); };
+    if (!(eq(fx[2], fx[3]) && eq(fx[2], fx[4]) && eq(fx[2], fx[5]) && eq(fx[2], fx[7]) && eq(fy[0], fy[1]) && eq(fy[0], fy[2]) &&
+          eq(fy[0], fy[3]) && eq(fz[0], fz[1]) && eq(fz[0], fz[4]) && eq(fz[0], fz[5]) && eq(fz[0], fz[7]))) return;
+    for (int k = 0; k < 8; ++k) {
+        g.r2[k] = (double)sph[k]; g.C[k][0] = (double)fx[k]; g.C[k][1] = (double)fy[k]; g.C[k][2] = (double)fz[k];
+        if (!(g.r2[k] > 0 && g.r2[k] < 0x1p60 && fabs(g.C[k][0]) < 0x1p30 && fabs(g.C[k][1]) < 0x1p30 && fabs(g.C[k][2]) < 0x1p30)) return;
+    }
+    for (int k = 0; k < 6; ++k) {
+        g.R[k] = sqrt(g.r2[k]);
+        if (!(g.R[k] >= 5e4 && g.R[k] <= 1.3e5)) return;
+    }
+    g.lo[0] = g.C[0][0] - g.R[0]; g.hi[0] = g.C[1][0] + g.R[1];
+    g.lo[2] = g.C[2][2] - g.R[2]; g.hi[2] = g.C[3][2] + g.R[3];
+    g.lo[1] = g.C[4][1] - g.R[4]; g.hi[1] = g.C[5][1] + g.R[5];
+    for (int a = 0; a < 3; ++a)
+        if (!(g.hi[a] - g.lo[a] >= 2 * kFirstPlanDepth && g.hi[a] - g.lo[a] <= 1000.0 && fabs(g.lo[a]) <= 1000.0 && fabs(g.hi[a]) <= 1000.0)) return;
+    if (!(g.C[0][0] > g.hi[0] && g.C[1][0] < g.lo[0] && g.C[2][2] > g.hi[2] && g.C[3][2] < g.lo[2] && g.C[4][1] > g.hi[1] && g.C[5][1] < g.lo[1])) return;
+    for (int k = 0; k < 6; ++k) {
+        const int own = k < 2 ? 0 : (k < 4 ? 2 : 1);
+        for (int a = 0; a < 3; ++a)
+            if (a != own && !(fabs(g.C[k][a]) <= 1000.0)) return;
+    }
+    const double ex = g.hi[0] - g.lo[0], ey = g.hi[1] - g.lo[1], ez = g.hi[2] - g.lo[2];
+    g.D = sqrt(ex * ex + ey * ey + ez * ez);
+    g.d0all = fp_d0(g, 0, g.w - 1); g.d1all = fp_d1(g, 0, g.h - 1); g.d2all = fp_d2(g, 0, g.h - 1);
+    if (!(g.d2all.hi < 0)) return;
+    const double a0 = fp_maxabs(g.d0all), a1 = fp_maxabs(g.d1all), a2 = fp_maxabs(g.d2all);
+    const double i0 = fp_minabs(g.d0all), i1 = fp_minabs(g.d1all), i2 = fp_minabs(g.d2all);
+    g.nmax = sqrt(a0 * a0 + a1 * a1 + a2 * a2) * (1 + 1e-9);
+    g.nmin2 = (i0 * i0 + i1 * i1 + i2 * i2) * (1 - 1e-9);
+    if (!(g.nmin2 > 0x1p-20 && g.nmax < 0x1p10)) return;
+    g.ok = true;
+}
+
+APT_HD void first_plan_premise_origin(FirstPlanGeom &g);
+
+template <class F>
+APT_HD int32_t fp_largest(int32_t nmax, F P) {
+    int32_t lo = 0, hi = nmax;
+    while (lo < hi) {
+        const int32_t mid = lo + (hi - lo + 1) / 2;
+        if (P(mid)) lo = mid;
+        else hi = mid - 1;
+    }
+    return lo;
+}
+
+APT_HD bool fp_inside_wall(const FirstPlanGeom &g, int k, int ax, FpIv o) {
+    if (!(o.lo >= g.lo[ax] && o.hi <= g.hi[ax])) return false;
+    double s = 0;
+    for (int a = 0; a < 3; ++a) {
+        const FpIv span = a == ax ? o : FpIv{g.lo[a], g.hi[a]};
+        const double m = fp_maxabs(fp_from(g.C[k][a], span));
+        s = s + m * m;
+    }
+    const double need = 2 * g.R[k] * kFirstPlanDepth - kFirstPlanDepth * kFirstPlanDepth + kFirstPlanCErr;
+    return s - g.r2[k] <= -need;
+}
+APT_HD bool fp_cols_inside(const FirstPlanGeom &g, int32_t i0, int32_t i1) {
+    const FpIv o = fp_origin(g.pos[0], fp_d0(g, i0, i1));
+    return fp_inside_wall(g, 0, 0, o) && fp_inside_wall(g, 1, 0, o);
+}
+APT_HD bool fp_rows_inside(const FirstPlanGeom &g, int32_t j0, int32_t j1) {
+    const FpIv oy = fp_origin(g.pos[1], fp_d1(g, j0, j1)), oz = fp_origin(g.pos[2], fp_d2(g, j0, j1));
+    if (!(oy.lo >= g.lo[1] && oy.hi <= g.hi[1] && oz.lo >= g.lo[2] && oz.hi <= g.hi[2])) return false;
+    bool ok = true;
+    for (int k = 2; k < 6; ++k) {
+        double s = 0;
+        for (int a = 0; a < 3; ++a) {
+            const FpIv span = a == 1 ? oy : (a == 2 ? oz : FpIv{g.lo[0], g.hi[0]});
+            const double m = fp_maxabs(fp_from(g.C[k][a], span));
+            s = s + m * m;
+        }
+        const double need = 2 * g.R[k] * kFirstPlanDepth - kFirstPlanDepth * kFirstPlanDepth + kFirstPlanCErr;
+        ok = ok && s - g.r2[k] <= -need;
+    }
+    return ok;
+}
+APT_HD void first_plan_premise_origin(FirstPlanGeom &g) {
+    if (g.ok && !(fp_cols_inside(g, g.w / 2, g.w / 2) && fp_rows_inside(g, g.h / 2, g.h / 2))) g.ok = false;
+}
+APT_HD bool fp_wall_far(const FirstPlanGeom &g, int k, int ax, double sgn, FpIv dcomp) {
+    const double toward = sgn > 0 ? dcomp.lo : -dcomp.hi;
+    if (!(toward > 0)) return false;
+    const double reach = sgn > 0 ? g.C[k][ax] - g.hi[ax] : g.lo[ax] - g.C[k][ax];
+    double other = 0;
+    for (int a = 0; a < 3; ++a)
+        if (a != ax) other = other + fp_maxabs(fp_from(g.C[k][a], FpIv{g.lo[a], g.hi[a]})) * (1 + 0x1p-20);
+    const double blo = reach * toward / g.nmax - other - 1.0;
+    return blo > g.D + 4.0 + 1.0;
+}
+APT_HD bool fp_line_misses(const FirstPlanGeom &g, int k, int ax, FpIv dp, FpIv dz) {
+    const double wp = g.C[k][ax] - g.pos[ax], wz = g.C[k][2] - g.pos[2];
+    const double rho2 = g.r2[k] + 4.0 + g.r2[k] * 0x1p-12;
+    const double gap = wp * wp + wz * wz - rho2;
+    if (!(gap > 0)) return false;
+    const FpIv tp = fp_lin(wp, dp, 0.0), tz = fp_lin(wz, dz, 0.0);
+    const double nabs = fp_max(fabs(tp.lo + tz.lo), fabs(tp.hi + tz.hi)) * (1 + 1e-9);
+    const double ip = fp_minabs(dp), iz = fp_minabs(dz);
+    return nabs * nabs < gap * (ip * ip + iz * iz) * (1 - 1e-9);
+}
+APT_HD bool fp_light_behind(const FirstPlanGeom &g, int32_t j0, int32_t j1) {
+    const FpIv d[3] = {g.d0all, fp_d1(g, j0, j1), fp_d2(g, j0, j1)};
+    double cmin = 0, bhi = 0;
+    for (int a = 0; a < 3; ++a) {
+        const FpIv t = fp_from(g.C[7][a], fp_origin(g.pos[a], d[a]));
+        const double m = fp_minabs(t);
+        cmin = cmin + m * m;
+        bhi = bhi + fp_mul(t, d[a]).hi;
+    }
+    if (!(cmin - g.r2[7] >= 4.0 + g.r2[7] * 0x1p-12)) return false;
+    return bhi < 0 && bhi / g.nmax <= -1.0;
+}
+
+APT_HD int32_t first_plan_entry(const FirstPlanGeom &g, int which) {
+    if (!g.ok || which < 0 || which > 13) return 0;
+    const int32_t w = g.w, h = g.h, mc = w / 2, mr = h / 2;
+    switch (which) {
+    case 0: case 1: {
+        if (!fp_cols_inside(g, mc, mc)) return 0;
+        if (which == 0) return mc - fp_largest(mc, [&](int32_t n) { return fp_cols_inside(g, mc - n, mc); });
+        return mc + 1 + fp_largest(w - 1 - mc, [&](int32_t n) { return fp_cols_inside(g, mc, mc + n); });
+    }
+    case 2: case 3: {
+        if (!fp_rows_inside(g, mr, mr)) return 0;
+        if (which == 2) return mr - fp_largest(mr, [&](int32_t n) { return fp_rows_inside(g, mr - n, mr); });
+        return mr + 1 + fp_largest(h - 1 - mr, [&](int32_t n) { return fp_rows_inside(g, mr, mr + n); });
+    }
+    case 4: return fp_largest(w, [&](int32_t n) { return fp_wall_far(g, 0, 0, 1.0, fp_d0(g, w - n, w - 1)); });
+    case 5: return fp_largest(w, [&](int32_t n) { return fp_wall_far(g, 1, 0, -1.0, fp_d0(g, 0, n - 1)); });
+    case 6: return fp_largest(h, [&](int32_t n) { return fp_wall_far(g, 4, 1, 1.0, fp_d1(g, h - n, h - 1)); });
+    case 7: return fp_largest(h, [&](int32_t n) { return fp_wall_far(g, 5, 1, -1.0, fp_d1(g, 0, n - 1)); });
+    case 8: return fp_wall_far(g, 3, 2, -1.0, g.d2all) ? 1 : 0;
+    case 9: return fp_largest(w, [&](int32_t n) { return fp_line_misses(g, 6, 0, fp_d0(g, 0, n - 1), g.d2all); });
+    case 10: return fp_largest(w, [&](int32_t n) { return fp_line_misses(g, 6, 0, fp_d0(g, w - n, w - 1), g.d2all); });
+    case 11: return fp_largest(h, [&](int32_t n) { return fp_line_misses(g, 6, 1, fp_d1(g, 0, n - 1), fp_d2(g, 0, n - 1)); });
+    case 12: return fp_largest(h, [&](int32_t n) { return fp_line_misses(g, 6, 1, fp_d1(g, h - n, h - 1), fp_d2(g, h - n, h - 1)); });
+    default: {
+        const int32_t miss = fp_largest(h, [&](int32_t n) { return fp_line_misses(g, 7, 1, fp_d1(g, 0, n - 1), fp_d2(g, 0, n - 1)); });
+        const int32_t behind = fp_largest(h, [&](int32_t n) { return fp_light_behind(g, 0, n - 1); });
+        return miss > behind ? miss : behind;
+    }
+    }
+}
+
+APT_HD bool first_plan_cond(uint32_t k, int32_t r, uint32_t width, uint32_t height, uint32_t col, uint32_t row) {
+    const bool on_col = k == 0 || k == 1 || k == 4 || k == 5 || k == 9 || k == 10;
+    const int32_t x = on_col ? (int32_t)col : (int32_t)row, n = on_col ? (int32_t)width : (int32_t)height;
+    const bool from_end = k == 4 || k == 6 || k == 10 || k == 12;
+    const bool at_least = k == 0 || k == 2 || from_end;
+    const int32_t t = from_end ? n - r : r;
+    if (k == 8) return r != 0;
+    return at_least ? x >= t : x < t;
+}
+APT_HD uint32_t first_plan_combine(uint32_t conds) {
+    uint32_t m = 0;
+    if ((conds & 0xFu) == 0xFu)
+        m = ((conds >> 4) & 1u) | (((conds >> 5) & 1u) << 1) | (((conds >> 8) & 1u) << 3) | (((conds >> 6) & 1u) << 4) | (((conds >> 7) & 1u) << 5);
+    m |= (conds & 0x1E00u) ? 64u : 0u;
+    m |= ((conds >> 13) & 1u) << 7;
+    return m;
+}
+APT_HD uint32_t first_plan_mask(const int32_t *r, uint32_t width, uint32_t height, uint32_t col, uint32_t row) {
+    uint32_t conds = 0;
+    for (uint32_t k = 0; k < 14; ++k) conds |= first_plan_cond(k, r[k], width, height, col, row) ? 1u << k : 0u;
+    return first_plan_combine(conds);
+}
+
+}
diff --git a/ascendpathtracing_amd/csrc/pt_kernels.h b/ascendpathtracing_amd/csrc/pt_kernels.h
--- a/ascendpathtracing_amd/csrc/pt_kernels.h
+++ b/ascendpathtracing_amd/csrc/pt_kernels.h
@@ -1,6 +1,7 @@
 #pragma once
 #include "pt_trace.h"
 #include "pt_trace2.h"
+#include "pt_first_plan.h"
 #include "pt_queue.h"
 #include "pt_frame_mt.h"
 
@@ -198,6 +199,21 @@
     uint32_t traced = 0;
     uint32_t queue_traced = 0;
 
+    uint32_t first_plan = 0;
+    const uint64_t ticket = TWO ? first_plan_ticket(ta) : 0;
+    if (TWO && ticket != 0 && ta.status) {
+        const uint64_t *const rec = reinterpret_cast<const uint64_t *>(ta.status + first_plan_slot_word(ticket));
+        const uint32_t k = lane < 14u ? lane : 13u;
+        const uint64_t e = rec[k];
+        if (__builtin_amdgcn_ballot_w64((uint32_t)(e >> 32) != (uint32_t)ticket) == 0) {
+            const int32_t r = (int32_t)(uint32_t)e;
+            const uint32_t c0 = (uint32_t)__builtin_amdgcn_readlane((int)pi, 0), r0 = (uint32_t)__builtin_amdgcn_readlane((int)pj, 0);
+            const uint32_t c1 = (uint32_t)__builtin_amdgcn_readlane((int)pi, 32), r1 = (uint32_t)__builtin_amdgcn_readlane((int)pj, 32);
+            const uint32_t conds0 = (uint32_t)__builtin_amdgcn_ballot_w64(first_plan_cond(k, r, fa.width, fa.height, c0, r0)) & 0x3FFFu;
+            const uint32_t conds1 = (uint32_t)__builtin_amdgcn_ballot_w64(first_plan_cond(k, r, fa.width, fa.height, c1, r1)) & 0x3FFFu;
+            first_plan = first_plan_combine(conds0) & first_plan_combine(conds1);
+        }
+    }
     const Gain3 gain = load_gain(sph, ta);
     struct Col { float r, g, b; };
     auto sample = [&](uint32_t k) __attribute__((always_inline)) -> Col {
@@ -225,7 +241,7 @@
         PathPair pp;
         camera_ray_pair(cam, fa.width, fa.height, pi, pj, sy, sx, chain_state_uniform(lane_state, u), pp.ox, pp.oy, pp.oz, pp.dx, pp.dy, pp.dz);
         asm("" : "+v"(pp.ox), "+v"(pp.oy), "+v"(pp.oz), "+v"(pp.dx), "+v"(pp.dy), "+v"(pp.dz));
-        trace2_ns8<MODE>(sc, tab8, pp, ta, planes);
+        trace2_ns8<MODE, true>(sc, tab8, pp, ta, planes, first_plan);
         traced += 2 * ta.depth;
         return Col2{Col{pp.rx.x * gain.r, pp.ry.x * gain.g, pp.rz.x * gain.b}, Col{pp.rx.y * gain.r, pp.ry.y * gain.g, pp.rz.y * gain.b}};
     };
diff --git a/ascendpathtracing_amd/csrc/pt_trace.h b/ascendpathtracing_amd/csrc/pt_trace.h
--- a/ascendpathtracing_amd/csrc/pt_trace.h
+++ b/ascendpathtracing_amd/csrc/pt_trace.h
@@ -57,6 +57,10 @@
     unsigned long long *traced;
     uint32_t *status;
 };
+static_assert(sizeof(const uint32_t *) == sizeof(uint64_t), "a ticket fits the slot");
+__host__ __device__ __forceinline__ uint64_t first_plan_ticket(const TraceArgs &ta) { return (uint64_t)reinterpret_cast<uintptr_t>(ta.grid); }
+inline void set_first_plan_ticket(TraceArgs &ta, uint64_t ticket) { ta.grid = reinterpret_cast<const uint32_t *>((uintptr_t)ticket); }
+
 template <uint32_t K>
 __device__ __forceinline__ uint32_t xcd_chunked_block(uint32_t wg, uint32_t nwg) {
     constexpr uint32_t kXcds = 8, G = kXcds * K;
diff --git a/ascendpathtracing_amd/csrc/pt_trace2.h b/ascendpathtracing_amd/csrc/pt_trace2.h
--- a/ascendpathtracing_amd/csrc/pt_trace2.h
+++ b/ascendpathtracing_amd/csrc/pt_trace2.h
@@ -68,9 +68,9 @@
 
 constexpr int kAbSkip = 0xC0;
 
-template <int MODE, int SKIP>
+template <int MODE, int SKIP, bool PLAN = false>
 __device__ __forceinline__ void intersect2_ns8_planes(const Scene8 &sc, const PathPair &s, const TraceArgs &ta, const KeyConsts &kc,
-                                                      float &aminA, float &aminB, Hit8 &hA, Hit8 &hB) {
+                                                      float &aminA, float &aminB, Hit8 &hA, Hit8 &hB, uint32_t plan = 0) {
     struct Term { f2 p, q; };
     auto term = [](auto half, f2 cpair, f2 o, f2 d) __attribute__((always_inline)) {
         const f2 t = pair_half_minus<decltype(half)::value>(cpair, o);
@@ -108,30 +108,56 @@
         aminB = minimum3_abs(aminB, h.disc.y, h.disc.y);
         stage(h, k);
     };
+    auto wall = [&](const Pre &h, int k) __attribute__((always_inline)) {
+        aminA = minimum3_abs(aminA, h.disc.x, h.disc.x);
+        aminB = minimum3_abs(aminB, h.disc.y, h.disc.y);
+        stage(h, k);
+    };
+    uint32_t here = 0;
+    if (PLAN) asm volatile("s_mov_b32 %0, %1" : "=s"(here) : "s"(plan));
+    auto planned = [&](auto bit) __attribute__((always_inline)) {
+        uint32_t run;
+        asm volatile("s_bitcmp0_b32 %1, %2\n\ts_cselect_b32 %0, 1, 0" : "=s"(run) : "s"(here), "n"(decltype(bit)::value) : "scc");
+        return run;
+    };
     static_assert((SKIP & 0x3F) == 0, "the walls have no test: the room lies inside their spheres");
+    using B0 = std::integral_constant<int, 0>; using B1 = std::integral_constant<int, 1>; using B3 = std::integral_constant<int, 3>;
+    using B4 = std::integral_constant<int, 4>; using B5 = std::integral_constant<int, 5>; using B6 = std::integral_constant<int, 6>;
+    using B7 = std::integral_constant<int, 7>;
     const f2 X1 = {sc.cx[0], sc.cx[1]}, X2 = {sc.cx[2], sc.cx[6]}, Y1 = {sc.cy[4], sc.cy[5]}, Y2 = {sc.cy[6], sc.cy[7]}, Y3 = {sc.cy[0], sc.cy[0]};
     const f2 Z1 = {sc.cz[2], sc.cz[3]}, Z2 = {sc.cz[0], sc.cz[6]};
     const f2 R0 = {sc.r2[0], sc.r2[1]}, R1 = {sc.r2[2], sc.r2[3]}, R2 = {sc.r2[4], sc.r2[5]}, R3 = {sc.r2[6], sc.r2[7]};
     using Lo = std::integral_constant<int, 0>;
     using Hi = std::integral_constant<int, 1>;
     const Term x2 = term(Lo{}, X2, s.ox, s.dx), y0 = term(Lo{}, Y3, s.oy, s.dy), z0 = term(Lo{}, Z2, s.oz, s.dz);
-    walls(pre(term(Lo{}, X1, s.ox, s.dx), y0, z0, Lo{}, R0), pre(term(Hi{}, X1, s.ox, s.dx), y0, z0, Hi{}, R0), 0);
-    walls(pre(x2, y0, term(Lo{}, Z1, s.oz, s.dz), Lo{}, R1), pre(x2, y0, term(Hi{}, Z1, s.oz, s.dz), Hi{}, R1), 2);
-    walls(pre(x2, term(Lo{}, Y1, s.oy, s.dy), z0, Lo{}, R2), pre(x2, term(Hi{}, Y1, s.oy, s.dy), z0, Hi{}, R2), 4);
-    tested(pre(term(Hi{}, X2, s.ox, s.dx), term(Lo{}, Y2, s.oy, s.dy), term(Hi{}, Z2, s.oz, s.dz), Lo{}, R3), 6);
-    tested(pre(x2, term(Hi{}, Y2, s.oy, s.dy), z0, Hi{}, R3), 7);
+    if (PLAN) {
+        if (planned(B0{}) != 0u) wall(pre(term(Lo{}, X1, s.ox, s.dx), y0, z0, Lo{}, R0), 0);
+        if (planned(B1{}) != 0u) wall(pre(term(Hi{}, X1, s.ox, s.dx), y0, z0, Hi{}, R0), 1);
+        wall(pre(x2, y0, term(Lo{}, Z1, s.oz, s.dz), Lo{}, R1), 2);
+        if (planned(B3{}) != 0u) wall(pre(x2, y0, term(Hi{}, Z1, s.oz, s.dz), Hi{}, R1), 3);
+        if (planned(B4{}) != 0u) wall(pre(x2, term(Lo{}, Y1, s.oy, s.dy), z0, Lo{}, R2), 4);
+        if (planned(B5{}) != 0u) wall(pre(x2, term(Hi{}, Y1, s.oy, s.dy), z0, Hi{}, R2), 5);
+        if (planned(B6{}) != 0u) tested(pre(term(Hi{}, X2, s.ox, s.dx), term(Lo{}, Y2, s.oy, s.dy), term(Hi{}, Z2, s.oz, s.dz), Lo{}, R3), 6);
+        if (planned(B7{}) != 0u) tested(pre(x2, term(Hi{}, Y2, s.oy, s.dy), z0, Hi{}, R3), 7);
+    } else {
+        walls(pre(term(Lo{}, X1, s.ox, s.dx), y0, z0, Lo{}, R0), pre(term(Hi{}, X1, s.ox, s.dx), y0, z0, Hi{}, R0), 0);
+        walls(pre(x2, y0, term(Lo{}, Z1, s.oz, s.dz), Lo{}, R1), pre(x2, y0, term(Hi{}, Z1, s.oz, s.dz), Hi{}, R1), 2);
+        walls(pre(x2, term(Lo{}, Y1, s.oy, s.dy), z0, Lo{}, R2), pre(x2, term(Hi{}, Y1, s.oy, s.dy), z0, Hi{}, R2), 4);
+        tested(pre(term(Hi{}, X2, s.ox, s.dx), term(Lo{}, Y2, s.oy, s.dy), term(Hi{}, Z2, s.oz, s.dz), Lo{}, R3), 6);
+        tested(pre(x2, term(Hi{}, Y2, s.oy, s.dy), z0, Hi{}, R3), 7);
+    }
     hA = A.finish(ta, kc);
     hB = B.finish(ta, kc);
 }
 
-template <int MODE, bool PLANES, bool FIRST>
+template <int MODE, bool PLANES, bool FIRST, bool PLAN = false>
 __device__ __forceinline__ void bounce2_ns8_t(const Scene8 &sc, const Tab8 tab, const PathPair &s, PathPair &n,
                                               const TraceArgs &ta, const KeyConsts &kc, uint32_t ones_off,
-                                              uint64_t &aliveA, uint64_t &aliveB, uint64_t &redoA, uint64_t &redoB) {
+                                              uint64_t &aliveA, uint64_t &aliveB, uint64_t &redoA, uint64_t &redoB, uint32_t plan = 0) {
     float aminA = 1.0f, aminB = 1.0f;
     Hit8 hA, hB;
     if (PLANES) {
-        intersect2_ns8_planes<MODE, kAbSkip>(sc, s, ta, kc, aminA, aminB, hA, hB);
+        intersect2_ns8_planes<MODE, kAbSkip, PLAN && FIRST>(sc, s, ta, kc, aminA, aminB, hA, hB, plan);
     } else {
         hA = intersect_ns8_v2<MODE>(sc, s.ox.x, s.oy.x, s.oz.x, s.dx.x, s.dy.x, s.dz.x, ta, kc, aminA);
         hB = intersect_ns8_v2<MODE>(sc, s.ox.y, s.oy.y, s.oz.y, s.dx.y, s.dy.y, s.dz.y, ta, kc, aminB);
@@ -213,14 +239,14 @@
     bounce2_ns8_t<MODE, PLANES, true>(sc, tab, s, n, ta, kc, ones_off, aliveA, aliveB, redoA, redoB);
 }
 
-template <int MODE, bool PLANES, bool FIRST = false>
+template <int MODE, bool PLANES, bool FIRST = false, bool PLAN = false>
 __device__ __forceinline__ void bounce2_ns8_last(const Scene8 &sc, const Tab8 tab, const PathPair &s, f2 &rx, f2 &ry, f2 &rz,
                                                  const TraceArgs &ta, const KeyConsts &kc, uint32_t ones_off,
-                                                 uint64_t &aliveA, uint64_t &aliveB, uint64_t &redoA, uint64_t &redoB) {
+                                                 uint64_t &aliveA, uint64_t &aliveB, uint64_t &redoA, uint64_t &redoB, uint32_t plan = 0) {
     float aminA = 1.0f, aminB = 1.0f;
     Hit8 hA, hB;
     if (PLANES) {
-        intersect2_ns8_planes<MODE, kAbSkip>(sc, s, ta, kc, aminA, aminB, hA, hB);
+        intersect2_ns8_planes<MODE, kAbSkip, PLAN && FIRST>(sc, s, ta, kc, aminA, aminB, hA, hB, plan);
     } else {
         hA = intersect_ns8_v2<MODE>(sc, s.ox.x, s.oy.x, s.oz.x, s.dx.x, s.dy.x, s.dz.x, ta, kc, aminA);
         hB = intersect_ns8_v2<MODE>(sc, s.ox.y, s.oy.y, s.oz.y, s.dx.y, s.dy.y, s.dz.y, ta, kc, aminB);
@@ -250,8 +276,8 @@
     redoB = __builtin_amdgcn_ballot_w64(!(aminB >= kFastMin));
 }
 
-template <int MODE, bool PLANES>
-__device__ __forceinline__ void trace2_ns8_t(const Scene8 &sc, const Tab8 tab, PathPair &s, const TraceArgs &ta) {
+template <int MODE, bool PLANES, bool PLAN = false>
+__device__ __forceinline__ void trace2_ns8_t(const Scene8 &sc, const Tab8 tab, PathPair &s, const TraceArgs &ta, uint32_t plan = 0) {
     const KeyConsts kc = make_key_consts(ta.eps);
     uint32_t ones_off = 8 * 16;
     asm volatile("" : "+v"(ones_off));
@@ -354,7 +380,7 @@
         bool redo_any = !fast_ok;
         if (__builtin_expect(fast_ok, 1)) {
             uint64_t redoA, redoB;
-            bounce2_ns8_t<MODE, PLANES, first>(sc, tab, in, out, ta, kc, ones_off, oa, ob, redoA, redoB);
+            bounce2_ns8_t<MODE, PLANES, first, PLAN && PLANES>(sc, tab, in, out, ta, kc, ones_off, oa, ob, redoA, redoB, plan);
             if (__builtin_expect((redoA | redoB) != 0, 0)) redo_any = redo_stands(in, redoA, redoB, first);
         }
         if (__builtin_expect(redo_any, 0)) {
@@ -381,7 +407,7 @@
         bool redo_any = !fast_ok;
         if (__builtin_expect(fast_ok, 1)) {
             uint64_t redoA, redoB;
-            bounce2_ns8_last<MODE, PLANES, first>(sc, tab, in, rx, ry, rz, ta, kc, ones_off, oa, ob, redoA, redoB);
+            bounce2_ns8_last<MODE, PLANES, first, PLAN && PLANES>(sc, tab, in, rx, ry, rz, ta, kc, ones_off, oa, ob, redoA, redoB, plan);
             if (__builtin_expect((redoA | redoB) != 0, 0)) redo_any = redo_stands(in, redoA, redoB, first);
         }
         if (__builtin_expect(redo_any, 0)) {
@@ -418,14 +444,14 @@
     }
 }
 
-template <int MODE>
-__device__ __forceinline__ void trace2_ns8(const Scene8 &sc, const Tab8 tab, PathPair &s, const TraceArgs &ta, bool planes) {
+template <int MODE, bool PLAN = false>
+__device__ __forceinline__ void trace2_ns8(const Scene8 &sc, const Tab8 tab, PathPair &s, const TraceArgs &ta, bool planes, uint32_t plan = 0) {
     if (planes) {
         Scene8 p = sc;
         p.cx[3] = p.cx[4] = p.cx[5] = p.cx[7] = sc.cx[2];
         p.cy[1] = p.cy[2] = p.cy[3] = sc.cy[0];
         p.cz[1] = p.cz[4] = p.cz[5] = p.cz[7] = sc.cz[0];
-        trace2_ns8_t<MODE, true>(p, tab, s, ta);
+        trace2_ns8_t<MODE, true, PLAN>(p, tab, s, ta, plan);
     } else {
         trace2_ns8_t<MODE, false>(sc, tab, s, ta);
     }
diff --git a/ascendpathtracing_amd/csrc/render_kernels.hip b/ascendpathtracing_amd/csrc/render_kernels.hip
--- a/ascendpathtracing_amd/csrc/render_kernels.hip
+++ b/ascendpathtracing_amd/csrc/render_kernels.hip
@@ -1,5 +1,6 @@
 #include <hip/hip_runtime.h>
 #include <algorithm>
+#include <atomic>
 #include <new>
 #include <stdint.h>
 #include <stdio.h>
@@ -81,6 +82,10 @@
     return APT_OK;
 }
 
+std::atomic<uint64_t> g_plan_ticket{1};
+uint64_t plan_ticket(uint32_t *status) {
+    return status ? g_plan_ticket.fetch_add(1u, std::memory_order_relaxed) : 0u;
+}
 uint32_t *status_word(apt_context &ctx, hipStream_t st) {
     int dev = 0;
     if (hipGetDevice(&dev) != hipSuccess) { (void)hipGetLastError(); return nullptr; }
@@ -90,7 +95,7 @@
     if (hipStreamIsCapturing(st, &cs) != hipSuccess) { (void)hipGetLastError(); return nullptr; }
     if (cs != hipStreamCaptureStatusNone) return nullptr;
     apt::DeviceBuffer<uint32_t> fresh;
-    if (fresh.alloc(1) != hipSuccess || hipMemset(fresh.get(), 0, sizeof(uint32_t)) != hipSuccess) { (void)hipGetLastError(); return nullptr; }
+    if (fresh.alloc(apt::kFirstPlanAllocWords) != hipSuccess || hipMemset(fresh.get(), 0, apt::kFirstPlanAllocWords * sizeof(uint32_t)) != hipSuccess) { (void)hipGetLastError(); return nullptr; }
     uint32_t *spare = nullptr;
     uint32_t *w = ctx.status_adopt(dev, fresh.release(), &spare);
     apt::DeviceBuffer<uint32_t> loser(spare);
@@ -265,10 +270,15 @@
     const dim3 grid((unsigned)fs.blocks);
     with_mode(p->mode, [&](auto m) {
         if (ns8 && group == 8) {
-            if (!retire && !rrk && p->samples >= 16)
-                hipLaunchKernelGGL((render_frame_kernel<m, kScene8, 8, false, true>), grid, dim3(kBlock), lds, st, spheres, fa, ta, lp);
-            else
+            if (!retire && !rrk && p->samples >= 16) {
+                uint64_t ticket = plan_ticket(ls.status);
+                if (ticket && !apt::launch_first_plan(st, spheres, fa.cam, fa.width, fa.height, ta.eps, ls.status, ticket)) ticket = 0;
+                TraceArgs ta2 = ta;
+                set_first_plan_ticket(ta2, ticket);
+                hipLaunchKernelGGL((render_frame_kernel<m, kScene8, 8, false, true>), grid, dim3(kBlock), lds, st, spheres, fa, ta2, lp);
+            } else {
                 hipLaunchKernelGGL((render_frame_kernel<m, kScene8, 8, false>), grid, dim3(kBlock), lds, st, spheres, fa, ta, lp);
+            }
         } else if (ns8) {
             with_flag(retire, [&](auto rt) {
                 hipLaunchKernelGGL((render_frame_kernel<m, kScene8, 1, rt>), grid, dim3(kBlock), lds, st, spheres, fa, ta, lp);
diff --git a/profiles/first_bounce_plan_counts.py b/profiles/first_bounce_plan_counts.py
--- /dev/null
+++ b/profiles/first_bounce_plan_counts.py
@@ -0,0 +1,60 @@
+#!/usr/bin/env python3
+import ctypes
+import json
+import os
+import sys
+
+import numpy as np
+
+ROOT = os.path.dirname(os.path.dirname(os.path.abspath(__file__)))
+sys.path.insert(0, ROOT)
+W, H, DEPTH = 1920, 1080, 8
+ISA = {0: 24, 1: 28, 3: 26, 4: 28, 5: 28, 6: 20, 7: 14}
+ADDED = 6
+
+
+def main():
+    from ascendpathtracing_amd import gen_data
+    L = ctypes.CDLL(os.path.join(ROOT, "ascendpathtracing_amd", "libfirstplan_mi355x.so"))
+    L.apt_first_plan_mask_host.restype = ctypes.c_uint32
+    sph = np.ascontiguousarray(gen_data.gen_spheres(), dtype=np.float32)
+    rec = np.zeros(16, dtype=np.int32)
+    assert L.apt_first_plan_host(ctypes.c_uint32(W), ctypes.c_uint32(H), ctypes.c_void_p(sph.ctypes.data), ctypes.c_double(1e-4), None,
+                                 ctypes.c_void_p(rec.ctypes.data)) == 0
+    c, j = np.arange(W)[:, None], np.arange(H)[None, :]
+    inside = (c >= rec[0]) & (c < rec[1]) & (j >= rec[2]) & (j < rec[3])
+    m = np.zeros((W, H), dtype=np.uint32)
+    m |= np.where(inside & (rec[8] != 0), 8, 0).astype(np.uint32)
+    m |= np.where(inside & (c >= W - rec[4]), 1, 0).astype(np.uint32)
+    m |= np.where(inside & (c < rec[5]), 2, 0).astype(np.uint32)
+    m |= np.where(inside & (j >= H - rec[6]), 16, 0).astype(np.uint32)
+    m |= np.where(inside & (j < rec[7]), 32, 0).astype(np.uint32)
+    m |= np.where((c < rec[9]) | (c >= W - rec[10]) | (j < rec[11]) | (j >= H - rec[12]), 64, 0).astype(np.uint32)
+    m |= np.where((j < rec[13]) & (c >= 0), 128, 0).astype(np.uint32)
+    rng = np.random.default_rng(0)
+    for cc, jj in zip(rng.integers(0, W, 4000), rng.integers(0, H, 4000)):
+        assert L.apt_first_plan_mask_host(ctypes.c_void_p(rec.ctypes.data), W, H, int(cc), int(jj)) == m[cc, jj]
+    q = m.ravel()
+    waves = q[0::2] & q[1::2]
+    shares = {k: float(((waves >> k) & 1).mean()) for k in ISA}
+    per_pair = {k: shares[k] * ISA[k] for k in ISA}
+    segments = 2 * DEPTH
+    out = {
+        "what": "gate of the first-bounce plan: wave shares over the C2 frame from the plan's CPU twin, priced with the listing's per-sphere counts",
+        "frame": [W, H], "record": [int(v) for v in rec],
+        "wave_share_sphere_left_out": {str(k): round(v, 4) for k, v in shares.items()},
+        "valu_per_sphere_block": {str(k): v for k, v in ISA.items()},
+        "valu_added_per_first_pair_bounce": ADDED,
+        "predicted_valu_saved_per_segment_by_sphere": {str(k): round(v / segments, 3) for k, v in per_pair.items()},
+        "predicted_valu_saved_per_segment": round((sum(per_pair.values()) - ADDED) / segments, 3),
+        "gate": "build when the total is >= 2.0 per segment; drop a sphere below 0.2",
+    }
+    out["gate_passed"] = out["predicted_valu_saved_per_segment"] >= 2.0 and all(v >= 0.2 for v in out["predicted_valu_saved_per_segment_by_sphere"].values())
+    with open(os.path.join(ROOT, "profiles", "first_bounce_plan_counts.json"), "w") as f:
+        json.dump(out, f, indent=1)
+        f.write("\n")
+    print(json.dumps(out, indent=1))
+
+
+if __name__ == "__main__":
+    main()
```

Measured after the change: 249,300 Mray/s (median of 6 runs). 1.02x the previous value.
